# peterropac/Aegolius

Measured on AMD Instinct MI355X. Metric: Mpoints/sec SDF eval, 1024^3 grid, 10-prim smooth-union tree, higher is better.
Workload: dtype f32

## Files before the change

### aegolius_amd/_engine.py

```python
import atexit
import contextlib
import ctypes
import importlib.util
import os
import sys
import threading

import numpy as np

_HERE = os.path.dirname(os.path.abspath(__file__))
LIB_PATH = os.path.join(_HERE, "libsdfk.so")

MODE_AUTO, MODE_INTERPRET, MODE_SPECIALIZED, MODE_NOCULL = 0, 1, 2, 3
(FLAVOUR_PLAIN_ARRAY, FLAVOUR_PLAIN_GRID, FLAVOUR_TILE_ARRAY, FLAVOUR_TILE_GRID, FLAVOUR_TILE_MASK, FLAVOUR_ROWS_ARRAY,
 FLAVOUR_ROWS_GRID, FLAVOUR_ROWS_MASK, FLAVOUR_ROWS2D_ARRAY, FLAVOUR_ROWS2D_GRID, FLAVOUR_RAYS, FLAVOUR_OCCUPANCY) = range(12)
FLAVOUR_FLAGS = 0x100
FLAVOUR_XY = 0x200

_c = ctypes
_vp, _i64, _int, _sz = _c.c_void_p, _c.c_int64, _c.c_int, _c.c_size_t
_fp = _c.POINTER(_c.c_float)

SIGNATURES = {
    "sdfk_abi_version": (_int, []),
    "sdfk_device_count": (_int, []),
    "sdfk_last_error": (_c.c_char_p, []),
    "sdfk_program_create": (_vp, [_vp, _sz, _vp, _sz, _vp, _sz, _int]),
    "sdfk_program_destroy": (None, [_vp]),
    "sdfk_program_set_params": (_int, [_vp, _vp, _sz]),
    "sdfk_program_set_cull": (_int, [_vp, _vp, _sz, _vp]),
    "sdfk_program_source": (_c.c_char_p, [_vp]),
    "sdfk_program_compile_check": (_int, [_vp, _c.POINTER(_sz)]),
    "sdfk_program_chain_members": (_int, [_vp]),
    "sdfk_program_compile_flavour": (_int, [_vp, _int, _c.POINTER(_sz), _c.POINTER(_c.c_double)]),
    "sdfk_debug_compile_external": (_int, [_vp, _int, _c.POINTER(_sz)]),
    "sdfk_debug_jit_stats": (None, [_c.POINTER(_i64), _c.POINTER(_c.c_double)]),
    "sdfk_jit_drain": (None, []),
    "sdfk_jit_cancel": (None, []),
    "sdfk_debug_set_rtc_defs": (None, [_c.c_char_p]),
    "sdfk_eval_device": (_int, [_vp, _vp, _i64, _i64, _vp, _vp, _int]),
    "sdfk_eval_device_rows": (_int, [_vp, _vp, _i64, _i64, _i64, _vp, _vp, _int]),
    "sdfk_eval_device_rows2d": (_int, [_vp, _vp, _i64, _i64, _i64, _vp, _vp, _int]),
    "sdfk_eval_device_rows2d_xy": (_int, [_vp, _vp, _i64, _i64, _i64, _vp, _vp, _int]),
    "sdfk_debug_cells_stats": (None, [_int, _c.POINTER(_c.c_longlong)]),
    "sdfk_debug_rays_stats": (None, [_int, _c.POINTER(_c.c_longlong)]),
    "sdfk_eval_device_rows3d": (_int, [_vp, _vp, _i64, _i64, _i64, _i64, _i64, _vp, _vp, _int]),
    "sdfk_debug_row_masks": (_int, [_vp, _vp, _i64, _i64, _i64, _vp, _c.POINTER(_i64), _c.POINTER(_int), _vp]),
    "sdfk_eval_grid_sharded": (_int, [_vp, _vp, _i64, _vp, _i64, _vp, _i64, _int, _vp, _vp, _int]),
    "sdfk_eval_grid_sharded_device": (_int, [_vp, _vp, _i64, _vp, _i64, _vp, _i64, _int, _vp, _int, _vp, _int]),
    "sdfk_eval_device_aux": (_int, [_vp, _vp, _i64, _i64, _vp, _int, _i64, _vp, _vp, _int]),
    "sdfk_eval_grid_aux": (_int, [_vp, _vp, _i64, _vp, _i64, _vp, _i64, _i64, _i64, _vp, _int, _i64, _vp, _vp, _int]),
    "sdfk_field_min": (_int, [_vp, _i64, _c.POINTER(_c.c_float), _vp]),
    "sdfk_grid_box_average": (_int, [_vp, _i64, _i64, _i64, _int, _int, _int, _int, _vp, _vp]),
    "sdfk_grid_edge_detect": (_int, [_vp, _i64, _i64, _i64, _vp, _vp]),
    "sdfk_debug_box_variant": (_int, [_i64, _i64, _i64, _int, _int, _int, _c.POINTER(_int)]),
    "sdfk_grid_signed": (_int, [_vp, _i64, _i64, _i64, _c.c_float, _int, _vp, _vp]),
    "sdfk_grid_boundary_mask": (_int, [_vp, _i64, _c.c_float, _vp, _vp]),
    "sdfk_grid_signed_slab": (_int, [_vp, _i64, _i64, _vp, _i64, _i64, _i64, _int, _vp, _vp]),
    "sdfk_eval_host": (_int, [_vp, _vp, _int, _i64, _i64, _vp, _int, _int]),
    "sdfk_eval_host_resident": (_int, [_vp, _vp, _int, _i64, _i64, _vp, _int, _int]),
    "sdfk_field_select_scratch": (_sz, [_i64]),
    "sdfk_field_select": (_int, [_vp, _i64, _c.c_float, _vp, _i64, _c.POINTER(_i64), _vp, _vp]),
    "sdfk_field_select_finish": (_int, [_i64, _i64, _vp, _i64, _vp, _vp]),
    "sdfk_field_gradient": (_int, [_vp, _i64, _i64, _i64, _int, _int, _vp, _i64, _vp]),
    "sdfk_field_crossings_2d": (_int, [_vp, _vp, _i64, _i64, _i64, _c.c_double, _c.c_double, _c.c_double, _vp, _vp]),
    "sdfk_lcwg_eval": (_int, [_int, _vp, _vp, _i64, _i64, _i64, _c.c_double, _c.c_double, _int, _c.c_double, _vp, _vp, _i64,
                              _vp]),
    "sdfk_lcwg_old_eval": (_int, [_int, _vp, _i64, _vp, _i64, _c.c_double, _c.c_double, _vp, _i64, _vp]),
    "sdfk_eval_select_scratch": (_sz, [_i64, _i64]),
    "sdfk_eval_device_select": (_int, [_vp, _vp, _i64, _i64, _i64, _int, _c.c_float, _vp, _i64, _c.POINTER(_i64), _vp, _vp, _int]),
    "sdfk_eval_grid_select": (_int, [_vp, _vp, _i64, _vp, _i64, _vp, _i64, _i64, _i64, _c.c_float, _vp, _i64, _c.POINTER(_i64),
                                     _vp, _vp, _int]),
    "sdfk_eval_select_finish": (_int, [_vp, _i64, _i64, _int, _i64, _vp, _i64, _vp, _vp]),
    "sdfk_vec_eval_device": (_int, [_vp, _int, _vp, _i64, _i64, _vp, _int, _i64, _int, _vp, _i64, _vp]),
    "sdfk_vec_set_interpret": (None, [_int]),
    "sdfk_vec_source": (_c.c_char_p, [_vp, _int, _int, _int]),
    "sdfk_vec_compile_check": (_int, [_vp, _int, _int, _int, _c.POINTER(_sz)]),
    "sdfk_vec_eval_host": (_int, [_vp, _int, _vp, _int, _i64, _vp, _i64, _vp, _i64, _vp, _i64, _vp, _int, _int, _vp, _int]),
    "sdfk_eval_grid": (_int, [_vp, _vp, _i64, _vp, _i64, _vp, _i64, _i64, _i64, _vp, _vp, _int]),
    "sdfk_eval_grid_host": (_int, [_vp, _vp, _i64, _vp, _i64, _vp, _i64, _i64, _i64, _vp, _int, _int]),
    "sdfk_set_default_mode": (None, [_int]),
    "sdfk_debug_brick_masks": (_int, [_vp, _vp, _i64, _i64, _vp, _vp]),
    "sdfk_linspace_f32": (_int, [_c.c_double, _c.c_double, _i64, _vp]),
    "sdfk_point_tree_build": (_i64, [_vp, _i64, _int, _vp, _i64, _vp, _vp, _vp]),
    "sdfk_grid_fill": (_int, [_vp, _i64, _vp, _i64, _vp, _i64, _vp, _i64, _i64, _i64, _vp]),
    "sdfk_set_device": (_int, [_int]),
    "sdfk_malloc": (_vp, [_sz]),
    "sdfk_free": (_int, [_vp]),
    "sdfk_memcpy_h2d": (_int, [_vp, _vp, _sz]),
    "sdfk_memcpy_d2h": (_int, [_vp, _vp, _sz]),
    "sdfk_memcpy_d2d": (_int, [_vp, _vp, _sz]),
    "sdfk_sync": (_int, [_vp]),
    "sdfk_event_create": (_vp, []),
    "sdfk_event_destroy": (_int, [_vp]),
    "sdfk_event_record": (_int, [_vp, _vp]),
    "sdfk_event_elapsed_ms": (_int, [_vp, _vp, _fp]),
    "sdfk_stream_probe": (_int, [_vp, _i64, _i64, _vp, _vp]),
    "sdfk_dual_has_rule": (_int, [_int]),
    "sdfk_program_jvp_check": (_int, [_vp, _c.POINTER(_int)]),
    "sdfk_eval_jvp_device": (_int, [_vp, _vp, _i64, _i64, _vp, _int, _int, _vp, _vp, _i64, _vp]),
    "sdfk_value_jvp_device": (_int, [_int, _vp, _vp, _vp, _i64, _vp, _vp, _vp]),
    "sdfk_program_vjp_check": (_int, [_vp, _c.POINTER(_int), _c.POINTER(_i64)]),
    "sdfk_vjp_limits": (_int, [_c.POINTER(_int), _c.POINTER(_int)]),
    "sdfk_eval_vjp_device": (_int, [_vp, _vp, _i64, _i64, _vp, _int, _int, _vp, _vp, _vp, _vp]),
    "sdfk_points_bin": (_int, [_vp, _i64, _i64, _vp, _i64, _i64, _i64, _vp, _vp]),
    "sdfk_points_extent": (_int, [_vp, _i64, _i64, _i64, _vp, _vp]),
    "sdfk_points_fill": (_int, [_vp, _i64, _i64, _i64, _int, _i64, _i64, _i64, _vp]),
    "sdfk_points_widen": (_int, [_vp, _i64, _int, _vp, _vp]),
    "sdfk_field_isosurface_scratch": (_sz, [_i64, _i64, _i64]),
    "sdfk_field_isosurface": (_int, [_vp, _vp, _i64, _vp, _i64, _vp, _i64, _c.c_float, _c.POINTER(_i64), _c.POINTER(_i64), _vp,
                                     _vp]),
    "sdfk_field_isosurface_finish": (_int, [_vp, _i64, _i64, _i64, _c.c_float, _i64, _i64, _vp, _i64, _vp, _i64, _int, _vp,
                                            _vp]),
    "sdfk_field_contour2d_scratch": (_sz, [_i64, _i64]),
    "sdfk_field_contour2d": (_int, [_vp, _vp, _i64, _vp, _i64, _c.c_float, _c.POINTER(_i64), _c.POINTER(_i64), _vp, _vp]),
    "sdfk_field_contour2d_finish": (_int, [_vp, _i64, _i64, _c.c_float, _i64, _i64, _vp, _i64, _vp, _i64, _int, _vp, _vp]),
    "sdfk_eval_grid_isosurface_scratch": (_sz, [_i64, _i64, _i64]),
    "sdfk_eval_grid_isosurface": (_int, [_vp, _vp, _i64, _vp, _i64, _vp, _i64, _c.c_float, _c.POINTER(_i64), _c.POINTER(_i64),
                                         _vp, _vp, _int]),
    "sdfk_eval_grid_isosurface_finish": (_int, [_vp, _vp, _i64, _vp, _i64, _vp, _i64, _c.c_float, _i64, _i64, _vp, _i64, _vp,
                                                _i64, _int, _vp, _vp, _int]),
    "sdfk_eval_grid_contour2d_scratch": (_sz, [_i64, _i64]),
    "sdfk_eval_grid_contour2d": (_int, [_vp, _vp, _i64, _vp, _i64, _c.c_float, _c.POINTER(_i64), _c.POINTER(_i64), _vp, _vp,
                                        _int]),
    "sdfk_eval_grid_contour2d_finish": (_int, [_vp, _vp, _i64, _vp, _i64, _c.c_float, _i64, _i64, _vp, _i64, _vp, _i64, _int,
                                               _vp, _vp, _int]),
    "sdfk_program_rays_check": (_int, [_vp, _c.POINTER(_int)]),
    "sdfk_trace_rays_device": (_int, [_vp, _vp, _i64, _vp, _i64, _i64, _c.c_float, _c.c_float, _c.c_float, _c.c_float,
                                      _c.c_float, _int, _vp, _vp, _vp, _vp, _i64, _vp, _int]),
    "sdfk_trace_camera_device": (_int, [_vp, _vp, _int, _int, _int, _c.c_float, _c.c_float, _c.c_float, _c.c_float,
                                        _c.c_float, _int, _vp, _vp, _vp, _vp, _i64, _vp, _int]),
    "sdfk_eval_grid_occupancy_scratch": (_sz, [_i64, _i64, _i64, _i64]),
    "sdfk_eval_grid_occupancy": (_int, [_vp, _vp, _i64, _vp, _i64, _vp, _i64, _vp, _vp, _vp, _vp, _vp, _vp, _int, _c.c_float,
                                        _c.c_float, _vp, _vp, _i64, _c.POINTER(_i64), _c.POINTER(_i64), _fp, _vp, _int]),
    "sdfk_field_row_sums": (_int, [_vp, _i64, _i64, _vp, _vp, _vp]),
    "sdfk_field_redistance_scratch": (_sz, [_i64, _i64, _i64]),
    "sdfk_field_redistance": (_int, [_vp, _vp, _i64, _vp, _i64, _vp, _i64, _c.c_float, _c.c_float, _int, _vp, _vp,
                                     _c.POINTER(_i64), _fp, _vp]),
    "sdfk_box_pad_ulps": (_int, []),
    "sdfk_box_has_rule": (_int, [_int]),
    "sdfk_program_box_check": (_int, [_vp, _c.POINTER(_int)]),
    "sdfk_enclose_boxes_device": (_int, [_vp, _vp, _vp, _i64, _i64, _vp, _vp, _vp, _vp]),
    "sdfk_enclose_octree_scratch": (_sz, []),
    "sdfk_enclose_octree_device": (_int, [_vp, _vp, _i64, _c.POINTER(_c.c_double), _int, _c.c_float, _vp, _vp, _vp, _i64,
                                          _c.POINTER(_i64), _c.POINTER(_i64), _c.POINTER(_int), _vp, _vp]),
}


class SdfkError(RuntimeError):
    pass


_lib = None
_lock = threading.Lock()


def _share_torch_hip_runtime():
    if "torch" in sys.modules:
        return
    try:
        spec = importlib.util.find_spec("torch")
    except (ImportError, ValueError):
        spec = None
    if spec is None or not spec.submodule_search_locations:
        return
    libdir = os.path.join(list(spec.submodule_search_locations)[0], "lib")
    for name in ("libamdhip64.so", "libhiprtc.so"):
        path = os.path.join(libdir, name)
        if os.path.exists(path):
            try:
                ctypes.CDLL(path, mode=ctypes.RTLD_GLOBAL)
            except OSError:
                return


def lib():
    global _lib
    if _lib is None:
        with _lock:
            if _lib is None:
                if not os.path.exists(LIB_PATH):
                    raise SdfkError(
                        "aegolius_amd: %s is missing - build it with "
                        "`python -c 'import __graft_entry__ as g; g.build()'` (needs hipcc, gfx950). "
                        "There is no CPU path." % LIB_PATH)
                _share_torch_hip_runtime()
                handle = ctypes.CDLL(LIB_PATH)
                for name, (res, args) in SIGNATURES.items():
                    fn = getattr(handle, name)
                    fn.restype, fn.argtypes = res, args
                if handle.sdfk_abi_version() != 1:
                    raise SdfkError("libsdfk.so ABI version mismatch")
                atexit.register(handle.sdfk_jit_cancel)
                _lib = handle
    return _lib


def last_error():
    msg = lib().sdfk_last_error()
    return msg.decode("utf-8", "replace") if msg else ""


def check(rc, what):
    if rc != 0:
        raise SdfkError("%s failed (%d): %s" % (what, rc, last_error()))


def device_count():
    return lib().sdfk_device_count()


def require_gpu():
    if device_count() < 1:
        raise SdfkError("aegolius_amd: no HIP device visible - SDF evaluation runs on an MI355X only "
                        "(there is no CPU path)")


def jit_stats():
    n, t = _i64(0), _c.c_double(0.0)
    lib().sdfk_debug_jit_stats(ctypes.byref(n), ctypes.byref(t))
    return n.value, t.value


def _ptr(a):
    return a.ctypes.data_as(_vp) if a is not None and a.size else None


def _release(owner, attr, destroy):
    try:
        h = getattr(owner, attr, None)
        setattr(owner, attr, None)
        if h and _lib is not None:
            getattr(_lib, destroy)(_vp(h))
    except Exception:
        pass


def coords_n(shape):
    if len(shape) != 2 or shape[0] != 3:
        raise ValueError("coordinates must have shape (3, N); got %r" % (tuple(shape),))
    return int(shape[1])


def host_coords(co, dtype=None):
    co = np.asarray(co)
    coords_n(co.shape)
    if dtype is None and co.dtype not in (np.float32, np.float64):
        dtype = np.float64
    return np.ascontiguousarray(co, dtype=dtype)


def axis_args(axes):
    ax = [np.ascontiguousarray(a, dtype=np.float32) for a in axes]
    args = []
    for a in ax:
        args += [_ptr(a), a.size]
    return ax, tuple(args)


def row_stride(n):
    return (n + 63) // 64 * 64


class DeviceBuffer:

    def __init__(self, nbytes, device=None, what=""):
        self.ptr, self.nbytes, self.device = None, int(nbytes), device if device is None else int(device)
        self.what = what or type(self).__name__
        if device is not None:
            check(lib().sdfk_set_device(self.device), "sdfk_set_device")
        self.ptr = lib().sdfk_malloc(self.nbytes) or None
        if self.ptr is None:
            raise SdfkError("%s: out of device memory (%d bytes): %s" % (self.what, self.nbytes, last_error()))

    def at(self, byte_offset=0, nbytes=0):
        if not self.ptr:
            raise SdfkError("%s has been freed" % self.what)
        if byte_offset < 0 or nbytes < 0 or byte_offset + nbytes > self.nbytes:
            raise SdfkError("%s: bytes [%d, %d) are outside its %d bytes" % (self.what, byte_offset, byte_offset + nbytes,
                                                                             self.nbytes))
        return _vp(self.ptr + byte_offset)

    def _live(self):
        self.at()
        if self.device is not None:
            check(lib().sdfk_set_device(self.device), "sdfk_set_device")

    def upload(self, host, byte_offset=0):
        host = np.ascontiguousarray(host)
        dst = self.at(byte_offset, host.nbytes)
        if host.nbytes:
            check(lib().sdfk_memcpy_h2d(dst, _ptr(host), host.nbytes), "sdfk_memcpy_h2d")

    def download(self, out, byte_offset=0):
        if not out.flags.c_contiguous:
            raise ValueError("%s: download needs a C-contiguous array" % self.what)
        src = self.at(byte_offset, out.nbytes)
        if out.nbytes:
            check(lib().sdfk_memcpy_d2h(_ptr(out), src, out.nbytes), "sdfk_memcpy_d2h")
        return out

    def copy_from(self, device_ptr, nbytes, byte_offset=0):
        dst = self.at(byte_offset, nbytes)
        if nbytes:
            check(lib().sdfk_memcpy_d2d(dst, _vp(device_ptr), nbytes), "sdfk_memcpy_d2d")

    def _filled(self, fill, *args):
        try:
            fill(*args)
        except BaseException:
            self.free()
            raise
        return self

    def free(self):
        _release(self, "ptr", "sdfk_free")

    def __enter__(self):
        return self

    def __exit__(self, *exc):
        self.free()

    def __del__(self):
        self.free()


class DeviceRows(DeviceBuffer):

    def __init__(self, rows, n, device=None, what=""):
        self.rows, self.n, self.stride = int(rows), int(n), row_stride(int(n))
        DeviceBuffer.__init__(self, self.rows * self.stride * 4, device, what)

    def offset(self, r):
        return 4 * r * self.stride

    def row(self, r):
        return self.at(self.offset(r), 4 * self.n)

    def row_ptr(self, r):
        return self.row(r).value

    def upload_rows(self, host):
        for r, line in enumerate(np.ascontiguousarray(host, dtype=np.float32)):
            self.upload(line, self.offset(r))

    def download_rows(self, count=None):
        out = np.empty((self.rows if count is None else count, self.n), dtype=np.float32)
        for r, line in enumerate(out):
            self.download(line, self.offset(r))
        return out


class Program:

    def __init__(self, code, params, tables, result_reg, cull_sites=None, cull_k=None):
        self.code = np.ascontiguousarray(code, dtype=np.uint32).reshape(-1, 2)
        self.params = np.ascontiguousarray(params, dtype=np.float32).ravel()
        self.tables = np.ascontiguousarray(tables, dtype=np.float32).ravel()
        self.result_reg = int(result_reg)
        self._h = lib().sdfk_program_create(_ptr(self.code), self.code.shape[0], _ptr(self.params), self.params.size,
                                            _ptr(self.tables), self.tables.size, self.result_reg)
        if not self._h:
            raise SdfkError("sdfk_program_create rejected the program: " + last_error())
        if cull_sites is not None and len(cull_sites):
            sites = np.ascontiguousarray(cull_sites, dtype=np.uint32).reshape(-1, 5)
            k = np.ascontiguousarray(cull_k, dtype=np.float32).ravel()
            check(lib().sdfk_program_set_cull(self._h, _ptr(sites), sites.shape[0], _ptr(k)), "sdfk_program_set_cull")

    @classmethod
    def from_lowered(cls, low, cull=True):
        if cull:
            return cls(low.code, low.params, low.tables, low.result_reg, low.cull_sites, low.cull_k)
        return cls(low.code, low.params, low.tables, low.result_reg)

    @property
    def handle(self):
        return self._h

    def set_params(self, params):
        p = np.ascontiguousarray(params, dtype=np.float32).ravel()
        check(lib().sdfk_program_set_params(self._h, _ptr(p), p.size), "sdfk_program_set_params")
        self.params = p

    def source(self):
        s = lib().sdfk_program_source(self._h)
        return s.decode() if s else None

    @property
    def chain_members(self):
        return int(lib().sdfk_program_chain_members(self._h))

    def compile_check(self):
        n = _sz(0)
        check(lib().sdfk_program_compile_check(self._h, ctypes.byref(n)), "sdfk_program_compile_check")
        return n.value

    def compile_flavour(self, flavour):
        n, t = _sz(0), _c.c_double(0.0)
        check(lib().sdfk_program_compile_flavour(self._h, int(flavour), ctypes.byref(n), ctypes.byref(t)),
              "sdfk_program_compile_flavour")
        return n.value, t.value

    def eval_host(self, co, device=0, mode=MODE_AUTO):
        require_gpu()
        co = host_coords(co)
        n = co.shape[1]
        out = np.empty(n, dtype=np.float32)
        check(lib().sdfk_eval_host(self._h, _ptr(co), 0 if co.dtype == np.float32 else 1, n, n, _ptr(out), device,
                                   mode), "sdfk_eval_host")
        return out

    def eval_device(self, d_co, n, row_stride, d_out, stream=None, mode=MODE_AUTO, row_len=None, flat=False,
                    plane_rows=None, first_row_in_plane=0):
        if row_len and plane_rows and not flat:
            check(lib().sdfk_eval_device_rows3d(self._h, _vp(d_co), n, row_stride, int(row_len), int(plane_rows),
                                                int(first_row_in_plane), _vp(d_out), _vp(stream or 0), mode),
                  "sdfk_eval_device_rows3d")
            return
        if row_len and flat:
            check(lib().sdfk_eval_device_rows2d(self._h, _vp(d_co), n, row_stride, int(row_len), _vp(d_out),
                                                _vp(stream or 0), mode), "sdfk_eval_device_rows2d")
            return
        if row_len:
            check(lib().sdfk_eval_device_rows(self._h, _vp(d_co), n, row_stride, int(row_len), _vp(d_out),
                                              _vp(stream or 0), mode), "sdfk_eval_device_rows")
            return
        check(lib().sdfk_eval_device(self._h, _vp(d_co), n, row_stride, _vp(d_out), _vp(stream or 0), mode),
              "sdfk_eval_device")

    def eval_device_xy(self, d_xy, n, row_stride, d_out, stream=None, mode=MODE_AUTO, row_len=None):
        check(lib().sdfk_eval_device_rows2d_xy(self._h, _vp(d_xy), n, row_stride, int(row_len or 0), _vp(d_out),
                                               _vp(stream or 0), mode), "sdfk_eval_device_rows2d_xy")

    def eval_grid(self, axes, start, count, d_out, stream=None, mode=MODE_AUTO):
        _, tab = axis_args(axes)
        check(lib().sdfk_eval_grid(self._h, *tab, start, count, _vp(d_out), _vp(stream or 0), mode), "sdfk_eval_grid")

    def _select(self, n, first, device, row_len=0, mode=MODE_AUTO):
        require_gpu()
        L = lib()
        check(L.sdfk_set_device(int(device)), "sdfk_set_device")

        def finish(m, d_index, d_scratch):
            check(L.sdfk_eval_select_finish(self._h, n, int(row_len), mode, m, d_index, m, d_scratch, None),
                  "sdfk_eval_select_finish")
        return _select(L.sdfk_eval_select_scratch(n, int(row_len)), first, finish)

    def select_grid(self, axes, threshold=0.0, start=0, count=None, device=0, mode=MODE_AUTO):
        ax, tab = axis_args(axes)
        total = ax[0].size * ax[1].size * ax[2].size
        count = total - start if count is None else count

        def first(d_scratch, m):
            check(lib().sdfk_eval_grid_select(self._h, *tab, start, count, float(threshold), None, 0, m, d_scratch, None,
                                              mode), "sdfk_eval_grid_select")
        grow = ax[2].size if ax[2].size > 1 else ax[1].size
        return self._select(count, first, device, row_len=grow if start % grow == 0 and count % grow == 0 else 0, mode=mode)

    def mesh_grid(self, axes, level, device=0, mode=MODE_AUTO, timings=None):
        require_gpu()
        check(lib().sdfk_set_device(int(device)), "sdfk_set_device")
        ax, tab = axis_args(axes)
        if len(ax) not in (2, 3):
            raise ValueError("mesh_grid: two or three axis tables")
        lead = (self._h,) + tab
        return extract_mesh("sdfk_eval_grid", [a.size for a in ax], level, lead, lead, (mode,), timings)

    def occupancy_grid(self, axes, sub_tables, half_widths, samples, level, lipschitz, d_out, slab_cells=0, device=0,
                       mode=MODE_AUTO, timings=None):
        require_gpu()
        L = lib()
        check(L.sdfk_set_device(int(device)), "sdfk_set_device")
        ax, tab = axis_args(axes)
        if len(ax) != 3 or len(sub_tables) != 3 or len(half_widths) != 3:
            raise ValueError("occupancy_grid: three axis, sub-sample and half-width tables")
        k = [int(samples) if a.size > 1 else 1 for a in ax]
        sub = [np.ascontiguousarray(t, dtype=np.float32) for t in sub_tables]
        hw = [np.ascontiguousarray(t, dtype=np.float32) for t in half_widths]
        for a, s, h, ka in zip(ax, sub, hw, k):
            if s.shape != (a.size * ka,) or h.shape != (a.size,):
                raise ValueError("occupancy_grid: an axis of %d points takes %d sub-samples and %d half-widths; got %r and %r"
                                 % (a.size, a.size * ka, a.size, s.shape, h.shape))
        shape = [a.size for a in ax]
        inside, near = _i64(0), _i64(0)
        ms = (_c.c_float * 3)() if timings is not None else None
        with DeviceBuffer(L.sdfk_eval_grid_occupancy_scratch(*shape, int(slab_cells)), what="occupancy") as scratch:
            check(L.sdfk_eval_grid_occupancy(self._h, *tab, *[_ptr(s) for s in sub], *[_ptr(h) for h in hw], int(samples),
                                             float(level), float(lipschitz), _vp(d_out), scratch.at(), int(slab_cells),
                                             ctypes.byref(inside), ctypes.byref(near), ms, None, mode),
                  "sdfk_eval_grid_occupancy")
        if timings is not None:
            for name, value in zip(("centre", "classify", "sample"), ms):
                timings[name] = timings.get(name, 0.0) + float(value)
        return int(inside.value), int(near.value)

    def select_host(self, co, threshold=0.0, device=0, mode=MODE_AUTO):
        require_gpu()
        co32 = host_coords(co, np.float32)
        n = co32.shape[1]
        if n == 0:
            return np.empty(0, dtype=np.int64)
        L = lib()
        check(L.sdfk_set_device(int(device)), "sdfk_set_device")
        with DeviceCoords(co32, what="select") as d_co:
            row_len, flat = 0, 0
            head = co32[:, :min(n, 1 << 22)]
            ch = np.flatnonzero((head[0] != head[0, 0]) | (head[1] != head[1, 0]))
            if ch.size and ch[0] >= 32 and n % int(ch[0]) == 0:
                row_len = int(ch[0])
            else:
                cx = np.flatnonzero(head[0] != head[0, 0])
                if cx.size and cx[0] >= 32 and n % int(cx[0]) == 0:
                    row_len = int(cx[0])
                    flat = int(co32[2, 0] == 0 and co32[2, row_len - 1] == 0 and co32[2, -1] == 0)

            def first(d_scratch, m):
                check(L.sdfk_eval_device_select(self._h, _vp(d_co.ptr), n, d_co.stride, row_len, flat, float(threshold), None,
                                                0, m, d_scratch, None, mode), "sdfk_eval_device_select")
            return self._select(n, first, device, row_len=row_len, mode=mode)

    def eval_grid_host(self, axes, start=0, count=None, device=0, mode=MODE_AUTO):
        require_gpu()
        ax, tab = axis_args(axes)
        total = ax[0].size * ax[1].size * ax[2].size
        count = total - start if count is None else count
        out = np.empty(count, dtype=np.float32)
        check(lib().sdfk_eval_grid_host(self._h, *tab, start, count, _ptr(out), device, mode), "sdfk_eval_grid_host")
        return out

    def eval_grid_sharded(self, axes, n_shards, devices=None, mode=MODE_AUTO):
        require_gpu()
        ax, tab = axis_args(axes)
        out = np.empty(ax[0].size * ax[1].size * ax[2].size, dtype=np.float32)
        dev = None if devices is None else np.ascontiguousarray(devices, dtype=np.int32)
        if dev is not None and dev.size != n_shards:
            raise ValueError("one device per shard")
        check(lib().sdfk_eval_grid_sharded(self._h, *tab, n_shards, _ptr(dev) if dev is not None else None, _ptr(out), mode),
              "sdfk_eval_grid_sharded")
        return out

    def eval_grid_sharded_resident(self, axes, n_shards, devices=None, gather_device=0, mode=MODE_AUTO):
        require_gpu()
        ax, tab = axis_args(axes)
        dev = None if devices is None else np.ascontiguousarray(devices, dtype=np.int32)
        if dev is not None and dev.size != n_shards:
            raise ValueError("one device per shard")
        field = DeviceField(ax[0].size * ax[1].size * ax[2].size, gather_device)
        check(lib().sdfk_eval_grid_sharded_device(self._h, *tab, n_shards, _ptr(dev) if dev is not None else None,
                                                  int(gather_device), _vp(field.ptr), mode), "sdfk_eval_grid_sharded_device")
        return field

    def __del__(self):
        _release(self, "_h", "sdfk_program_destroy")

# ... 234 lines not shown
```

### aegolius_amd/csrc/sdfk.hip

```cpp
#include <hip/hip_runtime.h>
#include <hip/hiprtc.h>

#include <chrono>
#include <algorithm>
#include <atomic>
#include <cmath>
#include <condition_variable>
#include <cstdio>
#include <cstdlib>
#include <cstring>
#include <deque>
#include <functional>
#include <map>
#include <memory>
#include <mutex>
#include <thread>
#include <string>
#include <vector>
#include <dirent.h>
#include <dlfcn.h>
#include <fcntl.h>
#include <signal.h>
#include <spawn.h>
#include <sys/wait.h>
// ... 436 lines not shown
            if (wv[b] && !(is_comb && b == result_vreg)) return false;
            if (wv[c] && !(is_comb && c == result_vreg)) return false;
        }
        (kind == SDFK_KIND_C_C ? wc : wv)[a] = 0;
    }
    return !wv[(unsigned)p->result_reg];
}

static bool is_cullable_op(unsigned op) {
    return op == SDFK_OP_VMIN || op == SDFK_OP_VMAX || op == SDFK_OP_VSUBTRACT || op == SDFK_OP_SMIN2 ||
           op == SDFK_OP_SMIN3 || op == SDFK_OP_SMAX3 || op == SDFK_OP_SSUB3;
}

extern "C" int sdfk_program_set_cull(sdfk_program* p, const uint32_t* rows, size_t n_sites, const float* k) {
    if (!p) return fail(-1, "null program");
    if (n_sites > 32767) return fail(-2, "sdfk_program_set_cull: at most 32767 sites");
    if (n_sites && (!rows || !k)) return fail(-1, "sdfk_program_set_cull: null arrays");
    std::lock_guard<std::mutex> lk(p->mu);
    if (!p->source.empty() || !p->dev.empty())
        return fail(-2, "sdfk_program_set_cull: must be called before the program is first used");
    if (p->n_aux > 0) n_sites = 0;
    const size_t n = p->code.size() / 2;
    std::vector<sdfk_cullsite> sites;
    for (size_t i = 0; i < n_sites; ++i) {
        sdfk_cullsite t{rows[5 * i], rows[5 * i + 1], rows[5 * i + 2], rows[5 * i + 3], rows[5 * i + 4], k[i], 0, 0};
        if (!(t.comb < n && t.a0 <= t.a1 && t.a1 + 1 == t.b0 && t.b0 <= t.b1 && t.b1 + 1 == t.comb))
            return fail(-2, "sdfk_program_set_cull: malformed site ranges");
        if (!(t.k >= 0.0f) || !std::isfinite(t.k)) return fail(-2, "sdfk_program_set_cull: bad Lipschitz sum");
        unsigned op, a, b, c;
        instr_fields(p, t.comb, &op, &a, &b, &c);
        if (!is_cullable_op(op)) return fail(-2, "sdfk_program_set_cull: site is not at a min/max-type combiner");
        if (i && rows[5 * i] <= rows[5 * (i - 1)]) return fail(-2, "sdfk_program_set_cull: sites must be sorted");
        for (const sdfk_cullsite& u : sites) {
            const bool disjoint = u.comb < t.a0;
            const bool nested = u.a0 >= t.a0 && (u.comb <= t.a1 || (u.a0 >= t.b0 && u.comb <= t.b1));
            if (!disjoint && !nested) return fail(-2, "sdfk_program_set_cull: sites overlap without nesting");
        }
        t.skip_a_ok = range_skippable(p, t.a0, t.a1, t.comb, b) ? 1 : 0;
        t.skip_b_ok = range_skippable(p, t.b0, t.b1, t.comb, c) ? 1 : 0;
        sites.push_back(t);
    }
    p->sites_all = sites;
    if (sites.size() > SDFK_MASK_SITES) {
        std::vector<size_t> order(sites.size());
        for (size_t i = 0; i < order.size(); ++i) order[i] = i;
        std::stable_sort(order.begin(), order.end(), [&](size_t x, size_t y) {
            return (sites[x].a1 - sites[x].a0) + (sites[x].b1 - sites[x].b0) > (sites[y].a1 - sites[y].a0) + (sites[y].b1 - sites[y].b0);
        });
        order.resize(SDFK_MASK_SITES);
        std::sort(order.begin(), order.end());
        std::vector<sdfk_cullsite> widest;
        for (size_t i : order) widest.push_back(sites[i]);
        sites.swap(widest);
    }
    p->sites = sites;
    p->chain_members = sdfk_chain_mode(g_ops, SDFK_OP_COUNT, p->code.data(), p->code.size() / 2, p->result_reg, p->sites_all);
    p->chain_mode = p->chain_members > 0;
    p->key.append("|cull");
    for (const sdfk_cullsite& t : p->sites_all) {
        p->key.append(reinterpret_cast<const char*>(&t), sizeof t);
    }
    return 0;
}

extern "C" const char* sdfk_program_source(sdfk_program* p) {
    if (!p) return nullptr;
    std::lock_guard<std::mutex> lk(p->mu);
    if (p->source.empty())
        p->source = sdfk_generate_source(g_ops, SDFK_OP_COUNT, p->code.data(), p->code.size() / 2, p->result_reg,
                                         p->sites, SDFK_FL_ALL, &p->sites_all);
    return p->source.c_str();
}

static std::atomic<int> g_twaves_override{0}, g_rwbricks_override{0};
static int tile_waves() {
    static int v = [] { const char* e = getenv("SDFK_TWAVES"); int t = e ? atoi(e) : 4; return (t >= 1 && t <= 16) ? t : 4; }();
    const int o = g_twaves_override.load();
    return o ? o : v;
}
static int tile_wbricks() {
    static int v = [] {
        const char* e = getenv("SDFK_WBRICKS");
        int t = e ? atoi(e) : 4;
        if (t < 1 || t > 32) t = 4;
        return t;
    }();
    return v;
}
static int tile_points() { return tile_waves() * tile_wbricks() * 128; }
static std::atomic<int> g_rwaves_override{0};
static int rows_waves(const sdfk_program*) {
    if (const int o = g_rwaves_override.load()) return o;
    return 4;
}
static int rows_wbricks(const sdfk_program* p);
static long long big_program_limit() {
    static const long long v = [] {
        const char* e = getenv("SDFK_BIG_PROGRAM");
        const long long t = e ? atoll(e) : 300;
        return t > 0 ? t : 300;
    }();
    return v;
}
static int rows_geo(const sdfk_program* p) {
    const bool big = p && !p->chain_mode && (long long)(p->code.size() / 2) > big_program_limit();
    return rows_wbricks(p) | (rows_waves(p) << 4) | (big ? 1 << 16 : 0);
}
static int rows_wbricks(const sdfk_program* p) {
    static int forced = [] { const char* e = getenv("SDFK_RWBRICKS"); int t = e ? atoi(e) : 0; return (t >= 1 && t <= 16) ? t : 0; }();
    if (const int o = g_rwbricks_override.load()) return o;
    if (forced) return forced;
    if (p && p->chain_mode) return p->chain_members <= 64 ? 2 : 1;
    return 2;
}
struct RowGeom {
    unsigned L, nchunk, nbricks;
    long long R;
    long long row0;
    int yrows;
    unsigned prow, seg0, nb0, bpp;
    unsigned inv_nchunk, inv_bpp;
};
static bool rows_geometry(long long n, long long row_len, RowGeom* g, long long plane_rows = 0, long long plane_phase = 0,
                          bool planes_on = false) {
    if (row_len < 32 || row_len > 0x7fffffffLL || n <= 0 || n % row_len != 0) return false;
    const long long R = n / row_len, brows = 16;
    const long long nchunk = (row_len % 32 == 0) ? row_len / 32 : (row_len + 62) / 32;
    long long prow = plane_rows, seg0 = 0;
    static const bool plane_blocks = [] { const char* e = getenv("SDFK_PLANE_BLOCKS"); return e && e[0] == '1'; }();
    if (!(plane_blocks || planes_on) || prow <= 0 || prow >= R || prow > 0x7fffffffLL) {
        prow = R > 0x7fffffffLL ? 0 : R;
        if (prow == 0) return false;
    } else if (plane_phase > 0) {
        seg0 = std::min(R, (prow - plane_phase % prow) % prow);
    }
    const long long nb0 = (seg0 + brows - 1) / brows, bpp = (prow + brows - 1) / brows;
    const long long planes = (R - seg0 + prow - 1) / prow;
    const long long nb = nchunk * (nb0 + planes * bpp);
    if (nb > 0x7fffffffLL - 1024) return false;
    g->L = (unsigned)row_len;
    g->nchunk = (unsigned)nchunk;
    g->nbricks = (unsigned)nb;
    g->R = R;
    g->row0 = 0;
    g->yrows = 0;
    g->prow = (unsigned)prow;
    g->seg0 = (unsigned)seg0;
    g->nb0 = (unsigned)nb0;
    g->bpp = (unsigned)bpp;
    g->inv_nchunk = (unsigned)std::min<unsigned long long>(0xffffffffull, (1ull << 32) / (unsigned long long)nchunk);
    g->inv_bpp = (unsigned)std::min<unsigned long long>(0xffffffffull, (1ull << 32) / (unsigned long long)bpp);
    return true;
}
static int tile_threads() { return 64 * tile_waves(); }
static std::string rtc_cache_dir() {
    static const std::string dir = [] {
        std::string d;
        if (const char* e = getenv("SDFK_CACHE_DIR")) {
            d = e;
            if (d.empty() || d == "off" || d == "0") return std::string();
        } else if (const char* x = getenv("XDG_CACHE_HOME"); x && *x) {
            d = std::string(x) + "/sdfk";
        } else if (const char* h = getenv("HOME"); h && *h) {
            (void)mkdir((std::string(h) + "/.cache").c_str(), 0700);
            d = std::string(h) + "/.cache/sdfk";
        } else {
            return std::string();
        }
        (void)mkdir(d.c_str(), 0700);
        return d;
    }();
    return dir;
}
static std::string rtc_cache_path(const std::string& src, const std::string& opts) {
    const std::string dir = rtc_cache_dir();
    if (dir.empty()) return std::string();
    int major = 0, minor = 0;
    (void)hiprtcVersion(&major, &minor);
    unsigned long long h = 1469598103934665603ull;
    auto mix = [&](const std::string& t) {
        for (unsigned char c : t) {
            h ^= c;
            h *= 1099511628211ull;
        }
    };
    mix(src);
    mix(opts);
    mix(std::to_string(major) + "." + std::to_string(minor) + "/abi" + std::to_string(SDFK_ABI_VERSION));
    char name[96];
    snprintf(name, sizeof name, "/sdfk-%016llx-%zu.co", h, src.size());
    return dir + name;
}
static const unsigned long long kCacheMagic = 0x53444643'4f424a31ull;
static unsigned long long fnv1a(const char* p, size_t n) {
    unsigned long long h = 1469598103934665603ull;
    for (size_t i = 0; i < n; ++i) {
        h ^= (unsigned char)p[i];
        h *= 1099511628211ull;
    }
    return h;
}
static bool rtc_cache_read(const std::string& path, std::vector<char>* out) {
    if (path.empty()) return false;
    FILE* f = fopen(path.c_str(), "rb");
    if (!f) return false;
    bool ok = false;
    if (fseek(f, 0, SEEK_END) == 0) {
        const long size = ftell(f);
        if (size > 24 && fseek(f, 0, SEEK_SET) == 0) {
            out->resize((size_t)size);
            ok = fread(out->data(), 1, (size_t)size, f) == (size_t)size;
            if (ok) {
                unsigned long long tr[3];
                memcpy(tr, out->data() + size - 24, 24);
                ok = tr[0] == kCacheMagic && tr[1] == (unsigned long long)(size - 24) && tr[2] == fnv1a(out->data(), (size_t)size - 24);
                out->resize((size_t)size - 24);
            }
        }
    }
    fclose(f);
    if (!ok) {
        out->clear();
        (void)remove(path.c_str());
    } else {
        (void)utimes(path.c_str(), nullptr);
    }
    return ok;
}
static void rtc_cache_evict(const std::string& dir) {
    static const long long cap = [] {
        const char* e = getenv("SDFK_CACHE_MAX_MB");
        const long long v = e ? atoll(e) : 512;
        return (v > 0 ? v : 512) * (1ll << 20);
    }();
    DIR* d = opendir(dir.c_str());
    if (!d) return;
    std::vector<std::pair<long long, std::pair<std::string, long long>>> files;
    long long total = 0;
    while (dirent* e = readdir(d)) {
        const std::string name = e->d_name;
        if (name.compare(0, 5, "sdfk-") != 0 || name.compare(0, 9, "sdfk-rtc-") == 0) continue;
        struct stat st;
        const std::string path = dir + "/" + name;
        if (stat(path.c_str(), &st) != 0) continue;
        total += (long long)st.st_size;
        files.push_back({(long long)st.st_mtime, {path, (long long)st.st_size}});
    }
    closedir(d);
    if (total <= cap) return;
    std::sort(files.begin(), files.end());
    for (const auto& f : files) {
        if (total <= cap / 4 * 3) break;
        if (remove(f.second.first.c_str()) == 0) total -= f.second.second;
    }
}
static void rtc_cache_write(const std::string& path, const std::vector<char>& co) {
    if (path.empty() || co.empty()) return;
    const std::string tmp = path + ".tmp" + std::to_string((long long)getpid());
    FILE* f = fopen(tmp.c_str(), "wb");
    if (!f) return;
    const unsigned long long tr[3] = {kCacheMagic, (unsigned long long)co.size(), fnv1a(co.data(), co.size())};
    bool ok = fwrite(co.data(), 1, co.size(), f) == co.size() && fwrite(tr, 1, sizeof tr, f) == sizeof tr;
    ok = (fclose(f) == 0) && ok;
    if (!ok || rename(tmp.c_str(), path.c_str()) != 0) (void)remove(tmp.c_str());
    else rtc_cache_evict(rtc_cache_dir());
}

static std::mutex g_rtc_mu;
static std::mutex g_defs_mu;
static std::string g_rtc_defs = [] { const char* e = getenv("SDFK_RTC_DEFS"); return std::string(e ? e : ""); }();
extern "C" void sdfk_debug_set_rtc_defs(const char* defs) {
    std::lock_guard<std::mutex> lk(g_defs_mu);
    std::string rest;
    int tw = 0, rwb = 0, rwv = 0;
    const std::string all = defs ? defs : "";
    size_t pos = 0;
    while (pos < all.size()) {
        size_t sp = all.find(' ', pos);
        if (sp == std::string::npos) sp = all.size();
        const std::string tok = all.substr(pos, sp - pos);
        if (tok.compare(0, 14, "-DSDFK_TWAVES=") == 0) tw = atoi(tok.c_str() + 14);
        else if (tok.compare(0, 16, "-DSDFK_RWBRICKS=") == 0) rwb = atoi(tok.c_str() + 16);
        else if (tok.compare(0, 14, "-DSDFK_RWAVES=") == 0) rwv = atoi(tok.c_str() + 14);
        else if (!tok.empty()) rest += tok + " ";
        pos = sp + 1;
    }
    g_twaves_override = (tw >= 1 && tw <= 16) ? tw : 0;
    g_rwbricks_override = (rwb >= 1 && rwb <= 15) ? rwb : 0;
    g_rwaves_override = (rwv >= 1 && rwv <= 16) ? rwv : 0;
    g_rtc_defs = rest;
}
static std::vector<std::string> rtc_options(int geo) {
    const int rwb = geo & 15, rwaves = ((geo >> 4) & 0xff) ? ((geo >> 4) & 0xff) : 4;
    const bool big = (geo >> 16) & 1;
    const char* opt = getenv("SDFK_RTC_OPT");
    std::vector<std::string> o = {"--offload-arch=gfx950", (opt && opt[0] == '-') ? opt : "-O3", "-ffp-contract=off", "-std=c++17",
                                  "-fno-honor-nans", "-mno-amdgpu-ieee",
                                  "-DSDFK_TWAVES=" + std::to_string(tile_waves()), "-DSDFK_WBRICKS=" + std::to_string(tile_wbricks()),
                                  "-DSDFK_RWBRICKS=" + std::to_string(rwb), "-DSDFK_RWAVES=" + std::to_string(rwaves)};
    if (big) {
        o.push_back("-mllvm");
        o.push_back("-disable-cgp");
        o.push_back("-mllvm");
        o.push_back("-disable-vector-combine");
    }
    if (const char* extra = getenv("SDFK_RTC_EXTRA")) {
        std::string e = extra;
        size_t q = 0;
        while (q < e.size()) {
            size_t sp = e.find(' ', q);
            if (sp == std::string::npos) sp = e.size();
            if (sp > q) o.push_back(e.substr(q, sp - q));
            q = sp + 1;
        }
    }
    std::string all;
    {
        std::lock_guard<std::mutex> lk(g_defs_mu);
        all = g_rtc_defs;
    }
    size_t pos = 0;
    while (pos < all.size()) {
        size_t sp = all.find(' ', pos);
        if (sp == std::string::npos) sp = all.size();
        if (sp > pos && all.compare(pos, 2, "-D") == 0) o.push_back(all.substr(pos, sp - pos));
        pos = sp + 1;
    }
    return o;
}
static std::string rtc_option_key(int rwb) {
    std::string k;
    for (const std::string& o : rtc_options(rwb)) k += o + " ";
    return k;
}
static int rtc_compile_uncached(const std::string& src, std::vector<char>* out, std::string* log, int rwb) {
    hiprtcProgram prog = nullptr;
    if (hiprtcCreateProgram(&prog, src.c_str(), "sdfk_spec.hip", 0, nullptr, nullptr) != HIPRTC_SUCCESS) {
        *log = "hiprtcCreateProgram failed";
        return -1;
    }
    const std::vector<std::string> o = rtc_options(rwb);
    std::vector<const char*> opts;
    for (const std::string& x : o) opts.push_back(x.c_str());
    hiprtcResult r = hiprtcCompileProgram(prog, (int)opts.size(), opts.data());
    size_t ls = 0;
    hiprtcGetProgramLogSize(prog, &ls);
    if (ls > 1) {
        log->resize(ls);
        hiprtcGetProgramLog(prog, &(*log)[0]);
    }
    if (r != HIPRTC_SUCCESS) {
        *log = std::string("hiprtc: ") + hiprtcGetErrorString(r) + "\n" + *log;
        hiprtcDestroyProgram(&prog);
        return -1;
    }
    size_t cs = 0;
    hiprtcGetCodeSize(prog, &cs);
    out->resize(cs);
    hiprtcGetCode(prog, out->data());
    hiprtcDestroyProgram(&prog);
    return 0;
}
extern char** environ;
static std::string rtc_helper_path() {
    static const std::string path = [] {
        if (const char* e = getenv("SDFK_RTC_HELPER")) return std::string(strcmp(e, "off") && strcmp(e, "0") ? e : "");
        Dl_info info;
        if (!dladdr((void*)&sdfk_abi_version, &info) || !info.dli_fname) return std::string();
        std::string p = info.dli_fname;
        const size_t slash = p.rfind('/');
        p = (slash == std::string::npos ? std::string(".") : p.substr(0, slash)) + "/sdfk_rtc_helper";
        return access(p.c_str(), X_OK) == 0 ? p : std::string();
    }();
    return path;
}
static std::string rtc_library_path() {
    Dl_info info;
    if (!dladdr((void*)&hiprtcCompileProgram, &info) || !info.dli_fname) return std::string();
    return info.dli_fname;
}
static bool rtc_helper_available() { return !rtc_helper_path().empty() && !rtc_library_path().empty(); }
static std::atomic<bool> g_cancel_builds{false};
static int rtc_compile_external(const std::string& src, std::vector<char>* out, std::string* log, int rwb) {
    static std::atomic<unsigned> serial{0};
    const std::string helper = rtc_helper_path(), lib = rtc_library_path();
    if (helper.empty() || lib.empty()) {
        *log = "sdfk_rtc_helper is not available";
        return -2;
    }
    std::string dir = rtc_cache_dir();
    if (dir.empty()) {
        const char* t = getenv("TMPDIR");
        dir = (t && *t) ? t : "/tmp";
    }
    (void)serial;
    std::string priv = dir + "/sdfk-rtc-XXXXXX";
    if (!mkdtemp(&priv[0])) {
        *log = "cannot create a private directory under " + dir + ": " + strerror(errno);
        return -2;
    }
    const std::string srcf = priv + "/src.hip", outf = priv + "/out.co";
    auto cleanup = [&] {
        (void)remove(srcf.c_str());
        (void)remove(outf.c_str());
        (void)remove((outf + ".tmp").c_str());
        (void)remove((outf + ".log").c_str());
        (void)rmdir(priv.c_str());
    };
    {
        const int fd = open(srcf.c_str(), O_WRONLY | O_CREAT | O_EXCL | O_CLOEXEC, 0600);
        FILE* f = fd >= 0 ? fdopen(fd, "wb") : nullptr;
        if (!f && fd >= 0) close(fd);
        const bool ok = f && fwrite(src.data(), 1, src.size(), f) == src.size();
        if (!f || fclose(f) != 0 || !ok) {
            cleanup();
            *log = "cannot write " + srcf;
            return -2;
        }
    }
    const std::vector<std::string> o = rtc_options(rwb);
    std::vector<char*> argv = {const_cast<char*>(helper.c_str()), const_cast<char*>(lib.c_str()), const_cast<char*>(srcf.c_str()),
                               const_cast<char*>(outf.c_str())};
    for (const std::string& x : o) argv.push_back(const_cast<char*>(x.c_str()));
    argv.push_back(nullptr);
    posix_spawn_file_actions_t fa;
    posix_spawn_file_actions_init(&fa);
    posix_spawn_file_actions_addclosefrom_np(&fa, 3);
    pid_t pid = 0;
    const int rc = posix_spawn(&pid, helper.c_str(), &fa, nullptr, argv.data(), environ);
    posix_spawn_file_actions_destroy(&fa);
    if (rc != 0) {
        cleanup();
        *log = std::string("posix_spawn of sdfk_rtc_helper: ") + strerror(rc);
        return -2;
    }
    static const double limit_s = [] { const char* e = getenv("SDFK_RTC_TIMEOUT"); const double v = e ? atof(e) : 0.0; return v > 0.0 ? v : 900.0; }();
    int status = 0;
    bool timed_out = false, cancelled = false;
    const auto t_spawn = std::chrono::steady_clock::now();
    for (;;) {
        const pid_t w = waitpid(pid, &status, WNOHANG);
        if (w == pid) break;
// ... 37 lines not shown
            const size_t n = fread(buf, 1, sizeof buf - 1, f);
            buf[n] = 0;
            *log += std::string(": ") + buf;
            fclose(f);
        }
    }
    cleanup();
    return result;
}

static int rtc_compile(const std::string& src, std::vector<char>* out, std::string* log, int rwb, bool* from_disk = nullptr,
                       std::string* disk_path = nullptr, bool external = false) {
    if (from_disk) *from_disk = false;
    const std::string path = rtc_cache_path(src, rtc_option_key(rwb));
    if (rtc_cache_read(path, out)) {
        if (from_disk) *from_disk = true;
        if (disk_path) *disk_path = path;
        return 0;
    }
    int rc = -2;
    if (rtc_helper_available()) rc = rtc_compile_external(src, out, log, rwb);
    if (rc == -2 && !external) {
        static std::atomic<bool> told{false};
        if (!told.exchange(true))
            fprintf(stderr, "[sdfk] compiler helper unavailable (%s): building inside this process — do not import HIP libraries on "
                            "other threads meanwhile\n", log->empty() ? "sdfk_rtc_helper not found next to libsdfk.so" : log->c_str());
        std::lock_guard<std::mutex> lk(g_rtc_mu);
        rc = rtc_compile_uncached(src, out, log, rwb);
    }
    if (rc == 0) rtc_cache_write(path, *out);
    return rc;
}

static const char* const kFlavourFn[SDFK_FL_COUNT][2] = {
    {"sdfk_spec_v4", "sdfk_spec_v1"}, {"sdfk_spec_g4", "sdfk_spec_g1"}, {"sdfk_spec_t", nullptr}, {"sdfk_spec_tg", nullptr},
    {"sdfk_spec_tmask", nullptr},     {"sdfk_spec_r", nullptr},         {"sdfk_spec_rg", nullptr}, {"sdfk_spec_rmask", nullptr},
    {"sdfk_spec_r", nullptr},         {"sdfk_spec_rg", nullptr},        {"sdfk_spec_rays", "sdfk_spec_raycam"},
    {"sdfk_spec_occ_list", "sdfk_spec_occ_all"}};

struct BuildWorker {
    static constexpr int kThreads = 2;
    std::mutex mu;
    std::condition_variable cv;
    std::deque<std::function<void()>> jobs;
    std::vector<std::thread> threads;
    bool stop = false;
    int busy = 0;
    void post(std::function<void()> job) {
        std::lock_guard<std::mutex> lk(mu);
        jobs.push_back(std::move(job));
        if ((int)threads.size() < kThreads && (int)threads.size() < busy + (int)jobs.size())
            threads.emplace_back([this] { loop(); });
        cv.notify_all();
    }
    void loop() {
        std::unique_lock<std::mutex> lk(mu);
        for (;;) {
            cv.wait(lk, [this] { return stop || !jobs.empty(); });
            if (jobs.empty()) return;
            std::function<void()> job = std::move(jobs.front());
            jobs.pop_front();
            ++busy;
            lk.unlock();
            job();
            lk.lock();
            --busy;
            cv.notify_all();
        }
    }
    void drain() {
        std::unique_lock<std::mutex> lk(mu);
        cv.wait(lk, [this] { return jobs.empty() && busy == 0; });
    }
    void drop_queued() {
        std::lock_guard<std::mutex> lk(mu);
        jobs.clear();
        cv.notify_all();
    }
    ~BuildWorker() {
        {
            std::lock_guard<std::mutex> lk(mu);
            stop = true;
            cv.notify_all();
        }
        for (std::thread& t : threads)
            if (t.joinable()) t.join();
    }
};
static BuildWorker g_builds;
extern "C" void sdfk_jit_drain(void) { g_builds.drain(); }
extern "C" void sdfk_jit_cancel(void) {
    g_cancel_builds.store(true);
    g_builds.drop_queued();
    g_builds.drain();
}
static std::atomic<long long> g_compile_count{0};
static std::atomic<long long> g_compile_micros{0};
extern "C" void sdfk_debug_jit_stats(int64_t* builds, double* seconds) {
    if (builds) *builds = g_compile_count.load();
    if (seconds) *seconds = (double)g_compile_micros.load() * 1e-6;
}

static std::shared_ptr<CodeObject> code_entry(const std::string& key) {
    std::lock_guard<std::mutex> lk(g_code_mu);
    std::shared_ptr<CodeObject>& e = g_code[key];
    if (!e) e = std::make_shared<CodeObject>();
    return e;
}
static void code_build(const std::shared_ptr<CodeObject>& e, const std::string& src, int rwb, bool external = false) {
    const auto t0 = std::chrono::steady_clock::now();
    std::vector<char> co;
    std::string log;
    bool from_disk = false;
    std::string disk_path;
    const int rc = rtc_compile(src, &co, &log, rwb, &from_disk, &disk_path, external);
    const double dt = std::chrono::duration<double>(std::chrono::steady_clock::now() - t0).count();
    if (!from_disk) {
        g_compile_count++;
        g_compile_micros += (long long)(dt * 1e6);
    }
    std::lock_guard<std::mutex> lk(e->mu);
    e->build_seconds = dt;
    if (rc == 0) {
        e->co.swap(co);
        e->disk_path = disk_path;
        e->state = 2;
    } else {
        e->error = log;
        e->state = 3;
        e->failed_at = std::chrono::steady_clock::now();
    }
    e->cv.notify_all();
}
template <typename MakeSource>
static std::shared_ptr<CodeObject> code_get(const std::string& key, MakeSource make_source, int rwb, bool wait) {
    std::shared_ptr<CodeObject> e = code_entry(key);
    std::unique_lock<std::mutex> lk(e->mu);
    if (e->state == 3 && std::chrono::steady_clock::now() - e->failed_at > std::chrono::seconds(30)) e->state = 0;
    if (e->state == 0) {
        e->state = 1;
        lk.unlock();
        const std::string src = make_source();
        if (wait || !rtc_helper_available()) {
            code_build(e, src, rwb);
        } else {
            g_builds.post([e, src, rwb] { code_build(e, src, rwb, true); });
        }
        return e;
    }
    if (wait) e->cv.wait(lk, [&] { return e->state != 1; });
    return e;
}
static std::string flavour_key(const sdfk_program* p, int flavour, int rwb, int with_flags = 0) {
    return p->key + "|f" + std::to_string(flavour) + ((with_flags & 1) ? "s" : "") + ((with_flags & 2) ? "x" : "") + "|" + rtc_option_key(rwb);
}
static std::string flavour_source(const sdfk_program* p, int flavour, int with_flags = 0) {
    return std::string((with_flags & 1) ? "#define SDFK_FLAGS 1\n" : "") + ((with_flags & 2) ? "#define SDFK_XY 1\n" : "") +
           sdfk_generate_source(g_ops, SDFK_OP_COUNT, p->code.data(), p->code.size() / 2, p->result_reg, p->sites, flavour,
                                &p->sites_all);
}

extern "C" int sdfk_program_chain_members(const sdfk_program* p) {
    return p && p->chain_mode ? p->chain_members : 0;
}
extern "C" int sdfk_program_compile_check(sdfk_program* p, size_t* code_size) {
    if (!p) return fail(-1, "null program");
    size_t total = 0;
    const int rwb = rows_geo(p);
    for (int f = 0; f < SDFK_FL_COUNT; ++f) {
        if (f == SDFK_FL_RAYS) continue;
        if (f == SDFK_FL_OCCUPANCY) continue;
        if (p->sites.empty() && f != SDFK_FL_PLAIN_ARRAY && f != SDFK_FL_PLAIN_GRID) continue;
        if (p->chain_mode && (f == SDFK_FL_TILE_ARRAY || f == SDFK_FL_TILE_GRID || f == SDFK_FL_TILE_MASK || f == SDFK_FL_ROWS_MASK)) continue;
        std::shared_ptr<CodeObject> e = code_get(flavour_key(p, f, rwb), [&] { return flavour_source(p, f); }, rwb, true);
        if (e->state != 2) return fail(-3, e->error);
        total += e->co.size();
    }
    if (code_size) *code_size = total;
    return 0;
}
extern "C" int sdfk_program_compile_flavour(sdfk_program* p, int flavour, size_t* code_size, double* seconds) {
    if (!p) return fail(-1, "null program");
    int with_flags = 0;
    if (flavour >= 0 && (flavour & SDFK_FLAVOUR_FLAGS)) with_flags |= 1;
    if (flavour >= 0 && (flavour & SDFK_FLAVOUR_XY)) with_flags |= 2;
    if (flavour >= 0) flavour &= ~(SDFK_FLAVOUR_FLAGS | SDFK_FLAVOUR_XY);
    if (flavour < 0 || flavour >= SDFK_FL_COUNT) return fail(-1, "sdfk_program_compile_flavour: unknown flavour");
    if (p->sites.empty() && flavour != SDFK_FL_PLAIN_ARRAY && flavour != SDFK_FL_PLAIN_GRID && flavour != SDFK_FL_RAYS &&
        flavour != SDFK_FL_OCCUPANCY)
        return fail(-2, "sdfk_program_compile_flavour: the program has no cull sites");
    if (with_flags && flavour == SDFK_FL_RAYS)
        return fail(-2, "sdfk_program_compile_flavour: the ray flavour has no flag-writing or two-row build");
    if (with_flags && flavour == SDFK_FL_OCCUPANCY)
        return fail(-2, "sdfk_program_compile_flavour: the occupancy flavour has no flag-writing or two-row build");
    if ((with_flags & 2) && flavour != SDFK_FL_PLAIN_ARRAY && flavour != SDFK_FL_ROWS2D_ARRAY)
        return fail(-2, "sdfk_program_compile_flavour: two-row coordinates exist for the plain and the flat row-block array kernels");
    if ((with_flags & 1) && (flavour == SDFK_FL_TILE_ARRAY || flavour == SDFK_FL_TILE_GRID || flavour == SDFK_FL_TILE_MASK ||
                       flavour == SDFK_FL_ROWS_MASK))
        return fail(-2, "sdfk_program_compile_flavour: this flavour has no flag-writing build");
    const int rwb = rows_geo(p);
    const auto t0 = std::chrono::steady_clock::now();
    std::shared_ptr<CodeObject> e =
        code_get(flavour_key(p, flavour, rwb, with_flags), [&] { return flavour_source(p, flavour, with_flags); }, rwb, true);
    if (e->state != 2) return fail(-3, e->error);
    if (code_size) *code_size = e->co.size();
    if (seconds) *seconds = std::chrono::duration<double>(std::chrono::steady_clock::now() - t0).count();
    return 0;
}

extern "C" int sdfk_debug_compile_external(sdfk_program* p, int flavour, size_t* code_size) {
    if (!p) return fail(-1, "null program");
    if (flavour < 0 || flavour >= SDFK_FL_COUNT) return fail(-1, "sdfk_debug_compile_external: unknown flavour");
    if (p->sites.empty() && flavour != SDFK_FL_PLAIN_ARRAY && flavour != SDFK_FL_PLAIN_GRID && flavour != SDFK_FL_RAYS &&
        flavour != SDFK_FL_OCCUPANCY)
        return fail(-2, "sdfk_debug_compile_external: the program has no cull sites");
    if (!rtc_helper_available()) return fail(-9, "sdfk_rtc_helper is not next to libsdfk.so (or hiprtc cannot be located)");
    std::vector<char> co;
    std::string log;
    if (rtc_compile_external(flavour_source(p, flavour), &co, &log, rows_geo(p)) != 0) return fail(-3, log);
    if (code_size) *code_size = co.size();
    return 0;
}

static std::shared_ptr<SpecModule> get_module(sdfk_program* p, int device, int flavour, bool wait, std::string* err,
                                              int with_flags = 0) {
    const int rwb = rows_geo(p);
    const std::string key = flavour_key(p, flavour, rwb, with_flags);
    std::shared_ptr<SpecModule> m;
    {
        std::lock_guard<std::mutex> lk(g_code_mu);
        std::shared_ptr<SpecModule>& slot = g_mods[std::make_pair(device, key)];
        if (!slot) slot = std::make_shared<SpecModule>();
        m = slot;
    }
    std::lock_guard<std::mutex> lk(m->mu);
    if (m->loaded) return m;
    for (int attempt = 0;; ++attempt) {
        std::shared_ptr<CodeObject> e;
        {
            std::lock_guard<std::mutex> ce(g_code_mu);
            auto it = g_code.find(key);
            if (it != g_code.end()) e = it->second;
        }
        int state = 0;
        if (e) {
            std::lock_guard<std::mutex> el(e->mu);
            state = e->state;
        }
        if (state != 2) {
            e = code_get(key, [&] { return flavour_source(p, flavour, with_flags); }, rwb, wait);
            std::lock_guard<std::mutex> el(e->mu);
            state = e->state;
        }
        if (state == 1) return nullptr;
        if (state != 2) {
            std::lock_guard<std::mutex> el(e->mu);
            *err = e->error;
            m->failed = true;
            m->error = e->error;
            return m;
        }
        hipError_t he;
        {
            std::lock_guard<std::mutex> rl(g_rtc_mu);
            he = hipModuleLoadData(&m->mod, e->co.data());
        }
        for (int i = 0; i < 2 && he == hipSuccess; ++i)
            if (kFlavourFn[flavour][i]) he = hipModuleGetFunction(&m->fn[i], m->mod, kFlavourFn[flavour][i]);
        if (he == hipSuccess && p->chain_mode && !kFlavourFn[flavour][1]) {
            const bool grid_fl = flavour == SDFK_FL_ROWS_GRID || flavour == SDFK_FL_ROWS2D_GRID;
            if (hipModuleGetFunction(&m->fn[1], m->mod, grid_fl ? "sdfk_spec_cellsg" : "sdfk_spec_cells") != hipSuccess) {
                m->fn[1] = nullptr;
                (void)hipGetLastError();
            }
        }
        if (he == hipSuccess && flavour == SDFK_FL_RAYS) {
            if (hipModuleGetFunction(&m->fn[2], m->mod, "sdfk_spec_rays_cull") != hipSuccess ||
                hipModuleGetFunction(&m->fn[3], m->mod, "sdfk_spec_raycam_cull") != hipSuccess) {
                m->fn[2] = m->fn[3] = nullptr;
                (void)hipGetLastError();
            }
        }
        if (he == hipSuccess) break;
        bool retry = false;
        {
            std::lock_guard<std::mutex> el(e->mu);
            if (attempt == 0 && e->state == 2 && !e->disk_path.empty()) {
                (void)remove(e->disk_path.c_str());
                fprintf(stderr, "[sdfk] cached code object %s does not load (%s): rebuilding\n", e->disk_path.c_str(),
                        hipGetErrorString(he));
                e->disk_path.clear();
                e->co.clear();
                e->state = 0;
                retry = true;
            }
        }
        if (m->mod) {
            (void)hipModuleUnload(m->mod);
            m->mod = nullptr;
        }
        (void)hipGetLastError();
        if (retry) {
            wait = true;
            continue;
        }
        m->failed = true;
        m->error = std::string("hipModuleLoadData/GetFunction: ") + hipGetErrorString(he);
        *err = m->error;
        return m;
    }
    m->failed = false;
    m->loaded = true;
    return m;
}

static int ensure_resident(sdfk_program* p, int device, hipStream_t stream, DevState** out) {
    std::lock_guard<std::mutex> lk(p->mu);
    DevState& d = p->dev[device];
    if (!d.d_code) {
        HIPCHK(hipMalloc(&d.d_code, p->code.size() * sizeof(uint32_t)));
        HIPCHK(hipMemcpy(d.d_code, p->code.data(), p->code.size() * sizeof(uint32_t), hipMemcpyHostToDevice));
        HIPCHK(hipMalloc(&d.d_params, std::max<size_t>(p->params.size(), 1) * sizeof(float)));
        HIPCHK(hipMalloc(&d.d_tables, std::max<size_t>(p->tables.size(), 1) * sizeof(float)));
        if (!p->tables.empty())
            HIPCHK(hipMemcpy(d.d_tables, p->tables.data(), p->tables.size() * sizeof(float), hipMemcpyHostToDevice));
    }
    if (d.params_version != p->params_version) {
        if (!p->params.empty()) {
            HIPCHK(hipMemcpyAsync(d.d_params, p->params.data(), p->params.size() * sizeof(float),
                                  hipMemcpyHostToDevice, stream));
            HIPCHK(hipStreamSynchronize(stream));
        }
        d.params_version = p->params_version;
    }
    *out = &d;
    return 0;
}

static inline unsigned blocks_for(long long n, int vec) {
    return (unsigned)((n + (long long)SDFK_BLOCK * vec - 1) / ((long long)SDFK_BLOCK * vec));
}

static std::atomic<bool> g_cells_stats_on{false};
static std::mutex g_cells_stats_mu;
static long long g_cells_stats[8] = {0, 0, 0, 0, 0, 0, 0, 0};
extern "C" void sdfk_debug_cells_stats(int enable, long long* out8) {
    g_cells_stats_on.store(enable != 0);
    if (out8) {
        std::lock_guard<std::mutex> lk(g_cells_stats_mu);
        for (int i = 0; i < 8; ++i) out8[i] = g_cells_stats[i];
        for (int i = 0; i < 8; ++i) g_cells_stats[i] = 0;
    }
}
struct CellLevelH {
    unsigned lx, ly, lz, ncx, ncy, ncz, xoff, pad;
};
struct CellsArg {
    CellLevelH lv;
    const void *sph, *span, *cand;
    unsigned enabled, ncells;
};
struct CellPassArg {
    CellLevelH lv, parent;
    void *sph, *span;
    const void *psph, *pspan;
    void* cand;
    unsigned* head;
    unsigned base, shard_cap;
    unsigned ncells, pad0;
    float inflate, pad;
};
static bool parse3(const char* e, unsigned* v) {
    int a = 0, b = 0, c = 0;
    if (!e || sscanf(e, "%d,%d,%d", &a, &b, &c) != 3 || a < 0 || b < 0 || c < 0 || a > 12 || b > 12 || c > 12) return false;
    v[0] = (unsigned)a; v[1] = (unsigned)b; v[2] = (unsigned)c;
    return true;
}
static CellLevelH cell_level(const RowGeom& rg, const unsigned l[3]) {
    CellLevelH lv{};
    lv.lx = l[0]; lv.ly = l[1]; lv.lz = l[2];
    const long long planes = rg.prow ? ((rg.R - rg.seg0) + rg.prow - 1) / rg.prow : 0;
    lv.xoff = rg.seg0 > 0 ? (1u << lv.lx) : 0u;
    lv.ncx = planes > 0 ? (unsigned)(((long long)lv.xoff + planes - 1) >> lv.lx) + 1u : 1u;
    lv.ncy = ((std::max(rg.bpp, rg.nb0) - 1u) >> lv.ly) + 1u;
    lv.ncz = ((rg.nchunk - 1u) >> lv.lz) + 1u;
    return lv;
}
static int prepare_cells(sdfk_program* p, DevState* d, hipFunction_t cells_fn, const RowGeom& rg, void** src, int n_src,
                         const float* prm, const float* tab, hipStream_t stream, CellsArg* out) {
    memset(out, 0, sizeof *out);
    static const int min_members = [] { const char* e = getenv("SDFK_CELLS_MIN"); const int v = e ? atoi(e) : 0; return v > 0 ? v : 17; }();
    static const bool off = [] { const char* e = getenv("SDFK_CELLS"); return e && e[0] == '0'; }();
    if (!cells_fn || off || p->chain_members < min_members) return 0;
    const bool is3d = rg.prow < (unsigned long long)rg.R;
    unsigned lf[3] = {is3d ? 3u : 0u, is3d ? 1u : 2u, is3d ? 0u : 1u};
    unsigned lc[3] = {lf[0] + (is3d ? 2u : 0u), lf[1] + 2u, lf[2] + 2u};
    static const char* e_fine = getenv("SDFK_CELL_FINE");
    static const char* e_coarse = getenv("SDFK_CELL_COARSE");
    (void)parse3(e_fine, lf);
    bool coarse = p->chain_members >= 128;
    if (e_coarse) coarse = parse3(e_coarse, lc);
    if (coarse && (lc[0] < lf[0] || lc[1] < lf[1] || lc[2] < lf[2])) coarse = false;
    const CellLevelH fine = cell_level(rg, lf);
    const CellLevelH crs = coarse ? cell_level(rg, lc) : CellLevelH{};
    const unsigned long long nf = (unsigned long long)fine.ncx * fine.ncy * fine.ncz;
    const unsigned long long nc = coarse ? (unsigned long long)crs.ncx * crs.ncy * crs.ncz : 0ull;
    if (nf == 0 || nf > 0x3fffffffull || nc > 0x3fffffffull) return 0;
    const unsigned long long members = (unsigned long long)p->chain_members, shards = 256;
    unsigned long long cshard = ((nc + shards - 1) / shards) * members;
    unsigned long long fshard = std::max(members, std::min(((nf + shards - 1) / shards) * members, (256ull * nf + (16ull << 20) + shards - 1) / shards));
    if (const char* e = getenv("SDFK_CELLS_POOL")) {
        const long long v = atoll(e);
        if (v > 0) fshard = std::min<unsigned long long>(fshard, (unsigned long long)v);
    }
    if (shards * (cshard + fshard) > 0x3fffffffull) return 0;
    const unsigned long long cap = shards * (cshard + fshard);
    const size_t o_fsph = 0, o_fspan = o_fsph + 16 * nf, o_csph = o_fspan + 8 * nf, o_cspan = o_csph + 16 * nc,
                 o_head = (o_cspan + 8 * nc + 63) & ~(size_t)63, o_pool = o_head + 2 * 64 * shards, total = o_pool + 4 * cap + 64;
    CellScratch* cs;
    {
        std::lock_guard<std::mutex> lk(p->mu);
        cs = &d->cells[stream];
    }
    if (cs->bytes < total) {
        if (cs->buf) {
            HIPCHK(hipStreamSynchronize(stream));
            (void)hipFree(cs->buf);
            cs->buf = nullptr;
            cs->bytes = 0;
        }
        if (hipMalloc(&cs->buf, total + total / 4) != hipSuccess) { (void)hipGetLastError(); return 0; }
        cs->bytes = total + total / 4;
    }
    char* b = cs->buf;
    HIPCHK(hipMemsetAsync(b + o_head, 0, 2 * 64 * shards, stream));
    CellPassArg cp{};
    cp.cand = b + o_pool;
    if (coarse) {
        cp.lv = crs; cp.parent = CellLevelH{}; cp.sph = b + o_csph; cp.span = b + o_cspan; cp.psph = nullptr; cp.pspan = nullptr;
        cp.ncells = (unsigned)nc; cp.inflate = 1.3f;
        cp.head = reinterpret_cast<unsigned*>(b + o_head);
        cp.base = 0u; cp.shard_cap = (unsigned)cshard;
        std::vector<void*> args = {(void*)&prm, (void*)&tab};
        for (int i = 0; i < n_src; ++i) args.push_back(src[i]);
        RowGeom g2 = rg;
        args.push_back(&g2);
        args.push_back(&cp);
        HIPCHK(hipModuleLaunchKernel(cells_fn, (unsigned)((nc + 3) / 4), 1, 1, 256, 1, 1, 0, stream, args.data(), nullptr));
    }
    cp.lv = fine; cp.parent = coarse ? crs : CellLevelH{}; cp.sph = b + o_fsph; cp.span = b + o_fspan;
    cp.psph = coarse ? b + o_csph : nullptr; cp.pspan = coarse ? b + o_cspan : nullptr;
    cp.ncells = (unsigned)nf; cp.inflate = 1.0f;
    cp.head = reinterpret_cast<unsigned*>(b + o_head + 64 * shards);
    cp.base = (unsigned)(shards * cshard); cp.shard_cap = (unsigned)fshard;
    {
        std::vector<void*> args = {(void*)&prm, (void*)&tab};
        for (int i = 0; i < n_src; ++i) args.push_back(src[i]);
        RowGeom g2 = rg;
        args.push_back(&g2);
        args.push_back(&cp);
        HIPCHK(hipModuleLaunchKernel(cells_fn, (unsigned)((nf + 3) / 4), 1, 1, 256, 1, 1, 0, stream, args.data(), nullptr));
    }
    static const bool trace = [] { const char* e = getenv("SDFK_CELLS_TRACE"); return e && e[0] == '1'; }();
    if (trace || g_cells_stats_on.load()) {
        HIPCHK(hipStreamSynchronize(stream));
        std::vector<uint2> sp(nf);
        unsigned head = 0;
        HIPCHK(hipMemcpy(sp.data(), b + o_fspan, 8 * nf, hipMemcpyDeviceToHost));
        {
            std::vector<unsigned> heads(2 * 16 * shards);
            HIPCHK(hipMemcpy(heads.data(), b + o_head, 2 * 64 * shards, hipMemcpyDeviceToHost));
            for (size_t i = 0; i < heads.size(); i += 16) head += heads[i];
        }
        unsigned long long sum = 0, all = 0, empty = 0, mx = 0;
        for (const uint2& x : sp) {
            if (x.y == 0xffffffffu) ++all;
            else { sum += x.y; mx = std::max<unsigned long long>(mx, x.y); if (x.y == 0) ++empty; }
        }
        {
            std::lock_guard<std::mutex> lk(g_cells_stats_mu);
            g_cells_stats[0] = (long long)nf; g_cells_stats[1] = (long long)nc; g_cells_stats[2] = (long long)head;
            g_cells_stats[3] = (long long)cap; g_cells_stats[4] = (long long)sum; g_cells_stats[5] = (long long)mx;
            g_cells_stats[6] = (long long)all; g_cells_stats[7] = (long long)empty;
        }
        if (trace) fprintf(stderr, "[sdfk cells] %d members: fine %ux%ux%u = %llu cells (2^%u planes x 2^%u blocks x 2^%u windows), coarse %llu; pool %u of %llu entries; "
                "fine lists: mean %.1f max %llu, %llu without a list, %llu empty\n", p->chain_members, fine.ncx, fine.ncy, fine.ncz, nf, fine.lx, fine.ly, fine.lz, nc,
                head, cap, (double)sum / (double)std::max<unsigned long long>(1, nf - all - empty), mx, all, empty);
    }
    out->lv = fine;
    out->sph = b + o_fsph;
    out->span = b + o_fspan;
    out->cand = b + o_pool;
    out->enabled = 1u;
    out->ncells = (unsigned)nf;
    return 0;
}

static int run(sdfk_program* p, const SrcArray* arr, const SrcGrid* grid, long long n, float* d_out, void* stream_,
               int mode, bool vec_ok, long long row_len = 0, const float* aux = nullptr, long long aux_stride = 0,
               bool flat = false, long long plane_rows = 0, long long plane_phase = 0, unsigned* d_flags = nullptr,
               unsigned thr_key = 0, bool xy = false) {
    if (!p) return fail(-1, "null program");
    if (n < 0) return fail(-1, "negative point count");
    if (p->n_aux > 0 && (!aux || aux_stride < n))
        return fail(-1, "this program reads auxiliary fields (staged evaluation): use sdfk_eval_device_aux / sdfk_eval_grid_aux");
    if (n == 0) return 0;
    if (mode == SDFK_MODE_AUTO) mode = g_default_mode;
    if (d_flags && (mode == SDFK_MODE_AUTO || mode == SDFK_MODE_INTERPRET)) mode = SDFK_MODE_SPECIALIZED;
    if (xy) {
        if (!arr || p->n_aux > 0) return fail(-1, "two-row coordinates: array source, no auxiliary fields");
        if (mode == SDFK_MODE_AUTO || mode == SDFK_MODE_INTERPRET) mode = SDFK_MODE_SPECIALIZED;
    }
    hipStream_t stream = (hipStream_t)stream_;
    int device = 0;
    HIPCHK(hipGetDevice(&device));
    DevState* d = nullptr;
    int rc = ensure_resident(p, device, stream, &d);
    if (rc) return rc;

    long long n4 = vec_ok ? (n / 4) * 4 : 0;
    long long tail = n - n4;

    static const long long spec_limit = [] {
        const char* e = getenv("SDFK_SPECIALIZE_LIMIT");
        const long long v = e ? atoll(e) : 1200;
        return v > 0 ? v : 1200;
    }();
    static const long long rows_limit = [] {
        const char* e = getenv("SDFK_ROWS_LIMIT");
        const long long v = e ? atoll(e) : 1200;
        return v > 0 ? v : 1200;
    }();
    if (mode == SDFK_MODE_AUTO && (long long)(p->code.size() / 2) > spec_limit && p->interp_ok && !p->chain_mode && !d_flags)
        mode = SDFK_MODE_INTERPRET;

    RowGeom rg;
    int flavour = arr ? SDFK_FL_PLAIN_ARRAY : SDFK_FL_PLAIN_GRID;
    const long long grow = grid ? (grid->n2 > 1 ? (long long)grid->n2 : (long long)grid->n1) : 0;
    if (!p->sites.empty() && mode != SDFK_MODE_NOCULL && mode != SDFK_MODE_INTERPRET) {
        if (arr && rows_geometry(n, row_len, &rg, (flat || d_flags) ? 0 : plane_rows, plane_phase, p->chain_mode))
            flavour = (flat || xy) ? SDFK_FL_ROWS2D_ARRAY : SDFK_FL_ROWS_ARRAY;
        else if (arr && vec_ok && !p->chain_mode && !d_flags && !xy) flavour = SDFK_FL_TILE_ARRAY;
        else if (grid && grid->start % grow == 0 &&
                 rows_geometry(n, grow, &rg, (grid->n2 > 1 && !d_flags) ? (long long)grid->n1 : 0,
                               grid->n2 > 1 ? (grid->start / grow) % (long long)grid->n1 : 0, p->chain_mode))
            flavour = grid->n2 > 1 ? SDFK_FL_ROWS_GRID : SDFK_FL_ROWS2D_GRID;
        else if (grid && vec_ok && !p->chain_mode && !d_flags) flavour = SDFK_FL_TILE_GRID;
        if (!p->chain_mode && (long long)(p->code.size() / 2) > rows_limit &&
            (flavour == SDFK_FL_ROWS_ARRAY || flavour == SDFK_FL_ROWS2D_ARRAY || flavour == SDFK_FL_ROWS_GRID || flavour == SDFK_FL_ROWS2D_GRID)) {
            const bool is_arr = arr != nullptr;
            if (vec_ok && !d_flags && !xy) flavour = is_arr ? SDFK_FL_TILE_ARRAY : SDFK_FL_TILE_GRID;
            else if (!d_flags) flavour = is_arr ? SDFK_FL_PLAIN_ARRAY : SDFK_FL_PLAIN_GRID;
        }
    }
    std::shared_ptr<SpecModule> sk;
    if (mode != SDFK_MODE_INTERPRET) {
        static const bool async_jit = [] { const char* e = getenv("SDFK_ASYNC_JIT"); return !(e && e[0] == '0'); }();
        const bool wait = mode != SDFK_MODE_AUTO || !p->interp_ok || !async_jit;
        std::string err;
        sk = get_module(p, device, flavour, wait, &err, (d_flags ? 1 : 0) | (xy ? 2 : 0));
        if (sk && sk->failed) {
            if (mode == SDFK_MODE_SPECIALIZED || !p->interp_ok)
                return fail(-3, "specialised kernel unavailable: " + err);
            static bool warned = false;
            if (!warned) {
                fprintf(stderr, "[sdfk] hiprtc specialisation failed, using the interpreter kernel: %s\n", err.c_str());
                warned = true;
            }
            sk.reset();
        }
    }
    if (!sk && !p->interp_ok)
        return fail(-4, "program needs more registers than the interpreter kernel has (use the specialised mode)");

    const float* prm = d->d_params;
    const float* tab = d->d_tables;
    if (sk) {
        if (flavour == SDFK_FL_ROWS_ARRAY || flavour == SDFK_FL_ROWS_GRID || flavour == SDFK_FL_ROWS2D_ARRAY ||
            flavour == SDFK_FL_ROWS2D_GRID) {
            const unsigned per_tile = (unsigned)(rows_waves(p) * rows_wbricks(p));
            const unsigned tiles = ((rg.nbricks + per_tile - 1) / per_tile + 127u) & ~127u;
            const unsigned rthreads = 64u * (unsigned)rows_waves(p);
            CellsArg cells{};
            const bool with_cells = p->chain_mode && sk->fn[1] != nullptr;
            if (arr) {
                const float* co = arr->co;
                long long stride = arr->stride;
                if (with_cells) {
                    void* src[] = {&co, &stride};
                    rc = prepare_cells(p, d, sk->fn[1], rg, src, 2, prm, tab, stream, &cells);
                    if (rc) return rc;
                }
                void* args[] = {&prm, &tab, &co, &stride, &rg, &d_out, &d_flags, &thr_key, &cells};
                HIPCHK(hipModuleLaunchKernel(sk->fn[0], tiles, 1, 1, rthreads, 1, 1, 0, stream, args, nullptr));
            } else {
                SrcGrid g = *grid;
                rg.row0 = grid->start / grow;
                rg.yrows = grid->n2 > 1 ? 0 : 1;
                if (with_cells) {
                    void* src[] = {&g};
                    rc = prepare_cells(p, d, sk->fn[1], rg, src, 1, prm, tab, stream, &cells);
                    if (rc) return rc;
                }
                void* args[] = {&prm, &tab, &g, &rg, &d_out, &d_flags, &thr_key, &cells};
                HIPCHK(hipModuleLaunchKernel(sk->fn[0], tiles, 1, 1, rthreads, 1, 1, 0, stream, args, nullptr));
            }
            return 0;
        }
        if (flavour == SDFK_FL_TILE_ARRAY || flavour == SDFK_FL_TILE_GRID) {
            const unsigned tiles = (unsigned)((n + tile_points() - 1) / tile_points());
            if (arr) {
                const float* co = arr->co;
                long long stride = arr->stride;
                void* args[] = {&prm, &tab, &co, &stride, &n, &d_out};
                HIPCHK(hipModuleLaunchKernel(sk->fn[0], tiles, 1, 1, tile_threads(), 1, 1, 0, stream, args, nullptr));
            } else {
                SrcGrid g = *grid;
                void* args[] = {&prm, &tab, &g, &n, &d_out};
                HIPCHK(hipModuleLaunchKernel(sk->fn[0], tiles, 1, 1, tile_threads(), 1, 1, 0, stream, args, nullptr));
            }
            return 0;
        }
        if (arr) {
            const float* co = arr->co;
            long long stride = arr->stride;
            if (n4) {
                long long off = 0;
                void* args[] = {&prm, &tab, &co, &stride, &off, &n4, &d_out, &aux, &aux_stride, &d_flags, &thr_key};
                HIPCHK(hipModuleLaunchKernel(sk->fn[0], blocks_for(n4, 4), 1, 1, SDFK_BLOCK, 1, 1, 0, stream, args,
                                             nullptr));
            }
            if (tail) {
                long long off = n4;
                void* args[] = {&prm, &tab, &co, &stride, &off, &tail, &d_out, &aux, &aux_stride, &d_flags, &thr_key};
                HIPCHK(hipModuleLaunchKernel(sk->fn[1], blocks_for(tail, 1), 1, 1, SDFK_BLOCK, 1, 1, 0, stream, args,
                                             nullptr));
            }
        } else {
            SrcGrid g = *grid;
            if (n4) {
                long long off = 0;
                void* args[] = {&prm, &tab, &g, &off, &n4, &d_out, &aux, &aux_stride, &d_flags, &thr_key};
                HIPCHK(hipModuleLaunchKernel(sk->fn[0], blocks_for(n4, 4), 1, 1, SDFK_BLOCK, 1, 1, 0, stream, args,
                                             nullptr));
            }
            if (tail) {
                long long off = n4;
                void* args[] = {&prm, &tab, &g, &off, &tail, &d_out, &aux, &aux_stride, &d_flags, &thr_key};
                HIPCHK(hipModuleLaunchKernel(sk->fn[1], blocks_for(tail, 1), 1, 1, SDFK_BLOCK, 1, 1, 0, stream, args,
                                             nullptr));
            }
        }
        return 0;
    }
    if (d_flags) return fail(-3, "fused selection needs the specialised kernels");
    const int n_instr = (int)(p->code.size() / 2);
    const long long zero = 0;
    auto launch = [&](auto src, int vec, long long off, long long cnt) {
        using SRC = decltype(src);
        const dim3 grid(blocks_for(cnt, vec)), block(SDFK_BLOCK);
#define SDFK_INTERP_GO(VEC, NC, NV) hipLaunchKernelGGL((sdfk_interp_kernel<VEC, NC, NV, SRC>), grid, block, 0, stream, d->d_code, \
                                                        n_instr, prm, tab, src, off, cnt, d_out, p->result_reg, aux, aux_stride)
        if (vec == 4) {
            if (p->interp_small) SDFK_INTERP_GO(4, SDFK_NC_SMALL, SDFK_NV_SMALL);
            else SDFK_INTERP_GO(4, SDFK_NC, SDFK_NV);
        } else {
            if (p->interp_small) SDFK_INTERP_GO(1, SDFK_NC_SMALL, SDFK_NV_SMALL);
            else SDFK_INTERP_GO(1, SDFK_NC, SDFK_NV);
        }
#undef SDFK_INTERP_GO
    };
    if (arr) {
        if (n4) launch(*arr, 4, zero, n4);
        if (tail) launch(*arr, 1, n4, tail);
    } else {
        if (n4) launch(*grid, 4, zero, n4);
        if (tail) launch(*grid, 1, n4, tail);
    }
    HIPCHK(hipGetLastError());
    return 0;
}

static bool aligned16(const void* p) { return (reinterpret_cast<uintptr_t>(p) & 15u) == 0; }

extern "C" int sdfk_eval_device(sdfk_program* p, const float* d_co, int64_t n, int64_t row_stride, float* d_out,
                                void* stream, int mode) {
    if (!d_co || !d_out) return fail(-1, "sdfk_eval_device: null device pointer");
    if (row_stride < n) return fail(-1, "sdfk_eval_device: row stride smaller than the point count");
    SrcArray a = {d_co, (long long)row_stride};
    bool vec_ok = aligned16(d_co) && aligned16(d_out) && (row_stride % 4 == 0);
    return run(p, &a, nullptr, n, d_out, stream, mode, vec_ok);
}

extern "C" int sdfk_eval_device_rows(sdfk_program* p, const float* d_co, int64_t n, int64_t row_stride, int64_t row_len,
                                     float* d_out, void* stream, int mode) {
    if (!d_co || !d_out) return fail(-1, "sdfk_eval_device_rows: null device pointer");
    if (row_stride < n) return fail(-1, "sdfk_eval_device_rows: row stride smaller than the point count");
    if (row_len < 1 || (n > 0 && n % row_len != 0))
        return fail(-1, "sdfk_eval_device_rows: the point count is not a multiple of the row length");
    SrcArray a = {d_co, (long long)row_stride};
    bool vec_ok = aligned16(d_co) && aligned16(d_out) && (row_stride % 4 == 0);
    return run(p, &a, nullptr, n, d_out, stream, mode, vec_ok, row_len);
}

extern "C" int sdfk_eval_device_rows2d_xy(sdfk_program* p, const float* d_xy, int64_t n, int64_t row_stride, int64_t row_len,
                                          float* d_out, void* stream, int mode) {
    if (!d_xy || !d_out) return fail(-1, "sdfk_eval_device_rows2d_xy: null device pointer");
    if (row_stride < n) return fail(-1, "sdfk_eval_device_rows2d_xy: row stride smaller than the point count");
    if (row_len < 0 || (row_len > 0 && n > 0 && n % row_len != 0))
        return fail(-1, "sdfk_eval_device_rows2d_xy: the point count is not a multiple of the row length");
    SrcArray a = {d_xy, (long long)row_stride};
    bool vec_ok = aligned16(d_xy) && aligned16(d_out) && (row_stride % 4 == 0);
    return run(p, &a, nullptr, n, d_out, stream, mode, vec_ok, row_len, nullptr, 0, row_len > 0, 0, 0, nullptr, 0, true);
}

extern "C" int sdfk_eval_device_rows3d(sdfk_program* p, const float* d_co, int64_t n, int64_t row_stride, int64_t row_len,
                                       int64_t plane_rows, int64_t first_row_in_plane, float* d_out, void* stream, int mode) {
    if (!d_co || !d_out) return fail(-1, "sdfk_eval_device_rows3d: null device pointer");
    if (row_stride < n) return fail(-1, "sdfk_eval_device_rows3d: row stride smaller than the point count");
    if (row_len < 1 || (n > 0 && n % row_len != 0))
        return fail(-1, "sdfk_eval_device_rows3d: the point count is not a multiple of the row length");
    if (plane_rows < 0 || first_row_in_plane < 0 || (plane_rows > 0 && first_row_in_plane >= plane_rows))
        return fail(-1, "sdfk_eval_device_rows3d: plane_rows >= 0 and 0 <= first_row_in_plane < plane_rows");
    SrcArray a = {d_co, (long long)row_stride};
    bool vec_ok = aligned16(d_co) && aligned16(d_out) && (row_stride % 4 == 0);
    return run(p, &a, nullptr, n, d_out, stream, mode, vec_ok, row_len, nullptr, 0, false, plane_rows, first_row_in_plane);
}

extern "C" int sdfk_eval_device_rows2d(sdfk_program* p, const float* d_co, int64_t n, int64_t row_stride, int64_t row_len,
                                       float* d_out, void* stream, int mode) {
    if (!d_co || !d_out) return fail(-1, "sdfk_eval_device_rows2d: null device pointer");
    if (row_stride < n) return fail(-1, "sdfk_eval_device_rows2d: row stride smaller than the point count");
    if (row_len < 1 || (n > 0 && n % row_len != 0))
        return fail(-1, "sdfk_eval_device_rows2d: the point count is not a multiple of the row length");
    SrcArray a = {d_co, (long long)row_stride};
    bool vec_ok = aligned16(d_co) && aligned16(d_out) && (row_stride % 4 == 0);
    return run(p, &a, nullptr, n, d_out, stream, mode, vec_ok, row_len, nullptr, 0, true);
}

extern "C" int sdfk_eval_device_aux(sdfk_program* p, const float* d_co, int64_t n, int64_t row_stride, const float* d_aux,
                                    int n_aux, int64_t aux_stride, float* d_out, void* stream, int mode) {
    if (!p || !d_co || !d_out) return fail(-1, "sdfk_eval_device_aux: null pointer");
    if (row_stride < n) return fail(-1, "sdfk_eval_device_aux: row stride smaller than the point count");
    if (n_aux < p->n_aux) return fail(-1, "sdfk_eval_device_aux: the program reads more auxiliary fields than were passed");
    SrcArray a = {d_co, (long long)row_stride};
    bool vec_ok = aligned16(d_co) && aligned16(d_out) && (row_stride % 4 == 0);
    return run(p, &a, nullptr, n, d_out, stream, mode, vec_ok, 0, d_aux, aux_stride);
}

extern "C" int sdfk_debug_row_masks(sdfk_program* p, const float* d_co, int64_t n, int64_t row_stride, int64_t row_len,
                                    uint64_t* d_masks, int64_t* n_bricks, int* brick_rows, void* stream_) {
    if (!p || !d_co) return fail(-1, "sdfk_debug_row_masks: null argument");
    if (p->sites.empty()) return fail(-2, "sdfk_debug_row_masks: program has no cull sites");
    if (p->chain_mode) return fail(-2, "sdfk_debug_row_masks: a chain-mode program keeps lists of surviving children, not mask words");
    RowGeom rg;
    if (row_stride < n || !rows_geometry(n, row_len, &rg))
        return fail(-1, "sdfk_debug_row_masks: the row-block kernel does not take this shape");
    if (n_bricks) *n_bricks = rg.nbricks;
    if (brick_rows) *brick_rows = 16;
    if (!d_masks) return 0;
    hipStream_t stream = (hipStream_t)stream_;
    int device = 0;
    HIPCHK(hipGetDevice(&device));
    DevState* d = nullptr;
    int rc = ensure_resident(p, device, stream, &d);
    if (rc) return rc;
    std::string err;
    std::shared_ptr<SpecModule> sk = get_module(p, device, SDFK_FL_ROWS_MASK, true, &err);
    if (!sk || sk->failed) return fail(-3, "specialised kernel unavailable: " + err);
    const float* prm = d->d_params;
    const float* tab = d->d_tables;
    long long stride = row_stride;
    void* args[] = {&prm, &tab, &d_co, &stride, &rg, &d_masks};
    const unsigned per_tile = (unsigned)(rows_waves(p) * rows_wbricks(p));
    HIPCHK(hipModuleLaunchKernel(sk->fn[0], (rg.nbricks + per_tile - 1) / per_tile, 1, 1, 64 * rows_waves(p), 1, 1, 0, stream,
                                 args, nullptr));
    return 0;
}

extern "C" int sdfk_debug_brick_masks(sdfk_program* p, const float* d_co, int64_t n, int64_t row_stride,
                                      uint64_t* d_masks, void* stream_) {
    if (!p || !d_co || !d_masks) return fail(-1, "sdfk_debug_brick_masks: null argument");
    if (!(aligned16(d_co) && row_stride % 4 == 0 && row_stride >= n && n > 0))
        return fail(-1, "sdfk_debug_brick_masks: needs 16-byte aligned rows");
    if (p->sites.empty()) return fail(-2, "sdfk_debug_brick_masks: program has no cull sites");
    if (p->chain_mode) return fail(-2, "sdfk_debug_brick_masks: chain-mode programs have no line-brick flavour");
    hipStream_t stream = (hipStream_t)stream_;
    int device = 0;
    HIPCHK(hipGetDevice(&device));
    DevState* d = nullptr;
    int rc = ensure_resident(p, device, stream, &d);
    if (rc) return rc;
    std::string err;
    std::shared_ptr<SpecModule> sk = get_module(p, device, SDFK_FL_TILE_MASK, true, &err);
    if (!sk || sk->failed) return fail(-3, "specialised kernel unavailable: " + err);
    const float* prm = d->d_params;
    const float* tab = d->d_tables;
    long long stride = row_stride, nn = n;
    void* args[] = {&prm, &tab, &d_co, &stride, &nn, &d_masks};
    HIPCHK(hipModuleLaunchKernel(sk->fn[0], (unsigned)((n + tile_points() - 1) / tile_points()), 1, 1, tile_threads(),
                                 1, 1, 0, stream, args, nullptr));
    return 0;
}

extern "C" int sdfk_linspace_f32(double lo, double hi, int64_t n, float* out) {
    if (n < 0 || (n > 0 && !out)) return fail(-1, "sdfk_linspace_f32: bad arguments");
    if (n == 0) return 0;
    if (n == 1) {
        out[0] = (float)lo;
        return 0;
    }
    const double div = (double)(n - 1);
    const double delta = hi - lo;
    const double step = delta / div;
    for (int64_t i = 0; i < n; ++i) {
        volatile double t = (step != 0.0) ? (double)i * step : ((double)i / div) * delta;
        out[i] = (float)(t + lo);
    }
    out[n - 1] = (float)hi;
    return 0;
}

struct AxisTables {
    float* d = nullptr;
    ~AxisTables() {
        if (d) (void)hipFree(d);
    }
};

static int upload_axes(const float* ax0, int64_t n0, const float* ax1, int64_t n1, const float* ax2, int64_t n2,
                       hipStream_t stream, AxisTables* t, SrcGrid* g, int64_t start) {
    if (!ax0 || !ax1 || !ax2 || n0 < 1 || n1 < 1 || n2 < 1) return fail(-1, "grid axes missing or empty");
    if (n1 > 0x7fffffff || n2 > 0x7fffffff) return fail(-1, "grid axis too long");
    HIPCHK(hipMalloc(&t->d, (size_t)(n0 + n1 + n2) * sizeof(float)));
    HIPCHK(hipMemcpyAsync(t->d, ax0, (size_t)n0 * sizeof(float), hipMemcpyHostToDevice, stream));
    HIPCHK(hipMemcpyAsync(t->d + n0, ax1, (size_t)n1 * sizeof(float), hipMemcpyHostToDevice, stream));
    HIPCHK(hipMemcpyAsync(t->d + n0 + n1, ax2, (size_t)n2 * sizeof(float), hipMemcpyHostToDevice, stream));
    g->ax0 = t->d;
    g->ax1 = t->d + n0;
    g->ax2 = t->d + n0 + n1;
    g->n1 = (unsigned)n1;
    g->n2 = (unsigned)n2;
    g->start = start;
    return 0;
}

extern "C" int sdfk_eval_grid(sdfk_program* p, const float* ax0, int64_t n0, const float* ax1, int64_t n1,
                              const float* ax2, int64_t n2, int64_t start, int64_t count, float* d_out, void* stream,
                              int mode) {
    if (!d_out) return fail(-1, "sdfk_eval_grid: null output");
    if (start < 0 || count < 0 || start + count > n0 * n1 * n2) return fail(-1, "sdfk_eval_grid: range outside the grid");
    AxisTables t;
    SrcGrid g;
    int rc = upload_axes(ax0, n0, ax1, n1, ax2, n2, (hipStream_t)stream, &t, &g, start);
    if (rc) return rc;
    rc = run(p, nullptr, &g, count, d_out, stream, mode, aligned16(d_out));
    if (rc) return rc;
    HIPCHK(hipStreamSynchronize((hipStream_t)stream));
    return 0;
}

extern "C" int sdfk_eval_grid_aux(sdfk_program* p, const float* ax0, int64_t n0, const float* ax1, int64_t n1,
                                  const float* ax2, int64_t n2, int64_t start, int64_t count, const float* d_aux, int n_aux,
                                  int64_t aux_stride, float* d_out, void* stream, int mode) {
    if (!p || !d_out) return fail(-1, "sdfk_eval_grid_aux: null pointer");
    if (start < 0 || count < 0 || start + count > n0 * n1 * n2) return fail(-1, "sdfk_eval_grid_aux: range outside the grid");
    if (n_aux < p->n_aux) return fail(-1, "sdfk_eval_grid_aux: the program reads more auxiliary fields than were passed");
    AxisTables t;
    SrcGrid g;
    int rc = upload_axes(ax0, n0, ax1, n1, ax2, n2, (hipStream_t)stream, &t, &g, start);
    if (rc) return rc;
    rc = run(p, nullptr, &g, count, d_out, stream, mode, aligned16(d_out), 0, d_aux, aux_stride);
    if (rc) return rc;
    HIPCHK(hipStreamSynchronize((hipStream_t)stream));
    return 0;
}

extern "C" int sdfk_eval_grid_host(sdfk_program* p, const float* ax0, int64_t n0, const float* ax1, int64_t n1,
                                   const float* ax2, int64_t n2, int64_t start, int64_t count, float* out, int device,
                                   int mode) {
    if (!p) return fail(-1, "null program");
    if (count < 0 || (count > 0 && !out)) return fail(-1, "sdfk_eval_grid_host: bad arguments");
    if (start < 0 || start + count > n0 * n1 * n2) return fail(-1, "sdfk_eval_grid_host: range outside the grid");
    if (count == 0) return 0;
    HIPCHK(hipSetDevice(device));
    int64_t chunk = std::min<int64_t>(count, (int64_t)1 << 27);
    const int64_t grow = n2 > 1 ? n2 : n1;
    if (start % grow == 0 && chunk > grow) chunk = chunk / grow * grow;
    float* d_out = nullptr;
    HIPCHK(hipMalloc(&d_out, (size_t)chunk * sizeof(float)));
    AxisTables t;
    SrcGrid g;
    int rc = upload_axes(ax0, n0, ax1, n1, ax2, n2, nullptr, &t, &g, start);
    for (int64_t s = 0; s < count && rc == 0; s += chunk) {
        const int64_t m = std::min(chunk, count - s);
        g.start = start + s;
        rc = run(p, nullptr, &g, m, d_out, nullptr, mode, true);
        if (rc == 0 && hipMemcpy(out + s, d_out, (size_t)m * sizeof(float), hipMemcpyDeviceToHost) != hipSuccess)
            rc = fail(-6, "sdfk_eval_grid_host: device-to-host copy failed");
    }
    (void)hipFree(d_out);
    return rc;
}

extern "C" int sdfk_eval_grid_sharded(sdfk_program* p, const float* ax0, int64_t n0, const float* ax1, int64_t n1,
                                      const float* ax2, int64_t n2, int n_shards, const int* devices, float* out,
                                      int mode) {
    if (!p || !out) return fail(-1, "sdfk_eval_grid_sharded: null argument");
    if (n_shards < 1 || n_shards > 64) return fail(-1, "sdfk_eval_grid_sharded: 1..64 shards");
    if (!ax0 || !ax1 || !ax2 || n0 < 1 || n1 < 1 || n2 < 1) return fail(-1, "grid axes missing or empty");
    int n_dev = 0;
    if (hipGetDeviceCount(&n_dev) != hipSuccess || n_dev < 1) return fail(-8, "sdfk_eval_grid_sharded: no HIP device");
    const int64_t total = n0 * n1 * n2, unit = n2 > 1 ? n2 : n1;
    const int64_t per = (total / unit / n_shards) * unit;
    std::vector<int> rc((size_t)n_shards, 0);
    std::vector<std::string> msg((size_t)n_shards);
    std::vector<std::thread> workers;
    for (int d = 0; d < n_shards; ++d) {
        const int dev = devices ? devices[d] : d % n_dev;
        if (dev < 0 || dev >= n_dev) return fail(-1, "sdfk_eval_grid_sharded: device index out of range");
    }
    for (int d = 0; d < n_shards; ++d) {
        const int dev = devices ? devices[d] : d % n_dev;
        const int64_t start = d * per, count = d < n_shards - 1 ? per : total - start;
        workers.emplace_back([=, &rc, &msg] {
            rc[(size_t)d] = count > 0 ? sdfk_eval_grid_host(p, ax0, n0, ax1, n1, ax2, n2, start, count, out + start, dev, mode) : 0;
            if (rc[(size_t)d]) msg[(size_t)d] = sdfk_last_error();
        });
    }
    for (std::thread& t : workers) t.join();
    for (int d = 0; d < n_shards; ++d)
        if (rc[(size_t)d]) return fail(rc[(size_t)d], "shard " + std::to_string(d) + ": " + msg[(size_t)d]);
    return 0;
}

extern "C" int sdfk_eval_grid_sharded_device(sdfk_program* p, const float* ax0, int64_t n0, const float* ax1, int64_t n1,
                                             const float* ax2, int64_t n2, int n_shards, const int* devices,
                                             int gather_device, float* d_full, int mode) {
    if (!p || !d_full) return fail(-1, "sdfk_eval_grid_sharded_device: null argument");
    if (n_shards < 1 || n_shards > 64) return fail(-1, "sdfk_eval_grid_sharded_device: 1..64 shards");
    if (!ax0 || !ax1 || !ax2 || n0 < 1 || n1 < 1 || n2 < 1) return fail(-1, "grid axes missing or empty");
    int n_dev = 0;
    if (hipGetDeviceCount(&n_dev) != hipSuccess || n_dev < 1) return fail(-8, "sdfk_eval_grid_sharded_device: no HIP device");
    if (gather_device < 0 || gather_device >= n_dev) return fail(-1, "sdfk_eval_grid_sharded_device: gather device out of range");
    for (int d = 0; d < n_shards; ++d) {
        const int dev = devices ? devices[d] : d % n_dev;
        if (dev < 0 || dev >= n_dev) return fail(-1, "sdfk_eval_grid_sharded_device: device index out of range");
    }
    const int64_t total = n0 * n1 * n2, unit = n2 > 1 ? n2 : n1;
    const int64_t per = (total / unit / n_shards) * unit;
    std::vector<int> rc((size_t)n_shards, 0);
    std::vector<std::string> msg((size_t)n_shards);
    std::vector<std::thread> workers;
    for (int d = 0; d < n_shards; ++d) {
        const int dev = devices ? devices[d] : d % n_dev;
        const int64_t start = d * per, count = d < n_shards - 1 ? per : total - start;
        workers.emplace_back([=, &rc, &msg] {
            auto shard = [&]() -> int {
                if (count <= 0) return 0;
                HIPCHK(hipSetDevice(dev));
                hipStream_t stream = nullptr;
                HIPCHK(hipStreamCreateWithFlags(&stream, hipStreamNonBlocking));
                static const bool force_copy = [] { const char* e = getenv("SDFK_FORCE_PEER_COPY"); return e && e[0] == '1'; }();
                const bool in_place = dev == gather_device && !force_copy;
                float* d_slab = in_place ? d_full + start : nullptr;
                int r = 0;
                if (!d_slab && hipMalloc(&d_slab, (size_t)count * sizeof(float)) != hipSuccess) r = fail(-5, "out of device memory for the slab");
                if (r == 0) r = sdfk_eval_grid(p, ax0, n0, ax1, n1, ax2, n2, start, count, d_slab, stream, mode);
                if (r == 0 && !in_place) {
                    if (hipMemcpyPeerAsync(d_full + start, gather_device, d_slab, dev, (size_t)count * sizeof(float), stream) != hipSuccess ||
                        hipStreamSynchronize(stream) != hipSuccess)
                        r = fail(-6, "peer copy of the slab failed");
                }
                if (!in_place && d_slab) (void)hipFree(d_slab);
                (void)hipStreamDestroy(stream);
                return r;
            };
            rc[(size_t)d] = shard();
            if (rc[(size_t)d]) msg[(size_t)d] = sdfk_last_error();
        });
    }
    for (std::thread& t : workers) t.join();
    for (int d = 0; d < n_shards; ++d)
        if (rc[(size_t)d]) return fail(rc[(size_t)d], "shard " + std::to_string(d) + ": " + msg[(size_t)d]);
    return 0;
}

extern "C" int sdfk_grid_fill(float* d_co, int64_t row_stride, const float* ax0, int64_t n0, const float* ax1,
                              int64_t n1, const float* ax2, int64_t n2, int64_t start, int64_t count, void* stream) {
    if (!d_co) return fail(-1, "sdfk_grid_fill: null output");
    if (row_stride < count) return fail(-1, "sdfk_grid_fill: row stride smaller than count");
    if (start < 0 || count < 0 || start + count > n0 * n1 * n2) return fail(-1, "sdfk_grid_fill: range outside the grid");
    if (count == 0) return 0;
    AxisTables t;
    SrcGrid g;
    int rc = upload_axes(ax0, n0, ax1, n1, ax2, n2, (hipStream_t)stream, &t, &g, start);
    if (rc) return rc;
    hipLaunchKernelGGL(sdfk_gridfill_kernel, dim3(blocks_for(count, 4)), dim3(SDFK_BLOCK), 0, (hipStream_t)stream, g,
                       (long long)count, d_co, (long long)row_stride);
    HIPCHK(hipGetLastError());
    HIPCHK(hipStreamSynchronize((hipStream_t)stream));
    return 0;
}

template <typename T>
static int64_t detect_row_len(const T* co, int64_t n, int64_t stride, bool* flat, int64_t* plane_rows) {
    const int64_t scan = std::min<int64_t>(n, (int64_t)1 << 22);
    const T *x = co, *y = co + stride, *z = co + 2 * stride;
    int64_t a = 0, b = 0;
    *flat = false;
    *plane_rows = 0;
    for (int64_t i = 1; i < scan && (!a || !b); ++i) {
        if (!b && x[i] != x[0]) b = i;
        if (!a && (x[i] != x[0] || y[i] != y[0])) a = i;
    }
    if (a >= 32 && n % a == 0) {
        if (b > a && b % a == 0) *plane_rows = b / a;
        return a;
    }
    if (b >= 32 && n % b == 0) {
        *flat = z[0] == (T)0 && z[b - 1] == (T)0 && z[n - 1] == (T)0;
        return b;
    }
    return 0;
}

struct HostSlot {
    float *h_co = nullptr, *h_out = nullptr, *d_co = nullptr, *d_out = nullptr;
    hipStream_t stream = nullptr;
    hipEvent_t done = nullptr;
    int64_t pending_start = -1, pending_count = 0;
};
struct HostStage {
    std::mutex mu;
    int64_t chunk = 0;
    HostSlot slot[2];
};
static std::mutex g_stage_mu;
static std::map<int, std::unique_ptr<HostStage>> g_stage;
static int host_threads() {
    static int v = [] {
        const char* e = getenv("SDFK_HOST_THREADS");
        int t = e ? atoi(e) : 0;
        if (t < 1) t = std::min(8, std::max(1, (int)std::thread::hardware_concurrency() / 4));
        return std::min(t, 64);
    }();
    return v;
}
template <typename F>
static void parallel_ranges(int64_t count, F fn) {
// ... 231 lines not shown
```

### aegolius_amd/csrc/sdfk_codegen.cpp

```cpp
#include "sdfk_codegen.h"

#include <algorithm>
#include <cstdio>
#include <cstring>
#include <map>
#include <set>

#include "sdfk_embedded.inc"

std::string sdfk_vector_prelude() { return std::string(kEmbeddedDevice) + "\n" + kEmbeddedVecdev + "\n"; }

static const char kWrappers[] = R"SDFKW(
template <int VEC, typename SRC>
static __device__ __forceinline__ void sdfk_body(const float* __restrict__ PRM, const float* __restrict__ TAB,
                                                 const SRC& src, long long off, long long n,
                                                 float* __restrict__ out, const float* __restrict__ aux,
                                                 long long aux_stride, unsigned* __restrict__ flags, unsigned thr) {
    const long long block_base = (long long)sdfk_bx() * (SDFK_BLOCK * VEC);
    const unsigned lane_off = sdfk_tx() * VEC;
#ifdef SDFK_FLAGS                                              // the flag-writing build of this flavour (its own code object:
    {                                                          // carried as a run-time branch it cost the field kernels registers)
        const bool active = block_base + lane_off < n;
        unsigned nib = 0u;
        if (active) {
// ... 1526 lines not shown
    while (some && sB > sA && !sdfk_slot_rows(g, lv, sB, rb0, rb1)) --sB;
    if (sB == sA) { rb0 = ra0; rb1 = ra1; }
    const long long lo = (long long)(cy << lv.ly) * SDFK_RROWS, hi = (long long)((cy + 1u) << lv.ly) * SDFK_RROWS;
    some = some && ra0 + lo < ra1;
    const unsigned w0 = cz << lv.lz, w1 = ((cz + 1u) << lv.lz) < g.nchunk ? ((cz + 1u) << lv.lz) - 1u : g.nchunk - 1u;
    some = some && w0 < g.nchunk;
    if (!some) {                                                // no brick maps here
        if (lane == 0) { cp.sph[cell] = make_float4(0.0f, 0.0f, 0.0f, -1.0f); cp.span[cell] = make_uint2(0u, 0u); }
        return;
    }
    // windows are aligned in the FLAT array: window k of a row starts up to 31 points before point 32 k of that row
    const unsigned zlo = 32u * w0 > 31u ? 32u * w0 - 31u : 0u;
    const unsigned zhi = 32u * w1 + 31u < g.L ? 32u * w1 + 31u : g.L - 1u;
    // the eight corner points (a lattice cell is their convex hull): lanes 0..7
    const long long rowsel[4] = {ra0 + lo, (ra0 + hi < ra1 ? ra0 + hi : ra1) - 1, (rb0 + lo < rb1 ? rb0 + lo : rb1 - 1),
                                 (rb0 + hi < rb1 ? rb0 + hi : rb1) - 1};
    const float3 pt = sdfk_cell_point(s, g, rowsel[(lane >> 1) & 3], (lane & 1) ? zhi : zlo);
    float mnx = pt.x, mxx = pt.x, mny = pt.y, mxy = pt.y, mnz = pt.z, mxz = pt.z;
#pragma unroll
    for (int o = 1; o < 8; o <<= 1) {
        mnx = fminf(mnx, __shfl_xor(mnx, o)); mxx = fmaxf(mxx, __shfl_xor(mxx, o));
        mny = fminf(mny, __shfl_xor(mny, o)); mxy = fmaxf(mxy, __shfl_xor(mxy, o));
        mnz = fminf(mnz, __shfl_xor(mnz, o)); mxz = fmaxf(mxz, __shfl_xor(mxz, o));
    }
    const V3T<float> ctr = {0.5f * (mnx + mxx), 0.5f * (mny + mxy), 0.5f * (mnz + mxz)};
    const float dx = pt.x - ctr.x, dy = pt.y - ctr.y, dz = pt.z - ctr.z;
    float r2 = dx * dx + dy * dy + dz * dz;
#pragma unroll
    for (int o = 1; o < 8; o <<= 1) r2 = fmaxf(r2, __shfl_xor(r2, o));
    r2 = __shfl(r2, 0);
    const float cxs = __shfl(ctr.x, 0), cys = __shfl(ctr.y, 0), czs = __shfl(ctr.z, 0);
    const V3T<float> c = {cxs, cys, czs};
    // the radius the cell ANSWERS for: bricks test their points against it. A coarse level answers for more than its own
    // sphere (cp.inflate): the circumsphere of a fine cell can reach beyond the circumsphere of the coarse cell it lies in
    // (fine box at a corner, boxes of different proportions), and a fine cell may only start from its parent's list if its
    // whole sphere lies inside what that list answers for.
    const float rho = (1.0001f * sqrtf(r2) + 1e-30f) * cp.inflate;
    if (lane == 0) cp.sph[cell] = make_float4(c.x, c.y, c.z, rho);
    // candidates: the parent's list if this cell's sphere lies inside the parent's answer, else every member
    unsigned off = 0u, cnt = SDFK_NLEAF;
    bool listed = false;
    if (cp.parent.ncx != 0u) {
        unsigned pcx = 0u;
        if (!(lv.xoff > 0u && cx == 0u)) pcx = (cp.parent.xoff + (sA - lv.xoff)) >> cp.parent.lx;
        const unsigned pcell = (pcx * cp.parent.ncy + (cy >> (cp.parent.ly - lv.ly))) * cp.parent.ncz + (cz >> (cp.parent.lz - lv.lz));
        const float4 ps = cp.psph[pcell];
        const uint2 sp = cp.pspan[pcell];
        const float ex = c.x - ps.x, ey = c.y - ps.y, ez = c.z - ps.z;
        if (ps.w > 0.0f && sp.y != SDFK_ALL_ALIVE && 1.00002f * (sqrtf(ex * ex + ey * ey + ez * ez) + rho) <= ps.w) {
            off = sp.x; cnt = sp.y; listed = true;
        }
    }
    const float cmag = 1e-6f * (fabsf(c.x) + fabsf(c.y) + fabsf(c.z) + rho);
    // The candidates' values at the centre: the first SDFK_CELL_NB batches of 64 stay in registers (one evaluation per
    // candidate); what lies beyond is evaluated again for the count and once more for the write.
#ifndef SDFK_CELL_NB
#define SDFK_CELL_NB 8
#endif
#define SDFK_POOL_SHARDS 256u                   // (host: prepare_cells)
    float ev[SDFK_CELL_NB];
    unsigned rv[SDFK_CELL_NB];
    float m = 3.0e38f;
#pragma unroll
    for (int bt = 0; bt < SDFK_CELL_NB; ++bt) {
        const unsigned j = 64u * bt + (unsigned)lane;
        ev[bt] = 3.0e38f;
        rv[bt] = 0u;
        if (64u * bt < cnt) {
            if (j < cnt) {
                rv[bt] = listed ? cp.cand[off + j] : sdfk_member_record(j);
                ev[bt] = SDFK_CHAIN_SGN * sdfk_leaf_rec<float>(rv[bt], c, PRM, TAB);
            }
            m = fminf(m, ev[bt]);
        }
    }
#pragma unroll 4
    for (unsigned j0 = 64u * SDFK_CELL_NB; j0 < cnt; j0 += 64u) {
        const unsigned j = j0 + (unsigned)lane;
        if (j < cnt) m = fminf(m, SDFK_CHAIN_SGN * sdfk_leaf_rec<float>(listed ? cp.cand[off + j] : sdfk_member_record(j), c, PRM, TAB));
    }
#pragma unroll
    for (int o = 1; o < 64; o <<= 1) m = fminf(m, __shfl_xor(m, o));
    const float thr0 = 1.0001f * SDFK_CHAIN_KMAX * rho + SDFK_CHAIN_KMAX * cmag + 1e-6f * (1.0f + fabsf(m));
    unsigned total = 0u;
#pragma unroll
    for (int bt = 0; bt < SDFK_CELL_NB; ++bt)
        if (64u * bt < cnt) total += (unsigned)__builtin_popcountll(__ballot(64u * bt + (unsigned)lane < cnt && !(ev[bt] - m >= thr0 + 1e-6f * fabsf(ev[bt]))));
#pragma unroll 4
    for (unsigned j0 = 64u * SDFK_CELL_NB; j0 < cnt; j0 += 64u) {
        const unsigned j = j0 + (unsigned)lane;
        bool run = false;
        if (j < cnt) {
            const float e = SDFK_CHAIN_SGN * sdfk_leaf_rec<float>(listed ? cp.cand[off + j] : sdfk_member_record(j), c, PRM, TAB);
            run = !(e - m >= thr0 + 1e-6f * fabsf(e));
        }
        total += (unsigned)__builtin_popcountll(__ballot(run));
    }
    // per microsecond and address), so the pool is cut into SDFK_POOL_SHARDS shards with a head each, dealt by cell index
    unsigned at = 0u;
    const unsigned shard = cell & (SDFK_POOL_SHARDS - 1u);
    if (lane == 0) at = atomicAdd(cp.head + 16u * shard, total);
    at = __shfl(at, 0);
    if (at > cp.shard_cap || total > cp.shard_cap - at) {       // the shard is full: bricks of this cell probe every member
        if (lane == 0) cp.span[cell] = make_uint2(0u, SDFK_ALL_ALIVE);
        return;
    }
    at += cp.base + shard * cp.shard_cap;
    unsigned n_out = 0u;
#pragma unroll
    for (int bt = 0; bt < SDFK_CELL_NB; ++bt)
        if (64u * bt < cnt) {
            const bool run = 64u * bt + (unsigned)lane < cnt && !(ev[bt] - m >= thr0 + 1e-6f * fabsf(ev[bt]));
            const unsigned long long bits = __ballot(run);
            if (run) cp.cand[at + n_out + (unsigned)__builtin_popcountll(bits & ((1ull << lane) - 1ull))] = rv[bt];
            n_out += (unsigned)__builtin_popcountll(bits);
        }
#pragma unroll 4
    for (unsigned j0 = 64u * SDFK_CELL_NB; j0 < cnt; j0 += 64u) {
        const unsigned j = j0 + (unsigned)lane;
        bool run = false;
        unsigned rec = 0u;
        if (j < cnt) {
            rec = listed ? cp.cand[off + j] : sdfk_member_record(j);
            const float e = SDFK_CHAIN_SGN * sdfk_leaf_rec<float>(rec, c, PRM, TAB);
            run = !(e - m >= thr0 + 1e-6f * fabsf(e));
        }
        const unsigned long long bits = __ballot(run);
        if (run) cp.cand[at + n_out + (unsigned)__builtin_popcountll(bits & ((1ull << lane) - 1ull))] = rec;
        n_out += (unsigned)__builtin_popcountll(bits);
    }
    if (lane == 0) cp.span[cell] = make_uint2(at, total);
}
#else
#define SDFK_CELLS_KARG
#endif
)SDFKR";
static const char kRowsArray[] = R"SDFKR(
extern "C" __global__ __launch_bounds__(64 * SDFK_RWAVES) SDFK_ROWS_ATTR void sdfk_spec_r(
    const float* __restrict__ PRM, const float* __restrict__ TAB, const float* __restrict__ co, long long stride,
    sdfk_rowgeom g, float* __restrict__ out, unsigned* __restrict__ flags, unsigned thr SDFK_CELLS_KARG) {
    const SrcArray s = {co, stride};
    sdfk_rows_kernel(PRM, TAB, s, g, out, flags, thr SDFK_CELLS_PASS);
}
#ifdef SDFK_CELLS
extern "C" __global__ __launch_bounds__(256) void sdfk_spec_cells(
    const float* __restrict__ PRM, const float* __restrict__ TAB, const float* __restrict__ co, long long stride,
    sdfk_rowgeom g, sdfk_cellpass cp) {
    const SrcArray s = {co, stride};
    sdfk_cells_kernel(PRM, TAB, s, g, cp);
}
#endif
)SDFKR";
static const char kRowsGrid[] = R"SDFKR(
// the same on a regular grid expanded from three per-axis tables (no coordinate array: 4 B/point); the slab
// starts at a row boundary and out[0] is its first point
extern "C" __global__ __launch_bounds__(64 * SDFK_RWAVES) void sdfk_spec_rg(
    const float* __restrict__ PRM, const float* __restrict__ TAB, SrcGrid s, sdfk_rowgeom g, float* __restrict__ out,
    unsigned* __restrict__ flags, unsigned thr SDFK_CELLS_KARG) {
    sdfk_rows_kernel(PRM, TAB, s, g, out, flags, thr SDFK_CELLS_PASS);
}
#ifdef SDFK_CELLS
extern "C" __global__ __launch_bounds__(256) void sdfk_spec_cellsg(
    const float* __restrict__ PRM, const float* __restrict__ TAB, SrcGrid s, sdfk_rowgeom g, sdfk_cellpass cp) {
    sdfk_cells_kernel(PRM, TAB, s, g, cp);
}
#endif
)SDFKR";
static const char kRowsMask[] = R"SDFKR(
// test aid: the skip masks (two 64-bit words per brick: sites 0-31, 32-63; bit 2k = first operand of site k
// skipped, bit 2k+1 = second) followed by the "uniform rows" flag in a third word
extern "C" __global__ __launch_bounds__(64 * SDFK_RWAVES) void sdfk_spec_rmask(
    const float* __restrict__ PRM, const float* __restrict__ TAB, const float* __restrict__ co, long long stride,
    sdfk_rowgeom g, unsigned long long* __restrict__ masks) {
    __shared__ __attribute__((aligned(16))) sdfk_rowmeta meta;
    const SrcArray s = {co, stride};
    unsigned rb, c;
    sdfk_rows_prepare(PRM, TAB, s, g, &meta, sdfk_bx(), rb, c);
    const unsigned q = sdfk_bx() * SDFK_RNBRICK + sdfk_tx();
    if (sdfk_tx() < SDFK_RNBRICK && q < g.nbricks) {
        masks[3ull * q] = meta.mask[0][sdfk_tx()];
        masks[3ull * q + 1] = meta.mask[1][sdfk_tx()];
        masks[3ull * q + 2] = meta.uniform[sdfk_tx()];
    }
}
)SDFKR";

namespace {

struct Gen {
    const sdfk_opinfo* ops;
    int n_ops;
    const uint32_t* code;
    size_t n_instr;
    const std::vector<sdfk_cullsite>* sites;
    std::string s;
    bool rows = false;

    std::vector<int> root_slot;
    int n_root = 0;
    void find_roots() {
        root_slot.assign(n_instr, -1);
        bool c0_intact = true;
        for (size_t i = 0; i < n_instr; ++i) {
            const uint32_t w = code[2 * i];
            const unsigned op = w & 255u, a = (w >> 8) & 255u, b = (w >> 16) & 255u;
            if ((int)op >= n_ops) continue;
            if (ops[op].kind != SDFK_KIND_C_C) continue;
            if (!strcmp(ops[op].name, "XFORM") && b == 0 && c0_intact && n_root < 64) root_slot[i] = n_root++;
            if (a == 0) c0_intact = false;
        }
    }

    void instr_x(size_t i, const char* indent, int mode) {
        const int r = root_slot.empty() ? -1 : root_slot[i];
        if (r < 0 || mode == 0 || (rows && mode == 1)) {
            instr(i, indent, rows && mode == 2);
            return;
        }
        char buf[1400];
        const uint32_t w = code[2 * i], poff = code[2 * i + 1];
        const unsigned a = (w >> 8) & 255u;
        if (rows) {
            snprintf(buf, sizeof buf,
                     "%sif constexpr (ZRUN) {\n"
                     "#ifdef SDFK_FLAT\n"
                     "%s  const V3T<float> bs = op_xform_base_x(X, PRM + %u);\n"
                     "%s  const V3P bp = {sp<f2>(bs.x), sp<f2>(bs.y), sp<f2>(bs.z)};\n"
                     "%s  SDFK_EACH C_%u[q] = op_xform_y(bp, C_0[q].y, PRM + %u);\n"
                     "#else\n"
                     "%s  const V3T<float> bs = op_xform_base(X, Y, PRM + %u);\n"
                     "%s  const V3P bp = {sp<f2>(bs.x), sp<f2>(bs.y), sp<f2>(bs.z)};\n"
                     "%s  SDFK_EACH C_%u[q] = op_xform_z(bp, C_0[q].z, PRM + %u);\n"
                     "#endif\n"
                     "%s} else { SDFK_EACH C_%u[q] = op_xform(C_0[q], PRM + %u, TAB, 0); }\n",
                     indent, indent, poff, indent, indent, a, poff, indent, poff, indent, indent, a, poff, indent, a, poff);
        } else if (mode == 1) {
            snprintf(buf, sizeof buf,
                     "%s{ const V3T<float> bs = op_xform_base(C_0.x, C_0.y, PRM + %u); bases[%d] = bs.x; bases[%d] = bs.y; "
                     "bases[%d] = bs.z;\n%s  C_%u = op_xform_z(bs, C_0.z, PRM + %u); }\n",
                     indent, poff, 3 * r, 3 * r + 1, 3 * r + 2, indent, a, poff);
        } else {
            snprintf(buf, sizeof buf,
                     "%sif constexpr (ZRUN) { const V3T<T> bs = {sp<T>(bases[%d]), sp<T>(bases[%d]), sp<T>(bases[%d])};\n"
                     "%s  C_%u = op_xform_z(bs, C_0.z, PRM + %u); }\n%selse C_%u = op_xform(C_0, PRM + %u, TAB, 0);\n",
                     indent, 3 * r, 3 * r + 1, 3 * r + 2, indent, a, poff, indent, a, poff);
        }
        s += buf;
    }

    void instr(size_t i, const char* indent) { instr(i, indent, false); }
    void instr(size_t i, const char* indent, bool arr) {
        char buf[256];
        const uint32_t w = code[2 * i], poff = code[2 * i + 1];
        const unsigned op = w & 255u, a = (w >> 8) & 255u, b = (w >> 16) & 255u, c = w >> 24;
        if ((int)op >= n_ops) return;
        const sdfk_opinfo& o = ops[op];
        if (!strcmp(o.name, "V_FIELD")) {
            snprintf(buf, sizeof buf, "%sV_%u = sdfk_aux<T>(AUX, AUXS, %u);\n", indent, a, c);
            s += buf;
            return;
        }
        const char* e = arr ? "SDFK_EACH " : "";
        const char* x = arr ? "[q]" : "";
        switch (o.kind) {
            case SDFK_KIND_C_C:
                snprintf(buf, sizeof buf, "%s%sC_%u%s = %s(C_%u%s, PRM + %u, TAB, %u);\n", indent, e, a, x, o.func, b, x, poff, c);
                break;
            case SDFK_KIND_V_C:
                snprintf(buf, sizeof buf, "%s%sV_%u%s = %s(C_%u%s, PRM + %u, TAB);\n", indent, e, a, x, o.func, b, x, poff);
                break;
            case SDFK_KIND_V_V:
                snprintf(buf, sizeof buf, "%s%sV_%u%s = %s(V_%u%s, PRM + %u);\n", indent, e, a, x, o.func, b, x, poff);
                break;
            default:
                snprintf(buf, sizeof buf, "%s%sV_%u%s = %s(V_%u%s, V_%u%s, PRM + %u);\n", indent, e, a, x, o.func, b, x, c, x, poff);
                break;
        }
        s += buf;
    }

    void declare(const char* ctype, const char* vtype, bool arr, bool init = false) {
        std::set<unsigned> cregs, vregs;
        for (size_t i = 0; i < n_instr; ++i) {
            const uint32_t w = code[2 * i];
            const unsigned op = w & 255u, a = (w >> 8) & 255u;
            if ((int)op >= n_ops) continue;
            if (ops[op].kind == SDFK_KIND_C_C) cregs.insert(a);
            else vregs.insert(a);
        }
        char buf[160];
        const char* dim = arr ? "[SDFK_NP]" : "";
        const char* ini = init ? " = {}" : "";
        for (unsigned c : cregs)
            if (c != 0) {
                snprintf(buf, sizeof buf, "    %s C_%u%s;\n", ctype, c, dim);
                s += buf;
            }
        for (unsigned v : vregs) {
            snprintf(buf, sizeof buf, "    %s V_%u%s%s;\n", vtype, v, dim, ini);
            s += buf;
        }
    }

    int site_opening_at(size_t i, size_t hi) const {
        int best = -1;
        for (size_t k = 0; k < sites->size(); ++k) {
            const sdfk_cullsite& t = (*sites)[k];
            if (t.a0 == i && t.comb <= hi && (best < 0 || t.comb > (*sites)[best].comb)) best = (int)k;
        }
        return best;
    }

// ... 871 lines not shown
```

### aegolius_amd/csrc/sdfk_fieldops.inc

```

#include "sdfk_vecdev.h"

#define SDFK_SEL_THREADS 256
#define SDFK_SEL_ITERS 8
#define SDFK_SEL_TILE (SDFK_SEL_THREADS * 4 * SDFK_SEL_ITERS)
#ifndef SDFK_SEL_TPW
#define SDFK_SEL_TPW 4
#endif

static __device__ __forceinline__ int sdfk_wave_inclusive(int v, int lane) {
    for (int d = 1; d < 64; d <<= 1) {
        const int t = __shfl_up(v, d, 64);
        if (lane >= d) v += t;
    }
    return v;
}

static __device__ __forceinline__ unsigned sdfk_sel_flags(const float* __restrict__ f, long long i, long long n, unsigned thr) {
    if (i + 4 <= n) {
        const sdfk_f4 v = __builtin_nontemporal_load(reinterpret_cast<const sdfk_f4*>(f + i));
        return (sdfk_sel_key(v[0]) <= thr ? 1u : 0u) | (sdfk_sel_key(v[1]) <= thr ? 2u : 0u) |
               (sdfk_sel_key(v[2]) <= thr ? 4u : 0u) | (sdfk_sel_key(v[3]) <= thr ? 8u : 0u);
    }
    unsigned m = 0;
// ... 219 lines not shown
extern "C" int sdfk_field_select(const float* d_field, int64_t n, float threshold, int64_t* d_index, int64_t capacity,
                                 int64_t* count, void* d_scratch, void* stream_) {
    if (!count || n < 0 || (n > 0 && !d_field) || capacity < 0) return fail(-1, "sdfk_field_select: bad arguments");
    if ((uintptr_t)d_field & 15) return fail(-1, "sdfk_field_select: the field must be 16-byte aligned");
    if ((uintptr_t)d_scratch & 7) return fail(-1, "sdfk_field_select: the scratch must be 8-byte aligned");
    *count = 0;
    if (n == 0) return 0;
    const unsigned thr = sdfk_sel_key(threshold);
    if (thr == 0xffffffffu) return 0;
    hipStream_t stream = (hipStream_t)stream_;
    const long long nb = (n + SDFK_SEL_TILE - 1) / SDFK_SEL_TILE;
    if (nb > 0x7fffffff) return fail(-1, "sdfk_field_select: field too large");
    Scratch sc;
    const size_t need = (d_index || d_scratch) ? sdfk_field_select_scratch(n) : (size_t)(nb + 1) * sizeof(unsigned long long);
    if (sc.get(d_scratch, need)) return fail(-5, "sdfk_field_select: out of device memory");
    unsigned long long* blk = static_cast<unsigned long long*>(sc.p);
    if (d_index || d_scratch)
        hipLaunchKernelGGL(sdfk_select_count_kernel<true>, dim3((unsigned)((nb + SDFK_SEL_TPW - 1) / SDFK_SEL_TPW)), dim3(SDFK_SEL_THREADS), 0, stream, d_field,
                           (long long)n, thr, blk, reinterpret_cast<unsigned*>(blk + nb + 1));
    else
        hipLaunchKernelGGL(sdfk_select_count_kernel<false>, dim3((unsigned)((nb + SDFK_SEL_TPW - 1) / SDFK_SEL_TPW)), dim3(SDFK_SEL_THREADS), 0, stream, d_field,
                           (long long)n, thr, blk, static_cast<unsigned*>(nullptr));
    hipLaunchKernelGGL(sdfk_select_scan_kernel, dim3(1), dim3(1024), 0, stream, blk, nb);
    hipError_t e = hipGetLastError();
    unsigned long long total = 0;
    if (e == hipSuccess) e = hipMemcpyAsync(&total, blk + nb, sizeof total, hipMemcpyDeviceToHost, stream);
    if (e == hipSuccess) e = hipStreamSynchronize(stream);
    if (e != hipSuccess) return fail(-6, std::string("sdfk_field_select: ") + hipGetErrorString(e));
    *count = (int64_t)total;
    if (!d_index || total == 0) return 0;
    if ((int64_t)total > capacity) return fail(-1, "sdfk_field_select: index buffer smaller than the selection");
    return select_scatter(nb, blk, d_index, stream);
}

extern "C" int sdfk_field_select_finish(int64_t n, int64_t count, int64_t* d_index, int64_t capacity, void* d_scratch,
                                        void* stream_) {
    if (n < 0 || count < 0 || capacity < 0 || !d_scratch || ((uintptr_t)d_scratch & 7))
        return fail(-1, "sdfk_field_select_finish: bad arguments");
    if (n == 0 || count == 0) return 0;
    if (!d_index || count > capacity) return fail(-1, "sdfk_field_select_finish: index buffer smaller than the selection");
    const long long nb = (n + SDFK_SEL_TILE - 1) / SDFK_SEL_TILE;
    unsigned long long* blk = static_cast<unsigned long long*>(d_scratch);
    unsigned long long total = 0;
    HIPCHK(hipMemcpy(&total, blk + nb, sizeof total, hipMemcpyDeviceToHost));
    if ((int64_t)total != count) return fail(-1, "sdfk_field_select_finish: the scratch does not hold a selection of that size");
    return select_scatter(nb, blk, d_index, (hipStream_t)stream_);
}

static long long sel_tiles(const SelGeom& g) { return (g.nslots + SDFK_SEL_THREADS - 1) / SDFK_SEL_THREADS; }
extern "C" size_t sdfk_eval_select_scratch(int64_t n, int64_t row_len) {
    if (n <= 0) return 16;
    long long words = sel_words(sel_geom(n, 0, false));
    if (row_len >= 32 && n % row_len == 0) words = std::max(words, sel_words(sel_geom(n, row_len, true)));
    const long long tiles = words / SDFK_SEL_THREADS + 2;
    return (size_t)(tiles + 1) * sizeof(unsigned long long) + (size_t)(words + 128) * sizeof(unsigned);
}
struct SelScratch {
    unsigned long long* blk;
    unsigned* flags;
    long long tiles;
};
static SelScratch sel_scratch(void* d_scratch, const SelGeom& g) {
    SelScratch sc;
    sc.tiles = sel_tiles(g);
    sc.blk = static_cast<unsigned long long*>(d_scratch);
    sc.flags = reinterpret_cast<unsigned*>(sc.blk + sc.tiles + 1);
    return sc;
}
static int flags_finish(const SelGeom& g, const SelScratch& sc, int64_t* d_index, int64_t capacity, int64_t* count,
                        hipStream_t stream) {
    hipLaunchKernelGGL(sdfk_flags_count_kernel, dim3((unsigned)sc.tiles), dim3(SDFK_SEL_THREADS), 0, stream, sc.flags, g, sc.blk);
    hipLaunchKernelGGL(sdfk_select_scan_kernel, dim3(1), dim3(1024), 0, stream, sc.blk, sc.tiles);
    if (d_index && capacity > 0)
        hipLaunchKernelGGL(sdfk_flags_scatter_kernel, dim3((unsigned)sc.tiles), dim3(SDFK_SEL_THREADS), 0, stream, sc.flags, g, sc.blk,
                           reinterpret_cast<long long*>(d_index), sc.blk + sc.tiles, (long long)capacity);
    hipError_t e = hipGetLastError();
    unsigned long long total = 0;
    if (e == hipSuccess) e = hipMemcpyAsync(&total, sc.blk + sc.tiles, sizeof total, hipMemcpyDeviceToHost, stream);
    if (e == hipSuccess) e = hipStreamSynchronize(stream);
    if (e != hipSuccess) return fail(-6, std::string("sdfk_eval_select: ") + hipGetErrorString(e));
    *count = (int64_t)total;
    if (!d_index || total == 0) return 0;
    if ((int64_t)total > capacity) return fail(-1, "sdfk_eval_select: index buffer smaller than the selection");
    return 0;
}
static bool select_tiled(const sdfk_program* p, long long n, long long row_len, int mode) {
    RowGeom rg;
    return !p->sites.empty() && mode != SDFK_MODE_NOCULL && row_len > 0 && rows_geometry(n, row_len, &rg);
}
static int select_prepare(const SelGeom& g, float threshold, void* d_scratch, hipStream_t stream, SelScratch* sc, unsigned* thr) {
    if (!d_scratch || ((uintptr_t)d_scratch & 7)) return fail(-1, "sdfk_eval_select: the scratch must be 8-byte aligned device memory");
    *sc = sel_scratch(d_scratch, g);
    *thr = sdfk_sel_key(threshold);
    if (g.RB == 16) HIPCHK(hipMemsetAsync(sc->flags + sel_words(g), 0, 64 * sizeof(unsigned), stream));
    else HIPCHK(hipMemsetAsync(sc->flags, 0, (size_t)(sel_words(g) + 64) * sizeof(unsigned), stream));
    return 0;
}

extern "C" int sdfk_eval_device_select(sdfk_program* p, const float* d_co, int64_t n, int64_t row_stride, int64_t row_len,
                                       int flat, float threshold, int64_t* d_index, int64_t capacity, int64_t* count,
                                       void* d_scratch, void* stream_, int mode) {
    if (!p || !d_co || !count || n < 0 || capacity < 0) return fail(-1, "sdfk_eval_device_select: bad arguments");
    if (row_stride < n) return fail(-1, "sdfk_eval_device_select: row stride smaller than the point count");
    if (row_len < 0 || (row_len > 0 && n % row_len != 0)) return fail(-1, "sdfk_eval_device_select: the point count is not a multiple of the row length");
    if (p->n_aux > 0) return fail(-1, "sdfk_eval_device_select: staged programs (auxiliary fields) are evaluated to a field first");
    *count = 0;
    if (n == 0) return 0;
    if (mode == SDFK_MODE_AUTO) mode = g_default_mode;
    hipStream_t stream = (hipStream_t)stream_;
    const SelGeom g = sel_geom(n, row_len, select_tiled(p, n, row_len, mode));
    SelScratch sc;
    unsigned thr = 0;
    int rc = select_prepare(g, threshold, d_scratch, stream, &sc, &thr);
    if (rc) return rc;
    if (thr == 0xffffffffu) {
        HIPCHK(hipMemsetAsync(sc.blk, 0, (size_t)(sc.tiles + 1) * sizeof(unsigned long long), stream));
        HIPCHK(hipStreamSynchronize(stream));
        return 0;
    }
    SrcArray a = {d_co, (long long)row_stride};
    const bool vec_ok = aligned16(d_co) && (row_stride % 4 == 0);
    rc = run(p, &a, nullptr, n, nullptr, stream_, mode, vec_ok, g.RB == 16 ? row_len : 0, nullptr, 0, flat != 0, 0, 0, sc.flags, thr);
    if (rc) return rc;
    return flags_finish(g, sc, d_index, capacity, count, stream);
}

extern "C" int sdfk_eval_grid_select(sdfk_program* p, const float* ax0, int64_t n0, const float* ax1, int64_t n1,
                                     const float* ax2, int64_t n2, int64_t start, int64_t n, float threshold,
                                     int64_t* d_index, int64_t capacity, int64_t* count, void* d_scratch, void* stream_,
                                     int mode) {
    if (!p || !count || capacity < 0) return fail(-1, "sdfk_eval_grid_select: bad arguments");
    if (start < 0 || n < 0 || start + n > n0 * n1 * n2) return fail(-1, "sdfk_eval_grid_select: range outside the grid");
    if (p->n_aux > 0) return fail(-1, "sdfk_eval_grid_select: staged programs (auxiliary fields) are evaluated to a field first");
    *count = 0;
    if (n == 0) return 0;
    if (mode == SDFK_MODE_AUTO) mode = g_default_mode;
    hipStream_t stream = (hipStream_t)stream_;
    const long long grow = n2 > 1 ? n2 : n1;
    const bool tiled = start % grow == 0 && select_tiled(p, n, grow, mode);
    const SelGeom g = sel_geom(n, grow, tiled);
    SelScratch sc;
    unsigned thr = 0;
    int rc = select_prepare(g, threshold, d_scratch, stream, &sc, &thr);
    if (rc) return rc;
    if (thr == 0xffffffffu) {
        HIPCHK(hipMemsetAsync(sc.blk, 0, (size_t)(sc.tiles + 1) * sizeof(unsigned long long), stream));
        HIPCHK(hipStreamSynchronize(stream));
        return 0;
    }
    AxisTables t;
    SrcGrid sg;
    rc = upload_axes(ax0, n0, ax1, n1, ax2, n2, stream, &t, &sg, start);
    if (rc) return rc;
    rc = run(p, nullptr, &sg, n, nullptr, stream_, mode, true, 0, nullptr, 0, false, 0, 0, sc.flags, thr);
    if (rc) return rc;
    return flags_finish(g, sc, d_index, capacity, count, stream);
}

extern "C" int sdfk_eval_select_finish(sdfk_program* p, int64_t n, int64_t row_len, int mode, int64_t count, int64_t* d_index,
                                       int64_t capacity, void* d_scratch, void* stream_) {
    if (!p || n < 0 || count < 0 || capacity < 0 || !d_scratch || ((uintptr_t)d_scratch & 7))
        return fail(-1, "sdfk_eval_select_finish: bad arguments");
    if (n == 0 || count == 0) return 0;
    if (!d_index || count > capacity) return fail(-1, "sdfk_eval_select_finish: index buffer smaller than the selection");
    if (mode == SDFK_MODE_AUTO) mode = g_default_mode;
    const SelGeom g = sel_geom(n, row_len, select_tiled(p, n, row_len, mode));
    const SelScratch sc = sel_scratch(d_scratch, g);
    unsigned long long total = 0;
    HIPCHK(hipMemcpy(&total, sc.blk + sc.tiles, sizeof total, hipMemcpyDeviceToHost));
    if ((int64_t)total != count) return fail(-1, "sdfk_eval_select_finish: the scratch does not hold a selection of that size");
    hipLaunchKernelGGL(sdfk_flags_scatter_kernel, dim3((unsigned)sc.tiles), dim3(SDFK_SEL_THREADS), 0, (hipStream_t)stream_,
                       sc.flags, g, sc.blk, reinterpret_cast<long long*>(d_index));
    HIPCHK(hipGetLastError());
    HIPCHK(hipStreamSynchronize((hipStream_t)stream_));
    return 0;
}

#define SDFK_GRAD_BAND 32

static __device__ __forceinline__ float sdfk_diff(float lo, float c, float hi, int pos, int n, bool* central) {
    *central = pos != 0 && pos != n - 1;
    return pos == 0 ? hi - c : (pos == n - 1 ? c - lo : hi - lo);
}
static __device__ __forceinline__ void sdfk_grad_fetch(const float* __restrict__ f, long long q, long long n, float* v) {
    if (q >= 0 && q + 4 <= n) {
        const sdfk_f4u t = *reinterpret_cast<const sdfk_f4u*>(f + q);
        v[0] = t[0]; v[1] = t[1]; v[2] = t[2]; v[3] = t[3];
    } else {
        for (int e = 0; e < 4; ++e) v[e] = (q + e >= 0 && q + e < n) ? f[q + e] : 0.0f;
    }
}

__global__ __launch_bounds__(256) void sdfk_gradient_kernel(const float* __restrict__ f, GridDims d, float* __restrict__ out,
                                                            long long stride, long long n, int ncomp, int normalize, int band,
                                                            unsigned S, unsigned total) {
    const unsigned per = (total + 7) / 8;
    const unsigned L = (sdfk_bx() % 8) * per + sdfk_bx() / 8;
    if (L >= total) return;
    const unsigned s = L % S, t = L / S, i = t % (unsigned)d.n0, b = t / (unsigned)d.n0;
    const long long plane = (long long)d.n1 * d.n2;
    const long long jlo = (long long)b * band, jhi = jlo + band < d.n1 ? jlo + band : d.n1;
    const long long lo = ((long long)i * d.n1 + jlo) * d.n2, hi = ((long long)i * d.n1 + jhi) * d.n2;
    const long long p = ((lo + 3) & ~3ll) + ((long long)s * 256 + sdfk_tx()) * 4;
    if (p >= ((hi + 3) & ~3ll) || p >= n) return;
    long long q = p - (long long)i * plane;
    int ii = (int)i;
    if (q >= plane) {
        q -= plane;
        ++ii;
    }
    int j = plane <= 0xffffffffll ? (int)((unsigned)q / (unsigned)d.n2) : (int)(q / d.n2);
    int k = (int)(q - (long long)j * d.n2);
    float c[4], zl, zr, ylo[4], yhi[4], xlo[4], xhi[4];
    sdfk_grad_fetch(f, p, n, c);
    zl = p > 0 ? f[p - 1] : 0.0f;
    zr = p + 4 < n ? f[p + 4] : 0.0f;
    if (ncomp > 1) {
        sdfk_grad_fetch(f, p - d.n2, n, ylo);
        sdfk_grad_fetch(f, p + d.n2, n, yhi);
    }
    if (ncomp > 2) {
        sdfk_grad_fetch(f, p - plane, n, xlo);
        sdfk_grad_fetch(f, p + plane, n, xhi);
    }
    sdfk_f4 o[3];
    for (int e = 0; e < 4; ++e) {
        bool cx = false, cy = false, cz;
        float gx = ncomp > 2 ? sdfk_diff(xlo[e], c[e], xhi[e], ii, d.n0, &cx) : 0.0f;
        float gy = ncomp > 1 ? sdfk_diff(ylo[e], c[e], yhi[e], j, d.n1, &cy) : 0.0f;
        float gz = sdfk_diff(e ? c[e - 1] : zl, c[e], e < 3 ? c[e + 1] : zr, k, d.n2, &cz);
        if (normalize) {
            sdfk_unit3(gx, gy, gz, cx, cy, cz);
        } else {
            gx = cx ? 0.5f * gx : gx;
            gy = cy ? 0.5f * gy : gy;
            gz = cz ? 0.5f * gz : gz;
        }
        o[0][e] = gx;
        o[1][e] = gy;
        o[2][e] = gz;
        if (++k == d.n2) {
            k = 0;
            if (++j == d.n1) {
                j = 0;
                ++ii;
            }
        }
    }
    for (int a = 3 - ncomp; a < 3; ++a) {
        float* dst = out + (long long)(a - (3 - ncomp)) * stride + p;
        if (p + 4 <= n) {
            __builtin_nontemporal_store(o[a], reinterpret_cast<sdfk_f4*>(dst));
        } else {
            for (int e = 0; p + e < n; ++e) dst[e] = o[a][e];
        }
    }
}

#define SDFK_GC_SEG 2
#define SDFK_GC_USE 62

template <int S4, bool NORM>
__global__ __launch_bounds__(256) void sdfk_gradient_carry_kernel(const float* __restrict__ f, GridDims d, float* __restrict__ out,
                                                                  long long stride, long long n, unsigned wgs_per_seg,
                                                                  unsigned total, int seg_len, unsigned group) {
    unsigned L;
    if (group == 0) {
        const unsigned per = (total + 7) / 8;
        L = (sdfk_bx() % 8) * per + sdfk_bx() / 8;
    } else {
        const unsigned x = sdfk_bx() % 8, t = sdfk_bx() / 8;
        L = ((t / group) * 8 + x) * group + t % group;
    }
    if (L >= total) return;
    const unsigned seg = L / wgs_per_seg, chunk = L - seg * wgs_per_seg;
    const int lane = sdfk_tx() & 63, wave = sdfk_tx() >> 6;
    const long long plane = (long long)d.n1 * d.n2;
    const int i0 = (int)seg * seg_len, i1 = min(i0 + seg_len, d.n0);
    const int a0 = (int)((4 - ((long long)i0 * plane) % 4) % 4);
    const long long g = -1 + (long long)(chunk * 4u + wave) * SDFK_GC_USE + (lane - 1);
    long long q = 4 * g + a0;
    long long P = (long long)i0 * plane + q;
    long long jq = q >= 0 ? q / d.n2 : -((-q + d.n2 - 1) / d.n2);
    int j0 = (int)jq, k0 = (int)(q - jq * d.n2);
    const bool lender = lane == 0 || lane == 63;
    float behind[4] = {0.0f, 0.0f, 0.0f, 0.0f}, centre[4], ahead[4] = {0.0f, 0.0f, 0.0f, 0.0f};
    if (i0 > 0) sdfk_grad_fetch(f, P - (plane - S4), n, behind);
    sdfk_grad_fetch(f, P, n, centre);
    for (int i = i0; i < i1; ++i) {
        if (i + 1 < d.n0) sdfk_grad_fetch(f, P + (plane - S4), n, ahead);
        float ylo[4], yhi[4];
        sdfk_grad_fetch(f, P - d.n2, n, ylo);
        sdfk_grad_fetch(f, P + d.n2, n, yhi);
        float xlo[4], xhi[4];
#pragma unroll
        for (int e = 0; e < 4; ++e) {
            if (e + S4 <= 3) xhi[e] = ahead[e + S4];
            if (e - S4 >= 0) xlo[e] = behind[e - S4];
        }
#pragma unroll
        for (int t = 0; t < S4; ++t) {
            xhi[4 - S4 + t] = __shfl_down(ahead[t], 1);
            xlo[t] = __shfl_up(behind[4 - S4 + t], 1);
        }
        const float zl = __shfl_up(centre[3], 1), zr = __shfl_down(centre[0], 1);
        if (!lender) {
            sdfk_f4 o[3];
// ... 117 lines not shown
```

### include/sdfk.h

```cpp
#ifndef SDFK_H
#define SDFK_H

#include <stddef.h>
#include <stdint.h>

#ifdef __cplusplus
extern "C" {
#endif

#define SDFK_ABI_VERSION 1

#define SDFK_MODE_AUTO 0
#define SDFK_MODE_INTERPRET 1
#define SDFK_MODE_SPECIALIZED 2
#define SDFK_MODE_NOCULL 3

typedef struct sdfk_program sdfk_program;

int sdfk_abi_version(void);
int sdfk_device_count(void);
const char* sdfk_last_error(void);

sdfk_program* sdfk_program_create(const uint32_t* code, size_t n_instr, const float* params, size_t n_params,
                                  const float* tables, size_t n_tables, int result_reg);
void sdfk_program_destroy(sdfk_program* prog);
int sdfk_program_set_params(sdfk_program* prog, const float* params, size_t n_params);
int sdfk_program_set_cull(sdfk_program* prog, const uint32_t* sites, size_t n_sites, const float* k);
int sdfk_program_chain_members(const sdfk_program* prog);
const char* sdfk_program_source(sdfk_program* prog);
int sdfk_program_compile_check(sdfk_program* prog, size_t* code_size);
#define SDFK_FLAVOUR_PLAIN_ARRAY 0
#define SDFK_FLAVOUR_PLAIN_GRID 1
#define SDFK_FLAVOUR_TILE_ARRAY 2
#define SDFK_FLAVOUR_TILE_GRID 3
#define SDFK_FLAVOUR_TILE_MASK 4
#define SDFK_FLAVOUR_ROWS_ARRAY 5
#define SDFK_FLAVOUR_ROWS_GRID 6
#define SDFK_FLAVOUR_ROWS_MASK 7
#define SDFK_FLAVOUR_ROWS2D_ARRAY 8
#define SDFK_FLAVOUR_ROWS2D_GRID 9
#define SDFK_FLAVOUR_RAYS 10
#define SDFK_FLAVOUR_OCCUPANCY 11
#define SDFK_FLAVOUR_FLAGS 0x100
#define SDFK_FLAVOUR_XY 0x200
int sdfk_program_compile_flavour(sdfk_program* prog, int flavour, size_t* code_size, double* seconds);
void sdfk_debug_cells_stats(int enable, long long* out8);
void sdfk_debug_rays_stats(int enable, long long* out8);
int sdfk_debug_compile_external(sdfk_program* prog, int flavour, size_t* code_size);
void sdfk_jit_drain(void);
void sdfk_jit_cancel(void);
void sdfk_debug_jit_stats(int64_t* builds, double* seconds);
void sdfk_debug_set_rtc_defs(const char* defs);

int sdfk_eval_device(sdfk_program* prog, const float* d_co, int64_t n, int64_t row_stride, float* d_out,
                     void* stream, int mode);
int sdfk_eval_device_rows(sdfk_program* prog, const float* d_co, int64_t n, int64_t row_stride, int64_t row_len,
                          float* d_out, void* stream, int mode);
int sdfk_eval_device_rows3d(sdfk_program* prog, const float* d_co, int64_t n, int64_t row_stride, int64_t row_len,
                            int64_t plane_rows, int64_t first_row_in_plane, float* d_out, void* stream, int mode);
int sdfk_eval_device_rows2d(sdfk_program* prog, const float* d_co, int64_t n, int64_t row_stride, int64_t row_len,
                            float* d_out, void* stream, int mode);
int sdfk_eval_device_rows2d_xy(sdfk_program* prog, const float* d_xy, int64_t n, int64_t row_stride, int64_t row_len,
                               float* d_out, void* stream, int mode);
int sdfk_eval_host(sdfk_program* prog, const void* co, int co_dtype, int64_t n, int64_t row_stride, float* out,
                   int device, int mode);
int sdfk_eval_host_resident(sdfk_program* prog, const void* co, int co_dtype, int64_t n, int64_t row_stride,
                            float* d_out, int device, int mode);
int sdfk_eval_grid(sdfk_program* prog, const float* ax0, int64_t n0, const float* ax1, int64_t n1, const float* ax2,
                   int64_t n2, int64_t start, int64_t count, float* d_out, void* stream, int mode);
int sdfk_eval_grid_host(sdfk_program* prog, const float* ax0, int64_t n0, const float* ax1, int64_t n1,
                        const float* ax2, int64_t n2, int64_t start, int64_t count, float* out, int device, int mode);
int sdfk_eval_grid_sharded(sdfk_program* prog, const float* ax0, int64_t n0, const float* ax1, int64_t n1,
                           const float* ax2, int64_t n2, int n_shards, const int* devices, float* out, int mode);
int sdfk_eval_grid_sharded_device(sdfk_program* prog, const float* ax0, int64_t n0, const float* ax1, int64_t n1,
                                  const float* ax2, int64_t n2, int n_shards, const int* devices, int gather_device,
                                  float* d_full, int mode);
void sdfk_set_default_mode(int mode);
int sdfk_debug_brick_masks(sdfk_program* prog, const float* d_co, int64_t n, int64_t row_stride, uint64_t* d_masks,
                           void* stream);
int sdfk_debug_row_masks(sdfk_program* prog, const float* d_co, int64_t n, int64_t row_stride, int64_t row_len,
                         uint64_t* d_masks, int64_t* n_bricks, int* brick_rows, void* stream);

int sdfk_eval_device_aux(sdfk_program* prog, const float* d_co, int64_t n, int64_t row_stride, const float* d_aux,
                         int n_aux, int64_t aux_stride, float* d_out, void* stream, int mode);
int sdfk_eval_grid_aux(sdfk_program* prog, const float* ax0, int64_t n0, const float* ax1, int64_t n1, const float* ax2,
                       int64_t n2, int64_t start, int64_t count, const float* d_aux, int n_aux, int64_t aux_stride,
                       float* d_out, void* stream, int mode);
int sdfk_field_min(const float* d_field, int64_t n, float* out_min, void* stream);
int sdfk_grid_box_average(float* d_field, int64_t n0, int64_t n1, int64_t n2, int k0, int k1, int k2, int iterations,
                          void* d_scratch, void* stream);
int sdfk_grid_edge_detect(float* d_field, int64_t n0, int64_t n1, int64_t n2, void* d_scratch, void* stream);
int sdfk_grid_signed(float* d_field, int64_t n0, int64_t n1, int64_t n2, float sep_min, int crop, void* d_scratch,
                     void* stream);
int sdfk_debug_box_variant(int64_t n0, int64_t n1, int64_t n2, int k0, int k1, int k2, int* out8);
int sdfk_grid_boundary_mask(const float* d_field, int64_t n, float sep_min, unsigned char* d_mask, void* stream);
int sdfk_grid_signed_slab(float* d_slab, int64_t plane0, int64_t planes, const unsigned char* d_mask, int64_t n0, int64_t n1,
                          int64_t n2, int crop, void* d_scratch, void* stream);

size_t sdfk_field_select_scratch(int64_t n);
int sdfk_field_select_finish(int64_t n, int64_t count, int64_t* d_index, int64_t capacity, void* d_scratch, void* stream);

size_t sdfk_eval_select_scratch(int64_t n, int64_t row_len);
int sdfk_eval_device_select(sdfk_program* prog, const float* d_co, int64_t n, int64_t row_stride, int64_t row_len, int flat,
                            float threshold, int64_t* d_index, int64_t capacity, int64_t* count, void* d_scratch,
                            void* stream, int mode);
int sdfk_eval_grid_select(sdfk_program* prog, const float* ax0, int64_t n0, const float* ax1, int64_t n1, const float* ax2,
                          int64_t n2, int64_t start, int64_t count_points, float threshold, int64_t* d_index,
                          int64_t capacity, int64_t* count, void* d_scratch, void* stream, int mode);
int sdfk_eval_select_finish(sdfk_program* prog, int64_t n, int64_t row_len, int mode, int64_t count, int64_t* d_index,
                            int64_t capacity, void* d_scratch, void* stream);
int sdfk_field_select(const float* d_field, int64_t n, float threshold, int64_t* d_index, int64_t capacity,
                      int64_t* count, void* d_scratch, void* stream);
int sdfk_field_gradient(const float* d_field, int64_t n0, int64_t n1, int64_t n2, int ncomp, int normalize,
                        float* d_vec, int64_t row_stride, void* stream);

int sdfk_field_crossings_2d(const float* d_uu, const float* d_ww, int64_t n0, int64_t n1, int64_t n2, double w, double d,
                            double thr, signed char* d_sign, void* stream);
int sdfk_lcwg_eval(int variant, const float* d_uu, const float* d_ww, int64_t n0, int64_t n1, int64_t n2, double w, double d,
                   int sign_kind, double sign_value, const void* d_sign, float* d_vec, int64_t row_stride, void* stream);
int sdfk_lcwg_old_eval(int variant, const float* d_r, int64_t r_stride, const float* d_uu, int64_t n, double w, double d,
                       float* d_vec, int64_t row_stride, void* stream);

typedef struct {
    int32_t op;
    int32_t src[2];
    float imm[4];
} sdfk_vec_instr;
int sdfk_vec_eval_device(const sdfk_vec_instr* prog, int n_instr, const float* d_p, int64_t n, int64_t p_stride,
                         const float* d_streams, int n_streams, int64_t stream_stride, int out_kind, float* d_out,
                         int64_t out_stride, void* stream);
void sdfk_vec_set_interpret(int on);
const char* sdfk_vec_source(const sdfk_vec_instr* prog, int n_instr, int n_streams, int out_kind);
int sdfk_vec_compile_check(const sdfk_vec_instr* prog, int n_instr, int n_streams, int out_kind, size_t* code_size);
int sdfk_vec_eval_host(const sdfk_vec_instr* prog, int n_instr, const void* p, int p_dtype, int64_t n, const float* ax0,
                       int64_t n0, const float* ax1, int64_t n1, const float* ax2, int64_t n2, const float* streams,
                       int n_streams, int out_kind, float* out, int device);

int sdfk_linspace_f32(double lo, double hi, int64_t n, float* out);
int64_t sdfk_point_tree_build(const float* pts, int64_t m, int leaf, float* table, int64_t table_cap, int64_t* order,
                              int64_t* n_root, int64_t* point_base);

int sdfk_grid_fill(float* d_co, int64_t row_stride, const float* ax0, int64_t n0, const float* ax1, int64_t n1,
                   const float* ax2, int64_t n2, int64_t start, int64_t count, void* stream);

int sdfk_set_device(int device);
void* sdfk_malloc(size_t bytes);
int sdfk_free(void* d_ptr);
int sdfk_memcpy_h2d(void* d_dst, const void* src, size_t bytes);
int sdfk_memcpy_d2h(void* dst, const void* d_src, size_t bytes);
int sdfk_memcpy_d2d(void* d_dst, const void* d_src, size_t bytes);
int sdfk_sync(void* stream);
void* sdfk_event_create(void);
int sdfk_event_destroy(void* ev);
int sdfk_event_record(void* ev, void* stream);
int sdfk_event_elapsed_ms(void* ev_start, void* ev_stop, float* ms);
int sdfk_stream_probe(const float* d_co, int64_t n, int64_t row_stride, float* d_out, void* stream);


int sdfk_dual_has_rule(int op);
int sdfk_program_jvp_check(sdfk_program* prog, int* first_bad_op);
int sdfk_eval_jvp_device(sdfk_program* prog, const float* d_co, int64_t n, int64_t row_stride, const float* d_dparams, int k,
                         int seed_points, float* d_value, float* d_tangent, int64_t tangent_stride, void* stream);
int sdfk_value_jvp_device(int op, const float* P, const float* d_v, const float* d_t, int64_t n, float* d_out_v,
                          float* d_out_t, void* stream);

int sdfk_program_vjp_check(sdfk_program* prog, int* first_bad_op, int64_t* tape_floats);
int sdfk_vjp_limits(int* tape_floats, int* max_params);
int sdfk_eval_vjp_device(sdfk_program* prog, const float* d_co, int64_t n, int64_t row_stride, const float* d_in, int mode,
                         int flags, float* d_out_value, double* h_pbar, double* h_loss, void* stream);

int sdfk_points_bin(const double* d_cloud, int64_t n, int64_t row_stride, const double* d_edges, int64_t rx, int64_t ry,
                    int64_t rz, unsigned char* d_grid, void* stream);
int sdfk_points_extent(const unsigned char* d_grid, int64_t rx, int64_t ry, int64_t rz, unsigned char* d_flags, void* stream);
int sdfk_points_fill(unsigned char* d_grid, int64_t rx, int64_t ry, int64_t rz, int axis, int64_t src, int64_t lo, int64_t hi,
                     void* stream);
int sdfk_points_widen(const unsigned char* d_grid, int64_t n, int kind, void* d_out, void* stream);

size_t sdfk_field_isosurface_scratch(int64_t n0, int64_t n1, int64_t n2);
int sdfk_field_isosurface(const float* d_field, const float* ax0, int64_t n0, const float* ax1, int64_t n1, const float* ax2,
                          int64_t n2, float level, int64_t* n_vertices, int64_t* n_faces, void* d_scratch, void* stream);
int sdfk_field_isosurface_finish(const float* d_field, int64_t n0, int64_t n1, int64_t n2, float level, int64_t n_vertices,
                                 int64_t n_faces, float* d_vertices, int64_t vertex_capacity, void* d_faces,
                                 int64_t face_capacity, int face_bytes, void* d_scratch, void* stream);
size_t sdfk_field_contour2d_scratch(int64_t n0, int64_t n1);
int sdfk_field_contour2d(const float* d_field, const float* ax0, int64_t n0, const float* ax1, int64_t n1, float level,
                         int64_t* n_vertices, int64_t* n_segments, void* d_scratch, void* stream);
int sdfk_field_contour2d_finish(const float* d_field, int64_t n0, int64_t n1, float level, int64_t n_vertices,
                                int64_t n_segments, float* d_vertices, int64_t vertex_capacity, void* d_segments,
                                int64_t segment_capacity, int segment_bytes, void* d_scratch, void* stream);
size_t sdfk_eval_grid_isosurface_scratch(int64_t n0, int64_t n1, int64_t n2);
int sdfk_eval_grid_isosurface(sdfk_program* prog, const float* ax0, int64_t n0, const float* ax1, int64_t n1, const float* ax2,
                              int64_t n2, float level, int64_t* n_vertices, int64_t* n_faces, void* d_scratch, void* stream,
                              int mode);
int sdfk_eval_grid_isosurface_finish(sdfk_program* prog, const float* ax0, int64_t n0, const float* ax1, int64_t n1,
                                     const float* ax2, int64_t n2, float level, int64_t n_vertices, int64_t n_faces,
                                     float* d_vertices, int64_t vertex_capacity, void* d_faces, int64_t face_capacity,
                                     int face_bytes, void* d_scratch, void* stream, int mode);
size_t sdfk_eval_grid_contour2d_scratch(int64_t n0, int64_t n1);
// ... 46 lines not shown
```

Baseline: 364,800.

## Add axis-table grid rows kernel computing coordinates and cull spheres from tables

Adds a dedicated grid-rows kernel that reads x/y/z directly from per-axis tables. It derives plane and row indices with a reciprocal multiply and builds brick bounding spheres from row end points, which assumes monotone row tables. This replaces the staged path that reused the array kernel's skeleton on table lookups. The host checks that the axes are monotone and free of NaN, and falls back to the staged build for non-monotone tables, oversized slabs, or the cells/chain-staged configurations. The change adds a new kernel variant and a cache key, and the new sphere logic is a correctness risk.

```diff
diff --git a/aegolius_amd/_engine.py b/aegolius_amd/_engine.py
--- a/aegolius_amd/_engine.py
+++ b/aegolius_amd/_engine.py
@@ -33,6 +33,9 @@
     "sdfk_program_compile_check": (_int, [_vp, _c.POINTER(_sz)]),
     "sdfk_program_chain_members": (_int, [_vp]),
     "sdfk_program_compile_flavour": (_int, [_vp, _int, _c.POINTER(_sz), _c.POINTER(_c.c_double)]),
+    "sdfk_program_flavour_source": (_i64, [_vp, _int, _vp, _i64]),
+    "sdfk_axis_monotone": (_int, [_vp, _i64]),
+    "sdfk_debug_grid_stats": (None, [_c.POINTER(_c.c_longlong)]),
     "sdfk_debug_compile_external": (_int, [_vp, _int, _c.POINTER(_sz)]),
     "sdfk_debug_jit_stats": (None, [_c.POINTER(_i64), _c.POINTER(_c.c_double)]),
     "sdfk_jit_drain": (None, []),
@@ -222,6 +225,17 @@
     return n.value, t.value
 
 
+def grid_stats():
+    out = (_c.c_longlong * 2)()
+    lib().sdfk_debug_grid_stats(out)
+    return int(out[0]), int(out[1])
+
+
+def axis_monotone(table):
+    t = np.ascontiguousarray(table, dtype=np.float32).ravel()
+    return bool(lib().sdfk_axis_monotone(_ptr(t), t.size))
+
+
 def _ptr(a):
     return a.ctypes.data_as(_vp) if a is not None and a.size else None
 
@@ -401,6 +415,13 @@
         check(lib().sdfk_program_compile_flavour(self._h, int(flavour), ctypes.byref(n), ctypes.byref(t)),
               "sdfk_program_compile_flavour")
         return n.value, t.value
+
+    def flavour_source(self, flavour):
+        n = lib().sdfk_program_flavour_source(self._h, int(flavour), None, 0)
+        check(min(int(n), 0), "sdfk_program_flavour_source")
+        buf = ctypes.create_string_buffer(int(n))
+        lib().sdfk_program_flavour_source(self._h, int(flavour), buf, int(n))
+        return buf.raw.decode()
 
     def eval_host(self, co, device=0, mode=MODE_AUTO):
         require_gpu()
diff --git a/aegolius_amd/csrc/sdfk.hip b/aegolius_amd/csrc/sdfk.hip
--- a/aegolius_amd/csrc/sdfk.hip
+++ b/aegolius_amd/csrc/sdfk.hip
@@ -612,6 +612,33 @@
     g->inv_bpp = (unsigned)std::min<unsigned long long>(0xffffffffull, (1ull << 32) / (unsigned long long)bpp);
     return true;
 }
+struct GridRows {
+    unsigned pl0, rin0;
+    unsigned inv_n1, pad;
+};
+static bool axis_is_nan(float v) {
+    unsigned u;
+    memcpy(&u, &v, sizeof u);
+    return (u & 0x7fffffffu) > 0x7f800000u;
+}
+extern "C" int sdfk_axis_monotone(const float* a, int64_t n) {
+    if (!a || n < 1) return 0;
+    bool up = true, down = true;
+    if (axis_is_nan(a[0])) return 0;
+    for (int64_t i = 1; i < n; ++i) {
+        if (axis_is_nan(a[i])) return 0;
+        up = up && a[i - 1] <= a[i];
+        down = down && a[i - 1] >= a[i];
+    }
+    return (up || down) ? 1 : 0;
+}
+static std::atomic<long long> g_grid_launches[2];
+extern "C" void sdfk_debug_grid_stats(long long* out2) {
+    for (int i = 0; i < 2; ++i) {
+        const long long v = g_grid_launches[i].exchange(0);
+        if (out2) out2[i] = v;
+    }
+}
 static int tile_threads() { return 64 * tile_waves(); }
 static std::string rtc_cache_dir() {
     static const std::string dir = [] {
@@ -729,10 +756,12 @@
 static std::mutex g_rtc_mu;
 static std::mutex g_defs_mu;
 static std::string g_rtc_defs = [] { const char* e = getenv("SDFK_RTC_DEFS"); return std::string(e ? e : ""); }();
+static std::atomic<bool> g_grid_staged{false};
 extern "C" void sdfk_debug_set_rtc_defs(const char* defs) {
     std::lock_guard<std::mutex> lk(g_defs_mu);
     std::string rest;
     int tw = 0, rwb = 0, rwv = 0;
+    bool staged = false;
     const std::string all = defs ? defs : "";
     size_t pos = 0;
     while (pos < all.size()) {
@@ -742,12 +771,14 @@
         if (tok.compare(0, 14, "-DSDFK_TWAVES=") == 0) tw = atoi(tok.c_str() + 14);
         else if (tok.compare(0, 16, "-DSDFK_RWBRICKS=") == 0) rwb = atoi(tok.c_str() + 16);
         else if (tok.compare(0, 14, "-DSDFK_RWAVES=") == 0) rwv = atoi(tok.c_str() + 14);
+        else if (tok == "-DSDFK_GRID_STAGED" || tok == "-DSDFK_GRID_STAGED=1") staged = true;
         else if (!tok.empty()) rest += tok + " ";
         pos = sp + 1;
     }
     g_twaves_override = (tw >= 1 && tw <= 16) ? tw : 0;
     g_rwbricks_override = (rwb >= 1 && rwb <= 15) ? rwb : 0;
     g_rwaves_override = (rwv >= 1 && rwv <= 16) ? rwv : 0;
+    g_grid_staged.store(staged);
     g_rtc_defs = rest;
 }
 static std::vector<std::string> rtc_options(int geo) {
@@ -1091,10 +1122,13 @@
     return e;
 }
 static std::string flavour_key(const sdfk_program* p, int flavour, int rwb, int with_flags = 0) {
-    return p->key + "|f" + std::to_string(flavour) + ((with_flags & 1) ? "s" : "") + ((with_flags & 2) ? "x" : "") + "|" + rtc_option_key(rwb);
-}
+    return p->key + "|f" + std::to_string(flavour) + ((with_flags & 1) ? "s" : "") + ((with_flags & 2) ? "x" : "") +
+           ((with_flags & 4) ? "g" : "") + "|" + rtc_option_key(rwb);
+}
+static bool grid_rows_flavour(int flavour) { return flavour == SDFK_FL_ROWS_GRID || flavour == SDFK_FL_ROWS2D_GRID; }
 static std::string flavour_source(const sdfk_program* p, int flavour, int with_flags = 0) {
     return std::string((with_flags & 1) ? "#define SDFK_FLAGS 1\n" : "") + ((with_flags & 2) ? "#define SDFK_XY 1\n" : "") +
+           ((with_flags & 4) ? "#define SDFK_GRID_STAGED 1\n" : "") +
            sdfk_generate_source(g_ops, SDFK_OP_COUNT, p->code.data(), p->code.size() / 2, p->result_reg, p->sites, flavour,
                                 &p->sites_all);
 }
@@ -1137,6 +1171,7 @@
     if ((with_flags & 1) && (flavour == SDFK_FL_TILE_ARRAY || flavour == SDFK_FL_TILE_GRID || flavour == SDFK_FL_TILE_MASK ||
                        flavour == SDFK_FL_ROWS_MASK))
         return fail(-2, "sdfk_program_compile_flavour: this flavour has no flag-writing build");
+    if (grid_rows_flavour(flavour) && g_grid_staged.load()) with_flags |= 4;
     const int rwb = rows_geo(p);
     const auto t0 = std::chrono::steady_clock::now();
     std::shared_ptr<CodeObject> e =
@@ -1145,6 +1180,16 @@
     if (code_size) *code_size = e->co.size();
     if (seconds) *seconds = std::chrono::duration<double>(std::chrono::steady_clock::now() - t0).count();
     return 0;
+}
+extern "C" int64_t sdfk_program_flavour_source(sdfk_program* p, int flavour, char* out, int64_t cap) {
+    if (!p || flavour < 0) return fail(-1, "sdfk_program_flavour_source: null program or unknown flavour");
+    int with_flags = ((flavour & SDFK_FLAVOUR_FLAGS) ? 1 : 0) | ((flavour & SDFK_FLAVOUR_XY) ? 2 : 0);
+    flavour &= ~(SDFK_FLAVOUR_FLAGS | SDFK_FLAVOUR_XY);
+    if (flavour >= SDFK_FL_COUNT) return fail(-1, "sdfk_program_flavour_source: unknown flavour");
+    if (grid_rows_flavour(flavour) && g_grid_staged.load()) with_flags |= 4;
+    const std::string src = flavour_source(p, flavour, with_flags);
+    if (out && cap > 0) memcpy(out, src.data(), (size_t)std::min<int64_t>(cap, (int64_t)src.size()));
+    return (int64_t)src.size();
 }
 
 extern "C" int sdfk_debug_compile_external(sdfk_program* p, int flavour, size_t* code_size) {
@@ -1438,7 +1483,7 @@
 static int run(sdfk_program* p, const SrcArray* arr, const SrcGrid* grid, long long n, float* d_out, void* stream_,
                int mode, bool vec_ok, long long row_len = 0, const float* aux = nullptr, long long aux_stride = 0,
                bool flat = false, long long plane_rows = 0, long long plane_phase = 0, unsigned* d_flags = nullptr,
-               unsigned thr_key = 0, bool xy = false) {
+               unsigned thr_key = 0, bool xy = false, bool tables_ok = false) {
     if (!p) return fail(-1, "null program");
     if (n < 0) return fail(-1, "negative point count");
     if (p->n_aux > 0 && (!aux || aux_stride < n))
@@ -1493,11 +1538,14 @@
         }
     }
     std::shared_ptr<SpecModule> sk;
+    bool grid_staged = false;
     if (mode != SDFK_MODE_INTERPRET) {
         static const bool async_jit = [] { const char* e = getenv("SDFK_ASYNC_JIT"); return !(e && e[0] == '0'); }();
         const bool wait = mode != SDFK_MODE_AUTO || !p->interp_ok || !async_jit;
         std::string err;
-        sk = get_module(p, device, flavour, wait, &err, (d_flags ? 1 : 0) | (xy ? 2 : 0));
+        grid_staged = grid_rows_flavour(flavour) &&
+                      (g_grid_staged.load() || !tables_ok || grid->start / grow + rg.R > 0xffffffffLL);
+        sk = get_module(p, device, flavour, wait, &err, (d_flags ? 1 : 0) | (xy ? 2 : 0) | (grid_staged ? 4 : 0));
         if (sk && sk->failed) {
             if (mode == SDFK_MODE_SPECIALIZED || !p->interp_ok)
                 return fail(-3, "specialised kernel unavailable: " + err);
@@ -1536,12 +1584,21 @@
                 SrcGrid g = *grid;
                 rg.row0 = grid->start / grow;
                 rg.yrows = grid->n2 > 1 ? 0 : 1;
+                GridRows gr{};
+                if (rg.yrows) {
+                    gr.pl0 = (unsigned)rg.row0;
+                } else {
+                    gr.pl0 = (unsigned)(rg.row0 / (long long)grid->n1);
+                    gr.rin0 = (unsigned)(rg.row0 % (long long)grid->n1);
+                    gr.inv_n1 = (unsigned)std::min<unsigned long long>(0xffffffffull, (1ull << 32) / (unsigned long long)grid->n1);
+                }
+                g_grid_launches[(grid_staged || with_cells) ? 1 : 0].fetch_add(1);
                 if (with_cells) {
                     void* src[] = {&g};
                     rc = prepare_cells(p, d, sk->fn[1], rg, src, 1, prm, tab, stream, &cells);
                     if (rc) return rc;
                 }
-                void* args[] = {&prm, &tab, &g, &rg, &d_out, &d_flags, &thr_key, &cells};
+                void* args[] = {&prm, &tab, &g, &rg, &d_out, &d_flags, &thr_key, &gr, &cells};
                 HIPCHK(hipModuleLaunchKernel(sk->fn[0], tiles, 1, 1, rthreads, 1, 1, 0, stream, args, nullptr));
             }
             return 0;
@@ -1762,6 +1819,7 @@
 
 struct AxisTables {
     float* d = nullptr;
+    bool tables_ok = false;
     ~AxisTables() {
         if (d) (void)hipFree(d);
     }
@@ -1781,6 +1839,11 @@
     g->n1 = (unsigned)n1;
     g->n2 = (unsigned)n2;
     g->start = start;
+    const bool flat = n2 == 1;
+    bool ok = sdfk_axis_monotone(flat ? ax1 : ax2, flat ? n1 : n2) != 0 && (!flat || (!axis_is_nan(ax2[0]) && ax2[0] == 0.0f));
+    for (int64_t i = 0; ok && i < n0; ++i) ok = !axis_is_nan(ax0[i]);
+    for (int64_t i = 0; ok && !flat && i < n1; ++i) ok = !axis_is_nan(ax1[i]);
+    t->tables_ok = ok;
     return 0;
 }
 
@@ -1793,7 +1856,7 @@
     SrcGrid g;
     int rc = upload_axes(ax0, n0, ax1, n1, ax2, n2, (hipStream_t)stream, &t, &g, start);
     if (rc) return rc;
-    rc = run(p, nullptr, &g, count, d_out, stream, mode, aligned16(d_out));
+    rc = run(p, nullptr, &g, count, d_out, stream, mode, aligned16(d_out), 0, nullptr, 0, false, 0, 0, nullptr, 0, false, t.tables_ok);
     if (rc) return rc;
     HIPCHK(hipStreamSynchronize((hipStream_t)stream));
     return 0;
@@ -1809,7 +1872,7 @@
     SrcGrid g;
     int rc = upload_axes(ax0, n0, ax1, n1, ax2, n2, (hipStream_t)stream, &t, &g, start);
     if (rc) return rc;
-    rc = run(p, nullptr, &g, count, d_out, stream, mode, aligned16(d_out), 0, d_aux, aux_stride);
+    rc = run(p, nullptr, &g, count, d_out, stream, mode, aligned16(d_out), 0, d_aux, aux_stride, false, 0, 0, nullptr, 0, false, t.tables_ok);
     if (rc) return rc;
     HIPCHK(hipStreamSynchronize((hipStream_t)stream));
     return 0;
@@ -1834,7 +1897,7 @@
     for (int64_t s = 0; s < count && rc == 0; s += chunk) {
         const int64_t m = std::min(chunk, count - s);
         g.start = start + s;
-        rc = run(p, nullptr, &g, m, d_out, nullptr, mode, true);
+        rc = run(p, nullptr, &g, m, d_out, nullptr, mode, true, 0, nullptr, 0, false, 0, 0, nullptr, 0, false, t.tables_ok);
         if (rc == 0 && hipMemcpy(out + s, d_out, (size_t)m * sizeof(float), hipMemcpyDeviceToHost) != hipSuccess)
             rc = fail(-6, "sdfk_eval_grid_host: device-to-host copy failed");
     }
diff --git a/aegolius_amd/csrc/sdfk_codegen.cpp b/aegolius_amd/csrc/sdfk_codegen.cpp
--- a/aegolius_amd/csrc/sdfk_codegen.cpp
+++ b/aegolius_amd/csrc/sdfk_codegen.cpp
@@ -1702,12 +1702,375 @@
 #endif
 )SDFKR";
 static const char kRowsGrid[] = R"SDFKR(
-// the same on a regular grid expanded from three per-axis tables (no coordinate array: 4 B/point); the slab
-// starts at a row boundary and out[0] is its first point
+struct sdfk_gridrows {
+    unsigned pl0, rin0;                         // plane (index into ax0) and row in it (into ax1) of the slab's first row;
+    unsigned inv_n1, pad;                       // flat grids: (row0, 0). inv_n1 = floor(2^32 / n1), see sdfk_udiv
+};
+#if !defined(SDFK_GRID_STAGED) && !defined(SDFK_CELLS) && !SDFK_CHAIN_STAGED && SDFK_RTILES == 1 && !defined(SDFK_LDSPAD)
+#define SDFK_GRID_TABLES 1
+#endif
+#ifdef SDFK_GRID_TABLES
+struct sdfk_gridmeta {
+    unsigned r0[SDFK_RNBRICK], nrow[SDFK_RNBRICK], win[SDFK_RNBRICK];   // per brick: first row, rows (0: dead), window
+    unsigned long long mask[SDFK_NMASK][SDFK_RNBRICK];
+#ifdef SDFK_SIMT
+    float4 cen[SDFK_NCEN];
+    float leafval[SDFK_NLEAF * SDFK_NCEN];
+#endif
+#ifdef SDFK_CHAIN
+    unsigned short alist[SDFK_RNBRICK][SDFK_NLEAF];
+    unsigned nalive[SDFK_RNBRICK];
+#endif
+};
+// (plane, row in plane) of local row r of the slab — any lane, no readfirstlane: the probe lanes call it too.
+// r + rin0 < 2^32 (the host sends longer slabs to the staged build); the estimate is never too large, the loop repairs it.
+static __device__ __forceinline__ void sdfk_grid_row(const SrcGrid& s, const sdfk_gridrows& gr, unsigned r, unsigned& ix, unsigned& iy) {
+#ifdef SDFK_FLAT
+    ix = gr.pl0 + r;                                               // rows run along y: one x per row, no planes
+    iy = 0u;
+#elif defined(SDFK_GRID_DIV)                                       // (A/B: the division of the staged kernel)
+    const unsigned long long g0 = (unsigned long long)gr.pl0 * s.n1 + gr.rin0 + r;
+    ix = (unsigned)(g0 / s.n1);
+    iy = (unsigned)(g0 - (unsigned long long)ix * s.n1);
+#else
+    const unsigned t = gr.rin0 + r;
+    unsigned q = __umulhi(t, gr.inv_n1);
+    while (t - q * s.n1 >= s.n1) ++q;
+    ix = gr.pl0 + q;
+    iy = t - q * s.n1;
+#endif
+}
+// the 4 values [z, z+4) of the row table; edge windows: indices clamped into the row as sdfk_win_quad does
+static __device__ __forceinline__ float4 sdfk_tab_quad(const float* __restrict__ tab, int z, int last, bool interior) {
+    if (interior) {
+        const sdfk_f4u v = *reinterpret_cast<const sdfk_f4u*>(tab + z);
+        return make_float4(v.x, v.y, v.z, v.w);
+    }
+    return make_float4(tab[min(max(z, 0), last)], tab[min(max(z + 1, 0), last)], tab[min(max(z + 2, 0), last)],
+                       tab[min(max(z + 3, 0), last)]);
+}
+// Bounding sphere of rows [ra, rb) x window points [i0, i0 + np) of the brick (first row r0, nrow >= 1 live rows, window
+// k): around the midpoint of its first and last point; radius = the maximum over its rows of the distance of the row's
+// two END points of the window part — on a monotone row table no point in between lies further out. Rows past the
+// brick's last stand for that row and indices outside the row for the row's nearest point, as in the staged kernel, so
+// on the same split this is its sphere to the bit. Every index stays inside its table: rows < nrow, points in [0, L).
+static __device__ __forceinline__ float4 sdfk_grid_sphere(const SrcGrid& s, const sdfk_rowgeom& g, const sdfk_gridrows& gr,
+                                                          unsigned r0, int nrow, unsigned k, int ra, int rb, int i0, int np) {
+#ifdef SDFK_ABLATE_BOUNDS
+    return make_float4(0.0f, 0.0f, 0.0f, 1.0f);
+#endif
+    const int last = (int)g.L - 1;
+    const int lo = min(ra, nrow - 1), hi = max(min(rb, nrow), lo + 1);          // rows [lo, hi), lo < hi <= nrow
+#ifdef SDFK_FLAT
+    const float* __restrict__ rowtab = s.ax1;
+#else
+    const float* __restrict__ rowtab = s.ax2;
+#endif
+    long long fl;
+    unsigned ix, iy, jx, jy;
+    sdfk_grid_row(s, gr, r0 + (unsigned)lo, ix, iy);
+    sdfk_grid_row(s, gr, r0 + (unsigned)(hi - 1), jx, jy);
+    const int zf = sdfk_win_z((long long)r0 + lo, g.L, k, i0, &fl), zl = sdfk_win_z((long long)r0 + hi - 1, g.L, k, i0 + np - 1, &fl);
+#ifdef SDFK_FLAT
+    const float yc = s.ax2[0];                                                  // the coordinate every row shares (z = 0)
+    const float cx = 0.5f * (s.ax0[ix] + s.ax0[jx]), cy = 0.5f * (yc + yc);
+#else
+    const float cx = 0.5f * (s.ax0[ix] + s.ax0[jx]), cy = 0.5f * (s.ax1[iy] + s.ax1[jy]);
+#endif
+    const float cz = 0.5f * (rowtab[min(max(zf, 0), last)] + rowtab[min(max(zl, 0), last)]);
+    float r2 = 0.0f;
+#pragma unroll 4
+    for (int rr = lo; rr < hi; ++rr) {
+        const int z0 = sdfk_win_z((long long)r0 + rr, g.L, k, i0, &fl);
+        const float za = rowtab[min(max(z0, 0), last)], ze = rowtab[min(max(z0 + np - 1, 0), last)];
+#ifdef SDFK_FLAT
+        const float dx = s.ax0[ix] - cx, dy = yc - cy;
+        ++ix;
+#else
+        const float dx = s.ax0[ix] - cx, dy = s.ax1[iy] - cy;
+        if (++iy == s.n1) { iy = 0u; ++ix; }                                    // (read again only while rr < hi: in range)
+#endif
+        const float zm = sd_rawmax(sd_abs(za - cz), sd_abs(ze - cz));
+        r2 = sd_rawmax(r2, sd_fma(zm, zm, sd_fma(dx, dx, dy * dy)));
+    }
+    const float rho = 1.00001f * sqrtf(r2) + 1e-30f;
+#ifdef SDFK_FLAT
+    return make_float4(cx, cz, cy, rho);                                        // (x, y along the row, z)
+#else
+    return make_float4(cx, cy, cz, rho);
+#endif
+}
+// probe centre sb of SDFK_NSUB of a brick (sb = 0 of 1: the whole brick), the sub-bricks of sdfk_sub_centre: a brick
+// whose rows come from more than one plane is split where the plane changes instead of in the middle
+static __device__ __forceinline__ float4 sdfk_grid_centre(const SrcGrid& s, const sdfk_rowgeom& g, const sdfk_gridrows& gr,
+                                                          unsigned r0, int nrow, unsigned k, unsigned sb) {
+#if defined(SDFK_SIMT) && SDFK_NSUB > 1
+    constexpr int NZP = 4, NRP = SDFK_NSUB / NZP, RPS = SDFK_RROWS / NRP, ZPS = SDFK_RZ / NZP;
+    static_assert(ZPS % 4 == 0 && RPS >= 1, "sub-brick shape");
+    int ra = (int)(sb / NZP) * RPS, rb = ra + RPS;
+#ifndef SDFK_FLAT
+    if constexpr (NRP == 2) {
+        unsigned ix, iy;
+        sdfk_grid_row(s, gr, r0, ix, iy);
+        if (iy + (unsigned)nrow > s.n1) {                          // the brick's live rows leave the plane of its first row
+            const int cut = (int)(s.n1 - iy);                      // ... after this many rows: 1 .. nrow - 1
+            ra = sb / NZP ? cut : 0;
+            rb = sb / NZP ? SDFK_RROWS : cut;
+        }
+    }
+#endif
+    return sdfk_grid_sphere(s, g, gr, r0, nrow, k, ra, rb, (int)(sb % NZP) * ZPS, ZPS);
+#else
+    (void)sb;
+    return sdfk_grid_sphere(s, g, gr, r0, nrow, k, 0, SDFK_RROWS, 0, SDFK_RZ);
+#endif
+}
+#ifdef SDFK_CHAIN
+// sdfk_chain_fold on this kernel's LDS record (the brick's sphere is its one probe centre: SDFK_NSUB == 1 in chain mode)
+static __device__ __forceinline__ void sdfk_grid_chain_fold(sdfk_gridmeta* meta, int b, int lane) {
+    static_assert(SDFK_NSUB == 1, "chain mode: one probe centre per brick");
+    const float4 cc = meta->cen[b];
+    const float rho = cc.w, cmag = 1e-6f * (fabsf(cc.x) + fabsf(cc.y) + fabsf(cc.z) + rho);
+    constexpr int NW = (SDFK_NLEAF + 63) / 64;
+    float m = 3.0e38f;
+#pragma unroll 4
+    for (int j = 0; j < NW; ++j) {
+        const int k = 64 * j + lane;
+        if (k < SDFK_NLEAF) m = fminf(m, SDFK_CHAIN_SGN * meta->leafval[k * SDFK_NCEN + b]);
+    }
+#pragma unroll
+    for (int o = 1; o < 64; o <<= 1) m = fminf(m, __shfl_xor(m, o));
+    const float thr0 = 1.0001f * SDFK_CHAIN_KMAX * rho + SDFK_CHAIN_KMAX * cmag + 1e-6f * (1.0f + fabsf(m));
+    int n_out = 0;
+#pragma unroll 1
+    for (int j = 0; j < NW; ++j) {
+        const int k = 64 * j + lane;
+        const bool in = k < SDFK_NLEAF;
+        const float e = in ? SDFK_CHAIN_SGN * meta->leafval[k * SDFK_NCEN + b] : 3.0e38f;
+        const bool run = in && !(e - m >= thr0 + 1e-6f * fabsf(e));
+        const unsigned long long bits = __ballot(run);
+        if (run) meta->alist[b][n_out + __builtin_popcountll(bits & ((1ull << lane) - 1ull))] = (unsigned short)k;
+        n_out += __builtin_popcountll(bits);
+    }
+    if (lane == 0) meta->nalive[b] = (unsigned)n_out;
+}
+#endif
+// phases A and B: every wave leaves the rows and the window of its bricks in LDS (sdfk_block_rows ends in a
+// readfirstlane: not for the divergent probe lanes), the probe lanes bound them from the tables and probe as before
+static __device__ __forceinline__ void sdfk_grid_prepare(const float* __restrict__ PRM, const float* __restrict__ TAB,
+                                                         const SrcGrid& s, const sdfk_rowgeom& g, const sdfk_gridrows& gr,
+                                                         sdfk_gridmeta* meta, unsigned tile, unsigned& rb0, unsigned& c0) {
+    const int lane = sdfk_tx() & 63, wave = __builtin_amdgcn_readfirstlane(sdfk_tx() >> 6);
+    const unsigned q0 = tile * SDFK_RNBRICK + wave * SDFK_RWBRICKS;
+    rb0 = sdfk_udiv(q0, g.nchunk, g.inv_nchunk);
+    c0 = q0 - rb0 * g.nchunk;
+    unsigned rb = rb0, c = c0;
+#pragma unroll
+    for (int j = 0; j < SDFK_RWBRICKS; ++j) {
+        long long r0, rend;
+        sdfk_block_rows(g, rb, r0, rend);
+        const bool live = q0 + j < g.nbricks && r0 < rend;        // (padding of the last tile, blocks of the last plane beyond the slab)
+        if (lane == 0) {
+            const int b = wave * SDFK_RWBRICKS + j;
+            meta->r0[b] = live ? (unsigned)r0 : 0u;
+            meta->nrow[b] = live ? (unsigned)(rend - r0 < SDFK_RROWS ? rend - r0 : SDFK_RROWS) : 0u;
+            meta->win[b] = c;
+#pragma unroll
+            for (int w = 0; w < SDFK_NMASK; ++w) meta->mask[w][b] = ~0ull;      // the fold lanes AND their decisions into these
+        }
+        if (++c == g.nchunk) { c = 0; ++rb; }
+    }
+    __syncthreads();
+#ifdef SDFK_SIMT
+    if (sdfk_tx() < SDFK_NCEN) {
+        const unsigned b = sdfk_tx() / SDFK_NSUB, sb = sdfk_tx() % SDFK_NSUB;
+        const int nrow = (int)meta->nrow[b];
+        float4 cc = make_float4(0.0f, 0.0f, 0.0f, 1.0f);          // a dead brick still meets the probe: harmless values, no table reads
+        if (nrow > 0) cc = sdfk_grid_centre(s, g, gr, meta->r0[b], nrow, meta->win[b], sb);
+        meta->cen[sdfk_tx()] = cc;
+    }
+    __syncthreads();
+#ifndef SDFK_ABLATE_PROBE
+    sdfk_probe_leaves(meta->cen, meta->leafval, PRM, TAB);
+    __syncthreads();
+#ifdef SDFK_CHAIN
+#pragma unroll 1
+    for (int j = 0; j < SDFK_RWBRICKS; ++j)
+        if (q0 + j < g.nbricks) sdfk_grid_chain_fold(meta, wave * SDFK_RWBRICKS + j, lane);
+#else
+    if (sdfk_tx() < SDFK_NCEN && tile * SDFK_RNBRICK + sdfk_tx() / SDFK_NSUB < g.nbricks) {
+        const float4 cc = meta->cen[sdfk_tx()];
+        V3T<float> ctr = {cc.x, cc.y, cc.z};
+        unsigned long long mk[SDFK_NMASK];
+        sdfk_probe_fold(meta->leafval, sdfk_tx(), ctr, cc.w, PRM, mk);
+#pragma unroll
+        for (int w = 0; w < SDFK_NMASK; ++w)
+            __hip_atomic_fetch_and(&meta->mask[w][sdfk_tx() / SDFK_NSUB], mk[w], __ATOMIC_RELAXED, __HIP_MEMORY_SCOPE_WORKGROUP);
+    }
+#endif
+#else
+    if (sdfk_tx() < SDFK_RNBRICK) {
+#pragma unroll
+        for (int w = 0; w < SDFK_NMASK; ++w) meta->mask[w][sdfk_tx()] = 0ull;
+    }
+#endif
+    __syncthreads();
+#else
+    if (sdfk_tx() < SDFK_RNBRICK && tile * SDFK_RNBRICK + sdfk_tx() < g.nbricks) {
+        const int nrow = (int)meta->nrow[sdfk_tx()];
+        float4 bb = make_float4(0.0f, 0.0f, 0.0f, 1.0f);
+        if (nrow > 0) bb = sdfk_grid_centre(s, g, gr, meta->r0[sdfk_tx()], nrow, meta->win[sdfk_tx()], 0u);
+        V3T<float> ctr = {bb.x, bb.y, bb.z};
+        unsigned long long mk[SDFK_NMASK];
+#pragma unroll
+        for (int w = 0; w < SDFK_NMASK; ++w) mk[w] = 0ull;
+#if !defined(SDFK_ABLATE_PROBE) && !defined(SDFK_CHAIN)
+        sdfk_probe_r(ctr, bb.w, PRM, TAB, mk);
+#endif
+#pragma unroll
+        for (int w = 0; w < SDFK_NMASK; ++w) meta->mask[w][sdfk_tx()] = mk[w];
+    }
+    __syncthreads();
+#endif
+}
+static __device__ __forceinline__ void sdfk_grid_kernel(const float* __restrict__ PRM, const float* __restrict__ TAB,
+                                                        const SrcGrid& s, const sdfk_rowgeom& g, const sdfk_gridrows& gr,
+                                                        float* __restrict__ out, unsigned* __restrict__ flags, unsigned thr) {
+    __shared__ __attribute__((aligned(16))) sdfk_gridmeta meta;
+    const int lane = sdfk_tx() & 63, wave = __builtin_amdgcn_readfirstlane(sdfk_tx() >> 6);
+    const int lr = lane / SDFK_RLPR;
+    const int zq = (lane % SDFK_RLPR) * (2 * SDFK_NP);
+    // (the XCD schedule of sdfk_rows_kernel)
+    const unsigned xg_t = sdfk_bx() / 8;
+    const unsigned tile = ((xg_t / SDFK_XGROUP) * 8 + sdfk_bx() % 8) * SDFK_XGROUP + xg_t % SDFK_XGROUP;
+    if (tile * SDFK_RNBRICK >= g.nbricks) return;                 // padding of the launch: nothing is read
+    unsigned rb, c;
+    sdfk_grid_prepare(PRM, TAB, s, g, gr, &meta, tile, rb, c);
+    const unsigned q0 = tile * SDFK_RNBRICK + wave * SDFK_RWBRICKS;
+#pragma unroll 1
+    for (int j = 0; j < SDFK_RWBRICKS; ++j) {
+        if (q0 + j >= g.nbricks) break;
+        const int b = wave * SDFK_RWBRICKS + j;
+        const unsigned k = c;
+        long long r0, rend;
+        sdfk_block_rows(g, rb, r0, rend);
+        if (++c == g.nchunk) { c = 0; ++rb; }
+        if (r0 >= rend) continue;
+        unsigned mw[2 * SDFK_NMASK];                             // the brick's skip bits as scalar words
+#pragma unroll
+        for (int w = 0; w < SDFK_NMASK; ++w) {
+            const unsigned long long m = meta.mask[w][b];
+            mw[2 * w] = __builtin_amdgcn_readfirstlane((unsigned)m);
+            mw[2 * w + 1] = __builtin_amdgcn_readfirstlane((unsigned)(m >> 32));
+        }
+        const bool interior = sdfk_interior(g.L, k);
+#ifdef SDFK_ABLATE_EDGE
+        if (!interior) continue;
+#endif
+        const bool live_row = r0 + lr < rend;
+        const int dr = live_row ? lr : (int)(rend - 1 - r0);      // rows past the end stand for the last one: r0 + dr < rend
+        long long f;                                              // flat index of this lane's first point
+        const int z = sdfk_win_z(r0 + dr, g.L, k, zq, &f);        // its index in the row (edge windows: may lie outside)
+        const int last = (int)g.L - 1;
+        // the lane's row: plane and row in it from the brick's (wave-uniform), x and y straight from the tables
+        unsigned ix, iy;
+        sdfk_grid_row(s, gr, (unsigned)r0, ix, iy);
+        ix = __builtin_amdgcn_readfirstlane(ix);
+        iy = __builtin_amdgcn_readfirstlane(iy);
+        V3P P[SDFK_NP];
+        f2 res[SDFK_NP];
+#ifdef SDFK_FLAT
+        const float cx = s.ax0[ix + (unsigned)dr], cy = s.ax2[0];  // (x, z = 0); y runs along the row
+        SDFK_EACH { P[q].x = sp<f2>(cx); P[q].z = sp<f2>(cy); }
+#pragma unroll
+        for (int q = 0; q < SDFK_NP; q += 2) {
+            const float4 v = sdfk_tab_quad(s.ax1, z + 2 * q, last, interior);
+            P[q].y = {v.x, v.y};
+            P[q + 1].y = {v.z, v.w};
+        }
+#else
+        iy += (unsigned)dr;
+        while (iy >= s.n1) { iy -= s.n1; ++ix; }                   // (n1 < 16: a block spans several planes)
+        const float cx = s.ax0[ix], cy = s.ax1[iy];
+        SDFK_EACH { P[q].x = sp<f2>(cx); P[q].y = sp<f2>(cy); }
+#pragma unroll
+        for (int q = 0; q < SDFK_NP; q += 2) {
+            const float4 v = sdfk_tab_quad(s.ax2, z + 2 * q, last, interior);
+            P[q].z = {v.x, v.y};
+            P[q + 1].z = {v.z, v.w};
+        }
+#endif
+#ifdef SDFK_ABLATE_EVAL
+#ifdef SDFK_FLAT
+        SDFK_EACH res[q] = P[q].y + __builtin_bit_cast(float, mw[0] ^ mw[1] ^ mw[2] ^ mw[3]);
+#else
+        SDFK_EACH res[q] = P[q].z + __builtin_bit_cast(float, mw[0] ^ mw[1] ^ mw[2] ^ mw[3]);
+#endif
+#elif !defined(SDFK_CHAIN)
+        sdfk_rows_culled<true>(cx, cy, P, mw, PRM, TAB, res);
+#endif
+#if defined(SDFK_CHAIN) && !defined(SDFK_ABLATE_EVAL)
+        {   // the children on the brick's list, in order; the first one starts the accumulator (sdfk_rows_kernel)
+            const unsigned cnt = __builtin_amdgcn_readfirstlane(meta.nalive[b]);
+            f2 acc[SDFK_NP];
+#pragma unroll 1
+            for (unsigned i = 0; i < cnt; ++i) {
+                const unsigned rec = __builtin_amdgcn_readfirstlane(sdfk_member_record((unsigned)meta.alist[b][i]));
+                f2 val[SDFK_NP];
+                SDFK_EACH val[q] = sdfk_leaf_rec<f2>(rec, P[q], PRM, TAB);
+                if (i == 0u) { SDFK_EACH acc[q] = val[q]; }
+                else { SDFK_EACH acc[q] = SDFK_CHAIN_CMB(acc[q], val[q], PRM); }
+            }
+            SDFK_EACH res[q] = sdfk_chain_tail<f2>(acc[q], P[q], PRM, TAB);
+        }
+#endif
+#ifdef SDFK_FLAGS                                                  // one bit per point, brick-tiled (see sdfk_rows_kernel)
+        {
+            unsigned bits = 0u;
+            SDFK_EACH bits |= ((sdfk_sel_key(res[q].x) <= thr ? 1u : 0u) | (sdfk_sel_key(res[q].y) <= thr ? 2u : 0u)) << (2 * q);
+            if (!interior) {                                       // an edge window: only the points of this row
+                unsigned ok = 0u;
+                SDFK_EACH {
+                    if (z + 2 * q >= 0 && z + 2 * q <= last) ok |= 1u << (2 * q);
+                    if (z + 2 * q + 1 >= 0 && z + 2 * q + 1 <= last) ok |= 2u << (2 * q);
+                }
+                bits &= ok;
+            }
+            if (!live_row) bits = 0u;                              // rows past the end of the last block: empty slots
+            reinterpret_cast<unsigned char*>(flags)[(unsigned long long)(q0 + j) * 64ull + (unsigned)lane] = (unsigned char)bits;
+        }
+#else
+        if (live_row) {
+            float* po = out + f;
+            if (interior) {
+#pragma unroll
+                for (int q = 0; q < SDFK_NP; q += 2) {
+                    sdfk_f4u v = {res[q].x, res[q].y, res[q + 1].x, res[q + 1].y};
+                    __builtin_nontemporal_store(v, reinterpret_cast<sdfk_f4u*>(po + 2 * q));
+                }
+            } else {
+                SDFK_EACH {
+                    if (z + 2 * q >= 0 && z + 2 * q <= last) po[2 * q] = res[q].x;
+                    if (z + 2 * q + 1 >= 0 && z + 2 * q + 1 <= last) po[2 * q + 1] = res[q].y;
+                }
+            }
+        }
+#endif
+    }
+}
+#endif  // SDFK_GRID_TABLES
+// sdfk_spec_rg: the field (or, SDFK_FLAGS, one bit per point) of whole rows of a regular grid spanned by three per-axis
+// tables — no coordinate array, 4 B/point; the slab starts at a row boundary and out[0] is its first point. The
+// axis-table kernel above, or (SDFK_GRID_STAGED, SDFK_CELLS) the array kernel's skeleton on table look-ups.
 extern "C" __global__ __launch_bounds__(64 * SDFK_RWAVES) void sdfk_spec_rg(
     const float* __restrict__ PRM, const float* __restrict__ TAB, SrcGrid s, sdfk_rowgeom g, float* __restrict__ out,
-    unsigned* __restrict__ flags, unsigned thr SDFK_CELLS_KARG) {
+    unsigned* __restrict__ flags, unsigned thr, sdfk_gridrows gr SDFK_CELLS_KARG) {
+#ifdef SDFK_GRID_TABLES
+    sdfk_grid_kernel(PRM, TAB, s, g, gr, out, flags, thr);
+#else
+    (void)gr;
     sdfk_rows_kernel(PRM, TAB, s, g, out, flags, thr SDFK_CELLS_PASS);
+#endif
 }
 #ifdef SDFK_CELLS
 extern "C" __global__ __launch_bounds__(256) void sdfk_spec_cellsg(
diff --git a/aegolius_amd/csrc/sdfk_fieldops.inc b/aegolius_amd/csrc/sdfk_fieldops.inc
--- a/aegolius_amd/csrc/sdfk_fieldops.inc
+++ b/aegolius_amd/csrc/sdfk_fieldops.inc
@@ -395,7 +395,7 @@
     SrcGrid sg;
     rc = upload_axes(ax0, n0, ax1, n1, ax2, n2, stream, &t, &sg, start);
     if (rc) return rc;
-    rc = run(p, nullptr, &sg, n, nullptr, stream_, mode, true, 0, nullptr, 0, false, 0, 0, sc.flags, thr);
+    rc = run(p, nullptr, &sg, n, nullptr, stream_, mode, true, 0, nullptr, 0, false, 0, 0, sc.flags, thr, false, t.tables_ok);
     if (rc) return rc;
     return flags_finish(g, sc, d_index, capacity, count, stream);
 }
diff --git a/include/sdfk.h b/include/sdfk.h
--- a/include/sdfk.h
+++ b/include/sdfk.h
@@ -44,6 +44,9 @@
 #define SDFK_FLAVOUR_FLAGS 0x100
 #define SDFK_FLAVOUR_XY 0x200
 int sdfk_program_compile_flavour(sdfk_program* prog, int flavour, size_t* code_size, double* seconds);
+int64_t sdfk_program_flavour_source(sdfk_program* prog, int flavour, char* out, int64_t cap);
+int sdfk_axis_monotone(const float* table, int64_t n);
+void sdfk_debug_grid_stats(long long* out2);
 void sdfk_debug_cells_stats(int enable, long long* out8);
 void sdfk_debug_rays_stats(int enable, long long* out8);
 int sdfk_debug_compile_external(sdfk_program* prog, int flavour, size_t* code_size);
```

Result: no change. 365,000, median of 5 (+0.1%).
